# linkedin/spark-tfrecord

Measured on AMD Instinct MI355X. Metric: rows/sec read+write (1M-row Example round-trip), higher is better.
Workload: dtype wire(int64/float32/bytes); 1 GPU; model=Example{id:int64, ints:Int64List[8], floats:FloatList[16], tokens:BytesList[2]}, global_batch=1000000, parallelism=dp1, rows_per_rank=1000000, engine=gpu, storage=/dev/shm, crc_verify=True

## Files before the change

### csrc/codec_core.h

```cpp
#pragma once

#include <cstdint>
#include <cstring>

#include "crc32c.h"

namespace tfrec {

using i64 = int64_t;
using u64 = uint64_t;
using u32 = uint32_t;
using u8 = uint8_t;

enum Kind : int32_t { KIND_BYTES = 1, KIND_FLOAT = 2, KIND_INT64 = 3 };

enum RecordFormat : int32_t { FMT_EXAMPLE = 0, FMT_SEQUENCE = 1, FMT_BYTE_ARRAY = 2 };

enum CodecErr : int32_t {
  ERR_OK = 0,
  ERR_TRUNCATED = -1,
  ERR_BAD_VARINT = -2,
  ERR_KIND_MISMATCH = -3,
  ERR_BAD_WIRETYPE = -4,
  ERR_OVERFLOW = -5,
// ... 455 lines not shown
    c.crc = crc32c_step8(c.crc, c.w0, c.tab);
    c.w0 = c.w1;
    c.wpos += 8;
    c.w1 = cur_load(c, c.wpos + 8);
  }
  u32 crc = c.crc;
  for (i64 b = c.wpos; b < c.len; ++b)
    crc = c.tab[0][(crc ^ c.base[b]) & 0xFF] ^ (crc >> 8);
  return ~crc;
}

TFR_HOSTDEV inline bool cur_varint(ScanCur& c, i64 end, u64* out) {
  i64 avail = end - c.pos;
  if (avail <= 0) return false;
  u64 w = cur_peek(c);
  u64 stops = ~w & kMsbMask;
  if (stops) {
    int nb = (ctz64(stops) >> 3) + 1;
    if (nb > avail) return false;
    u64 v = 0;
    for (int i = 0; i < nb; ++i) v |= ((w >> (8 * i)) & 0x7F) << (7 * i);
    *out = v;
    cur_advance(c, nb);
    return true;
  }
  if (avail < 9) return false;
  u64 v = 0;
  for (int i = 0; i < 8; ++i) v |= ((w >> (8 * i)) & 0x7F) << (7 * i);
  cur_advance(c, 8);
  for (int shift = 56; shift < 64 && c.pos < end; shift += 7) {
    u8 b = (u8)cur_peek(c);
    v |= (u64)(b & 0x7F) << shift;
    cur_advance(c, 1);
    if (!(b & 0x80)) {
      *out = v;
      return true;
    }
  }
  return false;
}

TFR_HOSTDEV inline int32_t cur_skip_field(ScanCur& c, i64 end, u32 wt) {
  u64 tmp;
  switch (wt) {
    case 0:
      return cur_varint(c, end, &tmp) ? ERR_OK : ERR_BAD_VARINT;
    case 1:
      if (end - c.pos < 8) return ERR_TRUNCATED;
      cur_advance(c, 8);
      return ERR_OK;
    case 2:
      if (!cur_varint(c, end, &tmp)) return ERR_BAD_VARINT;
      if ((u64)(end - c.pos) < tmp) return ERR_TRUNCATED;
      cur_advance(c, (i64)tmp);
      return ERR_OK;
    case 5:
      if (end - c.pos < 4) return ERR_TRUNCATED;
      cur_advance(c, 4);
      return ERR_OK;
    default:
      return ERR_BAD_WIRETYPE;
  }
}

TFR_HOSTDEV inline i64 cur_count_terms(ScanCur& c, i64 n) {
  i64 cnt = 0;
  while (n >= 8) {
    cnt += popcount64(~cur_peek(c) & kMsbMask);
    cur_advance(c, 8);
    n -= 8;
  }
  if (n > 0) {
    u64 mask = kMsbMask >> (8 * (8 - n));
    cnt += popcount64(~cur_peek(c) & mask);
    cur_advance(c, n);
  }
  return cnt;
}

TFR_HOSTDEV inline int32_t cur_count_list_body(ScanCur& c, i64 end, int32_t kind,
                                               i64* nvals, i64* nbytes) {
  while (c.pos < end) {
    u64 tag;
    if (!cur_varint(c, end, &tag)) return ERR_BAD_VARINT;
    u32 fieldno = (u32)(tag >> 3), wt = (u32)(tag & 7);
    if (fieldno != 1) {
      int32_t rc = cur_skip_field(c, end, wt);
      if (rc != ERR_OK) return rc;
      continue;
    }
    if (kind == KIND_BYTES) {
      if (wt != 2) return ERR_BAD_WIRETYPE;
      u64 blen;
      if (!cur_varint(c, end, &blen)) return ERR_BAD_VARINT;
      if ((u64)(end - c.pos) < blen) return ERR_TRUNCATED;
      *nvals += 1;
      *nbytes += (i64)blen;
      cur_advance(c, (i64)blen);
    } else if (kind == KIND_FLOAT) {
      if (wt == 2) {
        u64 blen;
        if (!cur_varint(c, end, &blen)) return ERR_BAD_VARINT;
        if ((u64)(end - c.pos) < blen) return ERR_TRUNCATED;
        *nvals += (i64)(blen / 4);
        cur_advance(c, (i64)blen);
      } else if (wt == 5) {
        if (end - c.pos < 4) return ERR_TRUNCATED;
        *nvals += 1;
        cur_advance(c, 4);
      } else {
        return ERR_BAD_WIRETYPE;
      }
    } else {
      if (wt == 2) {
        u64 blen;
        if (!cur_varint(c, end, &blen)) return ERR_BAD_VARINT;
        if ((u64)(end - c.pos) < blen) return ERR_TRUNCATED;
        if (blen && (c.base[c.pos + (i64)blen - 1] & 0x80))
          return ERR_BAD_VARINT;
        *nvals += cur_count_terms(c, (i64)blen);
      } else if (wt == 0) {
        u64 v;
        if (!cur_varint(c, end, &v)) return ERR_BAD_VARINT;
        *nvals += 1;
      } else {
        return ERR_BAD_WIRETYPE;
      }
    }
  }
  return ERR_OK;
}

TFR_HOSTDEV inline int32_t cur_scan_feature_body(ScanCur& c, i64 end,
                                                 int32_t expect_kind,
                                                 int32_t* kind_found, i64* nvals,
                                                 i64* nbytes) {
  while (c.pos < end) {
    u64 tag;
    if (!cur_varint(c, end, &tag)) return ERR_BAD_VARINT;
    u32 fieldno = (u32)(tag >> 3), wt = (u32)(tag & 7);
    if (fieldno >= 1 && fieldno <= 3 && wt == 2) {
      u64 blen;
      if (!cur_varint(c, end, &blen)) return ERR_BAD_VARINT;
      if ((u64)(end - c.pos) < blen) return ERR_TRUNCATED;
      *kind_found = (int32_t)fieldno;
      if (expect_kind >= 0 && (int32_t)fieldno != expect_kind)
        return ERR_KIND_MISMATCH;
      int32_t rc = cur_count_list_body(c, c.pos + (i64)blen, (int32_t)fieldno,
                                       nvals, nbytes);
      if (rc != ERR_OK) return rc;
    } else {
      int32_t rc = cur_skip_field(c, end, wt);
      if (rc != ERR_OK) return rc;
    }
  }
  return ERR_OK;
}

TFR_HOSTDEV inline int32_t cur_scan_features_body(ScanCur& c, i64 end, i64 data_rel,
                                                  const SchemaView& schema,
                                                  int want_seq, FieldStat* stats) {
  i64 body_start = c.pos;
  while (c.pos < end) {
    u64 tag;
    if (!cur_varint(c, end, &tag)) return ERR_BAD_VARINT;
    u32 fieldno = (u32)(tag >> 3), wt = (u32)(tag & 7);
    if (fieldno != 1 || wt != 2) {
      int32_t rc = cur_skip_field(c, end, wt);
      if (rc != ERR_OK) return rc;
      continue;
    }
    u64 entry_len;
    if (!cur_varint(c, end, &entry_len)) return ERR_BAD_VARINT;
    if ((u64)(end - c.pos) < entry_len) return ERR_TRUNCATED;
    i64 ee = c.pos + (i64)entry_len;
    int f = -1;
    bool key_seen = false;
    bool val_seen = false;
    while (c.pos < ee) {
      u64 etag;
      if (!cur_varint(c, ee, &etag)) return ERR_BAD_VARINT;
      u32 efn = (u32)(etag >> 3), ewt = (u32)(etag & 7);
      if (efn == 1 && ewt == 2) {
        if (val_seen) return ERR_RETRY_UNFUSED;
        u64 klen;
        if (!cur_varint(c, ee, &klen)) return ERR_BAD_VARINT;
        if ((u64)(ee - c.pos) < klen) return ERR_TRUNCATED;
        f = schema_find(schema, c.base + c.pos, (int)klen, want_seq);
        key_seen = true;
        cur_advance(c, (i64)klen);
      } else if (efn == 2 && ewt == 2) {
        if (!key_seen) return ERR_RETRY_UNFUSED;
        val_seen = true;
        u64 vlen;
        if (!cur_varint(c, ee, &vlen)) return ERR_BAD_VARINT;
        if ((u64)(ee - c.pos) < vlen) return ERR_TRUNCATED;
        i64 ve = c.pos + (i64)vlen;
        if (f < 0) {
          cur_advance(c, (i64)vlen);
          continue;
        }
        FieldStat* st = &stats[f];
        st->nvals = 0;
        st->nbytes = 0;
        st->nlists = 0;
        st->kind_found = 0;
        st->err = 0;
        st->pos = data_rel + c.pos;
        st->len = (i64)vlen;
        if (!want_seq) {
          int32_t rc = cur_scan_feature_body(c, ve, schema.fields[f].kind,
                                             &st->kind_found, &st->nvals,
                                             &st->nbytes);
          if (rc == ERR_RETRY_UNFUSED) return rc;
          if (rc != ERR_OK) st->err = rc;
        } else {
          while (c.pos < ve && st->err == ERR_OK) {
            u64 ltag;
            if (!cur_varint(c, ve, &ltag)) {
              st->err = ERR_BAD_VARINT;
              break;
            }
            u32 lfn = (u32)(ltag >> 3), lwt = (u32)(ltag & 7);
            if (lfn == 1 && lwt == 2) {
              u64 flen;
              if (!cur_varint(c, ve, &flen) || (u64)(ve - c.pos) < flen) {
                st->err = ERR_TRUNCATED;
                break;
              }
              st->nlists += 1;
              int32_t kf = 0;
              int32_t rc = cur_scan_feature_body(c, c.pos + (i64)flen,
                                                 schema.fields[f].kind, &kf,
                                                 &st->nvals, &st->nbytes);
              if (rc == ERR_RETRY_UNFUSED) return rc;
              if (rc != ERR_OK) {
                st->err = rc;
                break;
              }
              if (kf) st->kind_found = kf;
            } else {
              int32_t rc = cur_skip_field(c, ve, lwt);
              if (rc != ERR_OK) {
                st->err = ERR_TRUNCATED;
                break;
              }
            }
          }
        }
        if (c.pos < ve) cur_advance(c, ve - c.pos);
      } else {
        int32_t rc = cur_skip_field(c, ee, ewt);
        if (rc != ERR_OK) return rc;
      }
    }
    if (f >= 0 && !val_seen) {
      FieldStat* st = &stats[f];
      st->pos = data_rel + body_start;
      st->len = 0;
      st->nvals = 0;
      st->nbytes = 0;
      st->nlists = 0;
      st->kind_found = 0;
      st->err = 0;
    }
  }
  return ERR_OK;
}

TFR_HOSTDEV inline int32_t scan_record_fused(const u8* data, i64 abs_off,
                                             i64 rec_len, int32_t fmt,
                                             const SchemaView& schema,
                                             FieldStat* stats, u32* crc_out,
                                             const uint32_t (*tab)[256]) {
  ScanCur c;
  cur_init(c, data + abs_off, rec_len, tab);
  while (c.pos < rec_len) {
    u64 tag;
    if (!cur_varint(c, rec_len, &tag)) return ERR_BAD_VARINT;
    u32 fieldno = (u32)(tag >> 3), wt = (u32)(tag & 7);
    bool is_features = fieldno == 1;
    bool is_fl = (fmt == FMT_SEQUENCE && fieldno == 2);
    if ((is_features || is_fl) && wt == 2) {
      u64 blen;
      if (!cur_varint(c, rec_len, &blen)) return ERR_BAD_VARINT;
      if ((u64)(rec_len - c.pos) < blen) return ERR_TRUNCATED;
      int32_t rc = cur_scan_features_body(c, c.pos + (i64)blen, abs_off, schema,
                                          is_fl ? 1 : 0, stats);
      if (rc != ERR_OK) return rc;
    } else {
      int32_t rc = cur_skip_field(c, rec_len, wt);
      if (rc != ERR_OK) return rc;
    }
  }
  *crc_out = cur_finish_crc(c);
  return ERR_OK;
}


struct DecodeDst {
  i64* i64_vals;
  float* f32_vals;
  u8* bytes_data;
  i64* elem_len;
  i64* sub_count;
};

TFR_HOSTDEV inline int32_t extract_list_body(const u8* p, const u8* end, int32_t kind,
                                             const DecodeDst& dst, i64* vi, i64* bi) {
  while (p < end) {
    u64 tag;
    p = read_varint(p, end, &tag);
    if (!p) return ERR_BAD_VARINT;
    u32 fieldno = static_cast<u32>(tag >> 3);
    u32 wt = static_cast<u32>(tag & 7);
    if (fieldno != 1) {
      p = skip_field(p, end, wt);
      if (!p) return ERR_TRUNCATED;
      continue;
    }
    if (kind == KIND_BYTES) {
      u64 len;
      p = read_varint(p, end, &len);
      if (!p || static_cast<u64>(end - p) < len) return ERR_TRUNCATED;
      u8* d = dst.bytes_data + *bi;
      u64 i = 0;
      for (; i + 8 <= len; i += 8) {
        u64 w;
        __builtin_memcpy(&w, p + i, 8);
        __builtin_memcpy(d + i, &w, 8);
      }
      for (; i < len; ++i) d[i] = p[i];
      dst.elem_len[*vi] = static_cast<i64>(len);
      *bi += static_cast<i64>(len);
      *vi += 1;
      p += len;
    } else if (kind == KIND_FLOAT) {
      if (wt == 2) {
        u64 len;
        p = read_varint(p, end, &len);
        if (!p || static_cast<u64>(end - p) < len) return ERR_TRUNCATED;
        u64 n = len / 4;
        __builtin_memcpy(dst.f32_vals + *vi, p, n * 4);
        *vi += static_cast<i64>(n);
        p += len;
      } else {
        if (end - p < 4) return ERR_TRUNCATED;
        float v;
        __builtin_memcpy(&v, p, 4);
        dst.f32_vals[(*vi)++] = v;
        p += 4;
      }
    } else {
      if (wt == 2) {
        u64 len;
        p = read_varint(p, end, &len);
        if (!p || static_cast<u64>(end - p) < len) return ERR_TRUNCATED;
        const u8* q = p;
        const u8* qe = p + len;
        while (q < qe) {
          u64 v;
          q = read_varint(q, qe, &v);
          if (!q) return ERR_BAD_VARINT;
          dst.i64_vals[(*vi)++] = static_cast<i64>(v);
        }
        p = qe;
      } else {
        u64 v;
        p = read_varint(p, end, &v);
        if (!p) return ERR_BAD_VARINT;
        dst.i64_vals[(*vi)++] = static_cast<i64>(v);
      }
    }
  }
  return ERR_OK;
}

TFR_HOSTDEV inline int32_t extract_feature_body(const u8* p, const u8* end,
                                                int32_t kind, const DecodeDst& dst,
                                                i64* vi, i64* bi) {
  while (p < end) {
    u64 tag;
    p = read_varint(p, end, &tag);
    if (!p) return ERR_BAD_VARINT;
    u32 fieldno = static_cast<u32>(tag >> 3);
    u32 wt = static_cast<u32>(tag & 7);
    if (fieldno >= 1 && fieldno <= 3 && wt == 2) {
      u64 len;
      p = read_varint(p, end, &len);
      if (!p || static_cast<u64>(end - p) < len) return ERR_TRUNCATED;
      int32_t rc = extract_list_body(p, p + len, kind, dst, vi, bi);
      if (rc != ERR_OK) return rc;
      p += len;
    } else {
      p = skip_field(p, end, wt);
      if (!p) return ERR_TRUNCATED;
    }
  }
  return ERR_OK;
}

TFR_HOSTDEV inline int32_t extract_field(const u8* data, i64 pos, i64 len,
                                         int32_t kind, int32_t is_seq,
                                         const DecodeDst& dst, i64 val_base,
                                         i64 byte_base, i64 list_base) {
  if (pos < 0) return ERR_OK;
  const u8* p = data + pos;
  const u8* end = p + len;
  i64 vi = val_base;
  i64 bi = byte_base;
  if (!is_seq) return extract_feature_body(p, end, kind, dst, &vi, &bi);
  i64 li = list_base;
  while (p < end) {
    u64 tag;
    p = read_varint(p, end, &tag);
    if (!p) return ERR_BAD_VARINT;
    u32 fieldno = static_cast<u32>(tag >> 3);
    u32 wt = static_cast<u32>(tag & 7);
    if (fieldno == 1 && wt == 2) {
      u64 flen;
      p = read_varint(p, end, &flen);
      if (!p || static_cast<u64>(end - p) < flen) return ERR_TRUNCATED;
      i64 v_before = vi;
      int32_t rc = extract_feature_body(p, p + flen, kind, dst, &vi, &bi);
      if (rc != ERR_OK) return rc;
      dst.sub_count[li++] = vi - v_before;
      p += flen;
    } else {
      p = skip_field(p, end, wt);
      if (!p) return ERR_TRUNCATED;
    }
  }
  return ERR_OK;
}


struct FieldColumn {
  int32_t kind;
  int32_t is_seq;
  const u8* presence;
  const i64* row_off;
  const i64* list_off;
  const i64* sub_off;
  const i64* elem_off;
  const u8* bytes_data;
  const i64* i64_vals;
  const float* f32_vals;
};

TFR_HOSTDEV inline i64 list_body_size(const FieldColumn& c, i64 v0, i64 v1) {
  if (c.kind == KIND_FLOAT) {
    i64 n = v1 - v0;
    return n ? (1 + varint_size(static_cast<u64>(4 * n)) + 4 * n) : 0;
  }
  if (c.kind == KIND_INT64) {
    i64 packed = 0;
    for (i64 v = v0; v < v1; ++v)
      packed += varint_size(static_cast<u64>(c.i64_vals[v]));
    return packed ? (1 + varint_size(static_cast<u64>(packed)) + packed) : 0;
  }
  i64 sz = 0;
  for (i64 v = v0; v < v1; ++v) {
    i64 blen = c.elem_off[v + 1] - c.elem_off[v];
    sz += 1 + varint_size(static_cast<u64>(blen)) + blen;
  }
  return sz;
}

TFR_HOSTDEV inline i64 feature_body_size(const FieldColumn& c, i64 v0, i64 v1) {
  i64 body = list_body_size(c, v0, v1);
  return 1 + varint_size(static_cast<u64>(body)) + body;
}

TFR_HOSTDEV inline u8* emit_list_body(u8* o, const FieldColumn& c, i64 v0, i64 v1) {
  if (c.kind == KIND_FLOAT) {
    i64 n = v1 - v0;
    if (n) {
      *o++ = 0x0A;
      o = write_varint(o, static_cast<u64>(4 * n));
      __builtin_memcpy(o, c.f32_vals + v0, static_cast<size_t>(4 * n));
      o += 4 * n;
    }
  } else if (c.kind == KIND_INT64) {
    i64 packed = 0;
    for (i64 v = v0; v < v1; ++v)
      packed += varint_size(static_cast<u64>(c.i64_vals[v]));
    if (packed) {
      *o++ = 0x0A;
      o = write_varint(o, static_cast<u64>(packed));
      for (i64 v = v0; v < v1; ++v)
        o = write_varint(o, static_cast<u64>(c.i64_vals[v]));
    }
  } else {
    for (i64 v = v0; v < v1; ++v) {
      i64 b0 = c.elem_off[v];
      i64 blen = c.elem_off[v + 1] - b0;
      *o++ = 0x0A;
      o = write_varint(o, static_cast<u64>(blen));
      for (i64 i = 0; i < blen; ++i) o[i] = c.bytes_data[b0 + i];
      o += blen;
    }
  }
  return o;
}

TFR_HOSTDEV inline u8* emit_feature_body(u8* o, const FieldColumn& c, i64 v0, i64 v1) {
  i64 body = list_body_size(c, v0, v1);
  *o++ = static_cast<u8>((c.kind << 3) | 2);
  o = write_varint(o, static_cast<u64>(body));
  return emit_list_body(o, c, v0, v1);
}

TFR_HOSTDEV inline i64 features_entry_size(const FieldColumn& c, const SchemaView& s,
                                           int f, i64 v0, i64 v1) {
  i64 fb = feature_body_size(c, v0, v1);
  i64 klen = s.name_len(f);
  return (1 + varint_size(static_cast<u64>(klen)) + klen) +
         (1 + varint_size(static_cast<u64>(fb)) + fb);
}

TFR_HOSTDEV inline u8* emit_features_entry(u8* o, const FieldColumn& c,
                                           const SchemaView& s, int f, i64 v0, i64 v1) {
  i64 fb = feature_body_size(c, v0, v1);
  i64 klen = s.name_len(f);
  *o++ = 0x0A;
  o = write_varint(o, static_cast<u64>(klen));
  const u8* nm = s.name(f);
  for (i64 i = 0; i < klen; ++i) o[i] = nm[i];
  o += klen;
  *o++ = 0x12;
  o = write_varint(o, static_cast<u64>(fb));
  return emit_feature_body(o, c, v0, v1);
}

TFR_HOSTDEV inline i64 feature_list_body_size(const FieldColumn& c, i64 r) {
  i64 sz = 0;
  for (i64 j = c.list_off[r]; j < c.list_off[r + 1]; ++j) {
    i64 fb = feature_body_size(c, c.sub_off[j], c.sub_off[j + 1]);
    sz += 1 + varint_size(static_cast<u64>(fb)) + fb;
  }
  return sz;
}

TFR_HOSTDEV inline u8* emit_feature_list_body(u8* o, const FieldColumn& c, i64 r) {
  for (i64 j = c.list_off[r]; j < c.list_off[r + 1]; ++j) {
    i64 fb = feature_body_size(c, c.sub_off[j], c.sub_off[j + 1]);
    *o++ = 0x0A;
    o = write_varint(o, static_cast<u64>(fb));
    o = emit_feature_body(o, c, c.sub_off[j], c.sub_off[j + 1]);
  }
  return o;
}

TFR_HOSTDEV inline i64 feature_lists_entry_size(const FieldColumn& c,
                                                const SchemaView& s, int f, i64 r) {
  i64 flb = feature_list_body_size(c, r);
  i64 klen = s.name_len(f);
  return (1 + varint_size(static_cast<u64>(klen)) + klen) +
         (1 + varint_size(static_cast<u64>(flb)) + flb);
}

TFR_HOSTDEV inline u8* emit_feature_lists_entry(u8* o, const FieldColumn& c,
                                                const SchemaView& s, int f, i64 r) {
  i64 flb = feature_list_body_size(c, r);
  i64 klen = s.name_len(f);
  *o++ = 0x0A;
  o = write_varint(o, static_cast<u64>(klen));
  const u8* nm = s.name(f);
  for (i64 i = 0; i < klen; ++i) o[i] = nm[i];
  o += klen;
  *o++ = 0x12;
  o = write_varint(o, static_cast<u64>(flb));
  return emit_feature_list_body(o, c, r);
}

TFR_HOSTDEV inline i64 record_payload_size(const FieldColumn* cols,
                                           const SchemaView& s, int32_t fmt, i64 r) {
  i64 ctx_body = 0;
  i64 fl_body = 0;
  for (int f = 0; f < s.nfields; ++f) {
    const FieldColumn& c = cols[f];
    if (!c.presence[r]) continue;
    if (!c.is_seq) {
      i64 e = features_entry_size(c, s, f, c.row_off[r], c.row_off[r + 1]);
      ctx_body += 1 + varint_size(static_cast<u64>(e)) + e;
    } else {
      i64 e = feature_lists_entry_size(c, s, f, r);
      fl_body += 1 + varint_size(static_cast<u64>(e)) + e;
    }
  }
  i64 total = 0;
  if (fmt == FMT_EXAMPLE) {
    total += 1 + varint_size(static_cast<u64>(ctx_body)) + ctx_body;
  } else {
    if (ctx_body) total += 1 + varint_size(static_cast<u64>(ctx_body)) + ctx_body;
    total += 1 + varint_size(static_cast<u64>(fl_body)) + fl_body;
  }
  return total;
}

TFR_HOSTDEV inline u8* emit_record_payload(u8* o, const FieldColumn* cols,
                                           const SchemaView& s, int32_t fmt, i64 r) {
  i64 ctx_body = 0, fl_body = 0;
  for (int f = 0; f < s.nfields; ++f) {
    const FieldColumn& c = cols[f];
    if (!c.presence[r]) continue;
    if (!c.is_seq) {
      i64 e = features_entry_size(c, s, f, c.row_off[r], c.row_off[r + 1]);
      ctx_body += 1 + varint_size(static_cast<u64>(e)) + e;
    } else {
      i64 e = feature_lists_entry_size(c, s, f, r);
      fl_body += 1 + varint_size(static_cast<u64>(e)) + e;
    }
  }
  auto emit_ctx = [&](u8* oo) {
    for (int f = 0; f < s.nfields; ++f) {
      const FieldColumn& c = cols[f];
      if (!c.presence[r] || c.is_seq) continue;
      i64 e = features_entry_size(c, s, f, c.row_off[r], c.row_off[r + 1]);
      *oo++ = 0x0A;
      oo = write_varint(oo, static_cast<u64>(e));
      oo = emit_features_entry(oo, c, s, f, c.row_off[r], c.row_off[r + 1]);
    }
    return oo;
  };
  auto emit_fl = [&](u8* oo) {
    for (int f = 0; f < s.nfields; ++f) {
      const FieldColumn& c = cols[f];
      if (!c.presence[r] || !c.is_seq) continue;
      i64 e = feature_lists_entry_size(c, s, f, r);
      *oo++ = 0x0A;
      oo = write_varint(oo, static_cast<u64>(e));
      oo = emit_feature_lists_entry(oo, c, s, f, r);
    }
    return oo;
  };
  if (fmt == FMT_EXAMPLE) {
    *o++ = 0x0A;
    o = write_varint(o, static_cast<u64>(ctx_body));
    o = emit_ctx(o);
  } else {
    if (ctx_body) {
      *o++ = 0x0A;
      o = write_varint(o, static_cast<u64>(ctx_body));
      o = emit_ctx(o);
    }
    *o++ = 0x12;
    o = write_varint(o, static_cast<u64>(fl_body));
    o = emit_fl(o);
  }
  return o;
}



struct WriteCur {
  u8* base;
  i64 pos;
  i64 wpos;
  u64 win;
  u32 crc;
  const uint32_t (*tab)[256];
};

TFR_HOSTDEV inline void wcur_init(WriteCur& w, u8* base,
                                  const uint32_t (*tab)[256]) {
  w.base = base;
  w.pos = 0;
  w.wpos = 0;
  w.win = 0;
  w.crc = 0xFFFFFFFFu;
  w.tab = tab;
}

TFR_HOSTDEV inline void wcur_flush8(WriteCur& w) {
  __builtin_memcpy(w.base + w.wpos, &w.win, 8);
  w.crc = crc32c_step8(w.crc, w.win, w.tab);
  w.wpos += 8;
  w.win = 0;
}

TFR_HOSTDEV inline void wcur_put(WriteCur& w, u8 b) {
  w.win |= (u64)b << (8 * (w.pos - w.wpos));
  if (++w.pos - w.wpos == 8) wcur_flush8(w);
}

TFR_HOSTDEV inline void wcur_varint(WriteCur& w, u64 v) {
  while (v >= 0x80) {
    wcur_put(w, (u8)(v | 0x80));
    v >>= 7;
  }
  wcur_put(w, (u8)v);
}

TFR_HOSTDEV inline void wcur_bytes(WriteCur& w, const u8* src, i64 n) {
  while (n > 0 && (w.pos - w.wpos) != 0) {
    wcur_put(w, *src++);
    --n;
  }
  while (n >= 8) {
    __builtin_memcpy(&w.win, src, 8);
    w.pos += 8;
    wcur_flush8(w);
    src += 8;
    n -= 8;
  }
  while (n-- > 0) wcur_put(w, *src++);
}

TFR_HOSTDEV inline u32 wcur_finish(WriteCur& w) {
  int rem = (int)(w.pos - w.wpos);
  if (!rem) return ~w.crc;
  __builtin_memcpy(w.base + w.wpos, &w.win, (size_t)rem);
  u32 crc = w.crc;
  for (int i = 0; i < rem; ++i)
    crc = w.tab[0][(crc ^ (u8)(w.win >> (8 * i))) & 0xFF] ^ (crc >> 8);
  return ~crc;
}

TFR_HOSTDEV inline void wcur_list_body(WriteCur& w, const FieldColumn& c,
                                       i64 v0, i64 v1) {
  if (c.kind == KIND_FLOAT) {
    i64 n = v1 - v0;
    if (n) {
      wcur_put(w, 0x0A);
      wcur_varint(w, (u64)(4 * n));
      wcur_bytes(w, (const u8*)(c.f32_vals + v0), 4 * n);
    }
  } else if (c.kind == KIND_INT64) {
// ... 149 lines not shown
```

### csrc/ext.cpp

```cpp

#include <pybind11/numpy.h>
#include <pybind11/pybind11.h>
#include <pybind11/stl.h>

#include <fcntl.h>
#include <unistd.h>

#include <atomic>
#include <condition_variable>
#include <cstring>
#include <functional>
#include <map>
#include <mutex>
#include <stdexcept>
#include <string>
#include <thread>
#include <vector>

#include "codec_core.h"
#include "inflate_core.h"

namespace py = pybind11;
using namespace tfrec;

namespace {


class IOPool {
 public:
  static IOPool& instance() {
    static IOPool* pool = new IOPool(8);
    return *pool;
  }

  int run(bool is_write, int fd, u8* ptr, i64 n, i64 off) {
    return run_spans(n, [=](i64 o, i64 m) {
      return is_write ? do_write(fd, ptr + o, m, off + o)
                      : do_read(fd, ptr + o, m, off + o);
    });
  }

  template <typename Fn>
  int run_spans(i64 n, Fn&& fn) {
    return run_parts(n, 64 << 10, std::forward<Fn>(fn));
  }

  template <typename Fn>
  int run_parts(i64 n, i64 min_span, Fn&& fn) {
    if (n <= 0) return 0;
    int nspan = (int)nthreads_;
    i64 span = (n + nspan - 1) / nspan;
    if (span < min_span) {
      nspan = (int)((n + min_span - 1) / min_span);
      if (nspan < 1) nspan = 1;
      span = (n + nspan - 1) / nspan;
    }
    if (nspan == 1) return fn((i64)0, n);
    if (getenv("TFREC_POOL_DEBUG"))
      fprintf(stderr, "[pool] n=%lld nspan=%d span=%lld\n", (long long)n,
              nspan, (long long)span);
    std::atomic<int> err{0};
    std::atomic<int> left{nspan};
    {
      std::unique_lock<std::mutex> lk(mu_);
      for (int t = 0; t < nspan; ++t) {
        i64 o = (i64)t * span;
        i64 m = std::min(span, n - o);
        tasks_.push_back([=, &err, &left] {
          int e = fn(o, m);
          if (e) err.store(e, std::memory_order_relaxed);
          if (left.fetch_sub(1) == 1) {
            std::lock_guard<std::mutex> dl(done_mu_);
            done_cv_.notify_all();
          }
        });
      }
      cv_.notify_all();
    }
    std::unique_lock<std::mutex> dl(done_mu_);
    done_cv_.wait(dl, [&] { return left.load() == 0; });
    return err.load();
  }

 private:
  explicit IOPool(int n) : nthreads_(n) {
    for (int i = 0; i < n; ++i)
      workers_.emplace_back([this] { worker(); });
  }

  static int do_write(int fd, const u8* p, i64 n, i64 off) {
    while (n > 0) {
      ssize_t w = ::pwrite(fd, p, (size_t)n, (off_t)off);
      if (w < 0) {
        if (errno == EINTR) continue;
        return -errno;
      }
      p += w;
      n -= w;
      off += w;
    }
    return 0;
  }

  static int do_read(int fd, u8* p, i64 n, i64 off) {
    while (n > 0) {
      ssize_t r = ::pread(fd, p, (size_t)n, (off_t)off);
      if (r < 0) {
        if (errno == EINTR) continue;
        return -errno;
      }
      if (r == 0) return -EIO;
      p += r;
      n -= r;
      off += r;
    }
    return 0;
  }

  void worker() {
    for (;;) {
      std::function<void()> task;
      {
        std::unique_lock<std::mutex> lk(mu_);
        cv_.wait(lk, [this] { return !tasks_.empty(); });
        task = std::move(tasks_.back());
        tasks_.pop_back();
      }
      task();
    }
  }

  size_t nthreads_;
  std::vector<std::thread> workers_;
  std::vector<std::function<void()>> tasks_;
  std::mutex mu_;
  std::condition_variable cv_;
  std::mutex done_mu_;
  std::condition_variable done_cv_;
};

void pwrite_parallel(int fd, uintptr_t ptr, i64 n, i64 file_off) {
  int e;
  {
    py::gil_scoped_release rel;
    e = IOPool::instance().run(true, fd, (u8*)ptr, n, file_off);
  }
  if (e) throw std::runtime_error("pwrite failed: " + std::string(strerror(-e)));
}

void pread_parallel(int fd, uintptr_t ptr, i64 n, i64 file_off) {
  int e;
  {
    py::gil_scoped_release rel;
    e = IOPool::instance().run(false, fd, (u8*)ptr, n, file_off);
  }
  if (e) throw std::runtime_error("pread failed: " + std::string(strerror(-e)));
}

struct BufView {
  const u8* data;
  i64 size;
};

BufView as_bytes(const py::buffer& b, py::buffer_info& info) {
  info = b.request();
  if (info.itemsize != 1) throw std::invalid_argument("expected a byte buffer");
  return BufView{static_cast<const u8*>(info.ptr), static_cast<i64>(info.size)};
}


std::pair<py::array_t<i64>, py::array_t<i64>> scan_frames(py::buffer data,
                                                          bool verify_crc) {
  py::buffer_info info;
  BufView buf = as_bytes(data, info);
  std::vector<i64> offs, lens;
  i64 p = 0;
  while (p < buf.size) {
    if (buf.size - p < 12)
      throw std::runtime_error("corrupt TFRecord: truncated frame header at offset " +
                               std::to_string(p));
    u64 len;
    std::memcpy(&len, buf.data + p, 8);
    u32 len_crc;
    std::memcpy(&len_crc, buf.data + p + 8, 4);
    if (verify_crc && mask_crc(crc32c(buf.data + p, 8)) != len_crc)
      throw std::runtime_error("corrupt TFRecord: bad length CRC at offset " +
                               std::to_string(p));
    if (static_cast<u64>(buf.size - p - 12) < len + 4)
      throw std::runtime_error("corrupt TFRecord: truncated payload at offset " +
                               std::to_string(p));
    if (verify_crc) {
      u32 data_crc;
      std::memcpy(&data_crc, buf.data + p + 12 + len, 4);
      if (mask_crc(crc32c(buf.data + p + 12, len)) != data_crc)
        throw std::runtime_error("corrupt TFRecord: bad data CRC at offset " +
                                 std::to_string(p));
    }
    offs.push_back(p + 12);
    lens.push_back(static_cast<i64>(len));
    p += 12 + static_cast<i64>(len) + 4;
  }
  auto off_arr = py::array_t<i64>(offs.size());
  auto len_arr = py::array_t<i64>(lens.size());
  std::memcpy(off_arr.mutable_data(), offs.data(), offs.size() * 8);
  std::memcpy(len_arr.mutable_data(), lens.data(), lens.size() * 8);
  return {off_arr, len_arr};
}

std::pair<py::array_t<i64>, py::array_t<i64>> scan_frame_headers(py::buffer data) {
  return scan_frames(data, false);
}


const char* err_name(int32_t e) {
  switch (e) {
    case ERR_TRUNCATED: return "truncated message";
    case ERR_BAD_VARINT: return "malformed varint";
    case ERR_KIND_MISMATCH: return "feature kind does not match schema";
    case ERR_BAD_WIRETYPE: return "unexpected wire type";
    default: return "codec error";
  }
}

py::list decode_records(py::buffer data, py::array_t<i64> rec_off,
                        py::array_t<i64> rec_len, py::bytes schema_blob,
                        int32_t fmt) {
  py::buffer_info info;
  BufView buf = as_bytes(data, info);
  std::string blob = schema_blob;
  SchemaView schema = schema_view(reinterpret_cast<const u8*>(blob.data()));
  const i64 R = rec_off.size();
  const int F = schema.nfields;
  auto off = rec_off.unchecked<1>();
  auto len = rec_len.unchecked<1>();

  std::vector<FieldStat> stats(static_cast<size_t>(R) * F);
  {
    std::atomic<i64> bad_rec{-1};
    std::atomic<int32_t> bad_rc{0};
    std::atomic<int> bad_field{-1};
    {
      py::gil_scoped_release rel;
      IOPool::instance().run_parts(R, 4096, [&](i64 o, i64 m) {
        for (i64 r = o; r < o + m; ++r) {
          FieldStat* st = stats.data() + r * F;
          for (int f = 0; f < F; ++f) field_stat_clear(&st[f]);
          int32_t rc = scan_record(buf.data, off(r), len(r), fmt, schema, st);
          for (int f = 0; rc == ERR_OK && f < F; ++f)
            if (st[f].err != ERR_OK) {
              rc = st[f].err;
              bad_field.store(f);
            }
          if (rc != ERR_OK) {
            bad_rec.store(r);
            bad_rc.store(rc);
            return 1;
          }
        }
        return 0;
      });
    }
    if (bad_rec.load() >= 0) {
      i64 r = bad_rec.load();
      int32_t rc = bad_rc.load();
      if (rc == ERR_KIND_MISMATCH && bad_field.load() >= 0) {
        int f = bad_field.load();
        std::string nm(reinterpret_cast<const char*>(schema.name(f)),
                       schema.name_len(f));
        throw std::runtime_error("Feature '" + nm +
                                 "' kind does not match requested data type (record " +
                                 std::to_string(r) + ")");
      }
      throw std::runtime_error(std::string("TFRecord decode failed in record ") +
                               std::to_string(r) + ": " + err_name(rc));
    }
  }

  py::list out;
  for (int f = 0; f < F; ++f) {
    const FieldDescRaw& fd = schema.fields[f];
    i64 total_vals = 0, total_bytes = 0, total_lists = 0;
    auto presence = py::array_t<u8>(R);
    auto row_off_arr = py::array_t<i64>(R + 1);
    u8* pres = presence.mutable_data();
    i64* row_off_p = row_off_arr.mutable_data();
    row_off_p[0] = 0;
    py::array_t<i64> list_off_arr(fd.is_seq ? R + 1 : 1);
    i64* list_off_p = list_off_arr.mutable_data();
    list_off_p[0] = 0;
    for (i64 r = 0; r < R; ++r) {
      const FieldStat& st = stats[r * F + f];
      pres[r] = st.pos >= 0 ? 1 : 0;
      total_vals += st.nvals;
      total_bytes += st.nbytes;
      total_lists += st.nlists;
      row_off_p[r + 1] = total_vals;
      if (fd.is_seq) list_off_p[r + 1] = total_lists;
    }

    DecodeDst dst{};
    py::array_t<i64> i64_vals(0);
    py::array_t<float> f32_vals(0);
    py::array_t<u8> bytes_data(0);
    py::array_t<i64> elem_len(0);
    py::array_t<i64> sub_count(0);
    if (fd.kind == KIND_INT64) {
      i64_vals = py::array_t<i64>(total_vals);
      dst.i64_vals = i64_vals.mutable_data();
    } else if (fd.kind == KIND_FLOAT) {
      f32_vals = py::array_t<float>(total_vals);
      dst.f32_vals = f32_vals.mutable_data();
    } else {
      bytes_data = py::array_t<u8>(total_bytes);
      elem_len = py::array_t<i64>(total_vals);
      dst.bytes_data = bytes_data.mutable_data();
      dst.elem_len = elem_len.mutable_data();
    }
    if (fd.is_seq) {
      sub_count = py::array_t<i64>(total_lists);
      dst.sub_count = sub_count.mutable_data();
    }

    {
      std::vector<i64> byte_base_v(R);
      std::vector<i64> list_base_v(fd.is_seq ? R : 0);
      i64 bb = 0, lb = 0;
      for (i64 r = 0; r < R; ++r) {
        const FieldStat& st = stats[r * F + f];
        byte_base_v[r] = bb;
        bb += st.nbytes;
        if (fd.is_seq) {
          list_base_v[r] = lb;
          lb += st.nlists;
        }
      }
      const FieldStat* stp = stats.data();
      const u8* datap = buf.data;
      int rc;
      {
        py::gil_scoped_release rel;
        rc = IOPool::instance().run_parts(R, 4096, [&](i64 o, i64 m) {
          for (i64 r = o; r < o + m; ++r) {
            const FieldStat& st = stp[r * F + f];
            int32_t e = extract_field(datap, st.pos, st.len, fd.kind,
                                      fd.is_seq, dst, row_off_p[r],
                                      byte_base_v[r],
                                      fd.is_seq ? list_base_v[r] : 0);
            if (e != ERR_OK) return (int)-e;
          }
          return 0;
        });
      }
      if (rc != 0)
        throw std::runtime_error(std::string("TFRecord decode failed: ") +
                                 err_name((int32_t)-rc));
    }

    py::dict d;
    d["presence"] = presence;
    d["row_off"] = row_off_arr;
    if (fd.kind == KIND_INT64) d["values"] = i64_vals;
    else if (fd.kind == KIND_FLOAT) d["values"] = f32_vals;
    else {
      d["values"] = bytes_data;
      d["elem_len"] = elem_len;
    }
    if (fd.is_seq) {
      d["list_off"] = list_off_arr;
      d["sub_count"] = sub_count;
    }
    out.append(d);
  }
  return out;
}


template <typename T>
const T* opt_ptr(const py::dict& d, const char* key) {
  if (!d.contains(key)) return nullptr;
  auto arr = d[key].cast<py::array_t<T>>();
  return arr.data();
}

struct ColKeepAlive {
  std::vector<py::object> refs;
  template <typename T>
  const T* get(const py::dict& d, const char* key) {
    if (!d.contains(key)) return nullptr;
    py::array_t<T, py::array::c_style | py::array::forcecast> arr =
        py::cast<py::array_t<T, py::array::c_style | py::array::forcecast>>(d[key]);
    refs.push_back(arr);
    return arr.data();
  }
};

py::bytes encode_records(py::bytes schema_blob, int32_t fmt, py::list col_dicts,
                         i64 R) {
  std::string blob = schema_blob;
  SchemaView schema = schema_view(reinterpret_cast<const u8*>(blob.data()));
  const int F = schema.nfields;
  if (static_cast<int>(col_dicts.size()) != F)
    throw std::invalid_argument("column count does not match schema");

  ColKeepAlive keep;
  std::vector<FieldColumn> cols(F);
  for (int f = 0; f < F; ++f) {
    py::dict d = col_dicts[f].cast<py::dict>();
    FieldColumn& c = cols[f];
    c.kind = schema.fields[f].kind;
    c.is_seq = schema.fields[f].is_seq;
    c.presence = keep.get<u8>(d, "presence");
    c.row_off = keep.get<i64>(d, "row_off");
    c.list_off = keep.get<i64>(d, "list_off");
    c.sub_off = keep.get<i64>(d, "sub_off");
    c.elem_off = keep.get<i64>(d, "elem_off");
    c.bytes_data = keep.get<u8>(d, "values_bytes");
    c.i64_vals = keep.get<i64>(d, "values_i64");
    c.f32_vals = keep.get<float>(d, "values_f32");
    if (!c.presence || !c.row_off)
      throw std::invalid_argument("column missing presence/row_off");
  }

  std::string out;
  bool emit_mismatch = false;
  {
    py::gil_scoped_release rel;
    std::vector<i64> frame_off(R + 1);
    std::vector<i64> psize(R);
    const FieldColumn* cp = cols.data();
    IOPool::instance().run_parts(R, 4096, [&](i64 o, i64 m) {
      for (i64 r = o; r < o + m; ++r)
        psize[r] = record_payload_size(cp, schema, fmt, r);
      return 0;
    });
    frame_off[0] = 0;
    for (i64 r = 0; r < R; ++r)
      frame_off[r + 1] = frame_off[r] + psize[r] + kFrameOverhead;
    i64 total = frame_off[R];

    out.resize(static_cast<size_t>(total), '\0');
    u8* file = reinterpret_cast<u8*>(out.data());
    int rc = IOPool::instance().run_parts(R, 4096, [&](i64 o, i64 m) {
      for (i64 r = o; r < o + m; ++r) {
        u8* dst = file + frame_off[r] + 12;
        u32 crc = 0;
        i64 emitted = emit_record_payload_fused(dst, cp, schema, fmt, r, &crc,
                                                kCrcTables.t);
        if (emitted != psize[r]) return 1;
        write_frame_header_footer_crc(file, frame_off[r], psize[r], crc,
                                      kCrcTables.t);
      }
      return 0;
    });
    emit_mismatch = rc != 0;
  }
  if (emit_mismatch)
    throw std::runtime_error("internal error: emit size mismatch");
  return py::bytes(out);
}

py::bytes frame_byte_arrays(py::buffer data, py::array_t<i64> elem_off) {
  py::buffer_info info;
  BufView buf = as_bytes(data, info);
  auto off = elem_off.unchecked<1>();
  i64 R = elem_off.size() - 1;
  i64 total = 0;
  for (i64 r = 0; r < R; ++r) total += (off(r + 1) - off(r)) + kFrameOverhead;
  std::string out(static_cast<size_t>(total), '\0');
  u8* file = reinterpret_cast<u8*>(out.data());
  i64 fo = 0;
  for (i64 r = 0; r < R; ++r) {
    i64 n = off(r + 1) - off(r);
    std::memcpy(file + fo + 12, buf.data + off(r), static_cast<size_t>(n));
    write_frame_header_footer(file, fo, n, kCrcTables.t);
    fo += n + kFrameOverhead;
  }
  return py::bytes(out);
}


inline int lattice_code_for(int32_t kind, bool multi, bool seq) {
  int rank = 4 - kind;
  if (seq) return 6 + rank;
  if (multi) return 3 + rank;
  return rank;
}

void infer_features_body(const u8* p, const u8* end, bool seq,
                         std::map<std::string, int>& codes) {
  while (p < end) {
    u64 tag;
    p = read_varint(p, end, &tag);
    if (!p) throw std::runtime_error("malformed record during schema inference");
    u32 fieldno = static_cast<u32>(tag >> 3);
    u32 wt = static_cast<u32>(tag & 7);
    if (fieldno != 1 || wt != 2) {
      p = skip_field(p, end, wt);
      if (!p) throw std::runtime_error("malformed record during schema inference");
      continue;
    }
    u64 entry_len;
    p = read_varint(p, end, &entry_len);
    if (!p || static_cast<u64>(end - p) < entry_len)
      throw std::runtime_error("malformed record during schema inference");
    const u8* ep = p;
    const u8* ee = p + entry_len;
    p = ee;
    std::string key;
    const u8* val = nullptr;
    u64 val_len = 0;
    while (ep < ee) {
      u64 etag;
      ep = read_varint(ep, ee, &etag);
      if (!ep) throw std::runtime_error("malformed map entry during schema inference");
      u32 efn = static_cast<u32>(etag >> 3);
      u32 ewt = static_cast<u32>(etag & 7);
      if (efn == 1 && ewt == 2) {
        u64 klen;
        ep = read_varint(ep, ee, &klen);
        if (!ep || static_cast<u64>(ee - ep) < klen)
          throw std::runtime_error("malformed map entry during schema inference");
        key.assign(reinterpret_cast<const char*>(ep), klen);
        ep += klen;
      } else if (efn == 2 && ewt == 2) {
        ep = read_varint(ep, ee, &val_len);
        if (!ep || static_cast<u64>(ee - ep) < val_len)
          throw std::runtime_error("malformed map entry during schema inference");
        val = ep;
        ep += val_len;
      } else {
        ep = skip_field(ep, ee, ewt);
        if (!ep) throw std::runtime_error("malformed map entry during schema inference");
      }
    }
    if (key.empty() && !val) continue;
    int code = 0;
    if (val) {
      if (!seq) {
        int32_t kf = 0;
        i64 nvals = 0, nbytes = 0;
        int32_t rc = scan_feature_body(val, val + val_len, -1, &kf, &nvals, &nbytes);
        if (rc != ERR_OK)
          throw std::runtime_error("malformed Feature during schema inference");
        if (kf != 0 && nvals > 0) code = lattice_code_for(kf, nvals > 1, false);
      } else {
        const u8* lp = val;
        const u8* le = val + val_len;
        int32_t kind_seen = 0;
        bool any_vals = false;
        while (lp < le) {
          u64 ltag;
          lp = read_varint(lp, le, &ltag);
          if (!lp) throw std::runtime_error("malformed FeatureList during inference");
          u32 lfn = static_cast<u32>(ltag >> 3);
          u32 lwt = static_cast<u32>(ltag & 7);
          if (lfn == 1 && lwt == 2) {
            u64 flen;
            lp = read_varint(lp, le, &flen);
            if (!lp || static_cast<u64>(le - lp) < flen)
              throw std::runtime_error("malformed FeatureList during inference");
            int32_t kf = 0;
            i64 nvals = 0, nbytes = 0;
            int32_t rc = scan_feature_body(lp, lp + flen, -1, &kf, &nvals, &nbytes);
            if (rc != ERR_OK)
              throw std::runtime_error("malformed Feature during schema inference");
            if (kf) {
              kind_seen = std::max(kind_seen, lattice_code_for(kf, false, false));
              if (nvals >= 0) any_vals = true;
            }
            lp += flen;
          } else {
            lp = skip_field(lp, le, lwt);
            if (!lp) throw std::runtime_error("malformed FeatureList during inference");
          }
        }
        (void)any_vals;
        if (kind_seen) code = 6 + kind_seen;
      }
    }
    auto it = codes.find(key);
    if (it == codes.end()) codes[key] = code;
    else it->second = std::max(it->second, code);
  }
}

py::dict infer_schema_codes(py::buffer data, py::array_t<i64> rec_off,
                            py::array_t<i64> rec_len, int32_t fmt) {
  py::buffer_info info;
  BufView buf = as_bytes(data, info);
  auto off = rec_off.unchecked<1>();
  auto len = rec_len.unchecked<1>();
  std::map<std::string, int> ctx_codes, seq_codes;
  for (i64 r = 0; r < rec_off.size(); ++r) {
    const u8* p = buf.data + off(r);
    const u8* end = p + len(r);
    while (p < end) {
      u64 tag;
      p = read_varint(p, end, &tag);
      if (!p) throw std::runtime_error("malformed record during schema inference");
      u32 fieldno = static_cast<u32>(tag >> 3);
      u32 wt = static_cast<u32>(tag & 7);
      bool is_features = fieldno == 1;
      bool is_fl = (fmt == FMT_SEQUENCE && fieldno == 2);
      if ((is_features || is_fl) && wt == 2) {
        u64 blen;
        p = read_varint(p, end, &blen);
        if (!p || static_cast<u64>(end - p) < blen)
          throw std::runtime_error("malformed record during schema inference");
        infer_features_body(p, p + blen, is_fl, is_fl ? seq_codes : ctx_codes);
        p += blen;
      } else {
        p = skip_field(p, end, wt);
        if (!p) throw std::runtime_error("malformed record during schema inference");
      }
    }
  }
  auto safe_str = [](const std::string& v) {
    return py::reinterpret_steal<py::str>(
        PyUnicode_DecodeUTF8(v.data(), (Py_ssize_t)v.size(), "replace"));
  };
  py::dict out;
  for (auto& kv : ctx_codes) out[safe_str(kv.first)] = kv.second;
  for (auto& kv : seq_codes) {
    out[safe_str(kv.first)] = kv.second;
  }
  return out;
}

py::dict scan_stats_debug(py::buffer data, py::array_t<i64> rec_off,
                          py::array_t<i64> rec_len, int32_t fmt,
                          py::bytes schema_blob, bool fused) {
  py::buffer_info info;
  BufView buf = as_bytes(data, info);
  std::string blob = schema_blob;
  SchemaView schema = schema_view(reinterpret_cast<const u8*>(blob.data()));
  const int F = schema.nfields;
  auto off = rec_off.unchecked<1>();
  auto len = rec_len.unchecked<1>();
  i64 R = rec_off.size();
  auto stats_arr = py::array_t<i64>({R, (i64)F, (i64)6});
  auto crc_arr = py::array_t<i64>(R);
  auto rc_arr = py::array_t<i64>(R);
  auto* st_all = reinterpret_cast<FieldStat*>(stats_arr.mutable_data());
  for (i64 r = 0; r < R; ++r) {
    FieldStat* st = st_all + r * F;
    for (int f = 0; f < F; ++f) field_stat_clear(&st[f]);
    int32_t rc;
    u32 crc = 0;
    if (fused) {
      rc = scan_record_fused(buf.data, off(r), len(r), fmt, schema, st, &crc,
                             kCrcTables.t);
      if (rc == ERR_RETRY_UNFUSED) {
        for (int f = 0; f < F; ++f) field_stat_clear(&st[f]);
        rc = scan_record(buf.data, off(r), len(r), fmt, schema, st);
        crc = crc32c(buf.data + off(r), (size_t)len(r));
      }
    } else {
      rc = scan_record(buf.data, off(r), len(r), fmt, schema, st);
      crc = crc32c(buf.data + off(r), (size_t)len(r));
    }
    crc_arr.mutable_at(r) = rc == ERR_OK ? (i64)crc : -1;
    rc_arr.mutable_at(r) = rc;
  }
  py::dict out;
  out["stats"] = stats_arr;
  out["crc"] = crc_arr;
  out["rc"] = rc_arr;
  return out;
}

py::bytes host_inflate_segment(py::buffer comp, i64 expect) {
  auto info = comp.request();
// ... 79 lines not shown
```

### csrc/hip/kernels.hip

```cpp

#include <hip/hip_runtime.h>
#include <pybind11/pybind11.h>
#include <pybind11/stl.h>
#include <rocprim/rocprim.hpp>

#include <fcntl.h>
#include <sys/mman.h>
#include <sys/stat.h>
#include <unistd.h>

#include <cstdint>
#include <map>
#include <mutex>
#include <stdexcept>
#include <string>
#include <vector>

#include "../codec_core.h"

namespace py = pybind11;
using namespace tfrec;

#define HIP_CHECK(expr)                                                          \
  do {                                                                           \
    hipError_t _e = (expr);                                                      \
    if (_e != hipSuccess)                                                        \
      throw std::runtime_error(std::string("HIP error: ") +                      \
                               hipGetErrorString(_e) + " at " __FILE__ ":" +     \
                               std::to_string(__LINE__));                        \
  } while (0)

namespace {

constexpr int kBlock = 256;

__device__ inline void stage_crc_tables(uint32_t (*lds)[256]) {
  const uint32_t* src = &kCrcTables.t[0][0];
  uint32_t* dst = &lds[0][0];
  for (int i = threadIdx.x; i < 8 * 256; i += blockDim.x) dst[i] = src[i];
  __syncthreads();
}

__device__ inline void set_err(int32_t* err, int32_t code, i64 r) {
  err[0] = code;
  i64 v = r + 1;
  atomicMax(&err[1], v > 0x7FFFFFFF ? (int32_t)0x7FFFFFFF : (int32_t)v);
}


__global__ void crc_verify_kernel(const u8* __restrict__ data,
                                  const i64* __restrict__ off,
                                  const i64* __restrict__ len, i64 R,
                                  unsigned long long* err_out) {
  __shared__ uint32_t tab[8][256];
  stage_crc_tables(tab);
  for (i64 r = blockIdx.x * (i64)blockDim.x + threadIdx.x; r < R;
       r += (i64)gridDim.x * blockDim.x) {
    const u8* h = data + off[r] - 12;
    u32 len_crc, data_crc;
    __builtin_memcpy(&len_crc, h + 8, 4);
    __builtin_memcpy(&data_crc, h + 12 + len[r], 4);
    bool ok = mask_crc(crc32c_sw(h, 8, 0, tab)) == len_crc &&
              mask_crc(crc32c_sw(h + 12, (size_t)len[r], 0, tab)) == data_crc;
    if (!ok) atomicMin(err_out, (unsigned long long)(r + 1));
  }
}


static_assert(sizeof(FieldStat) == 48, "FieldStat layout shared with Python");

__global__ void scan_records_kernel(const u8* __restrict__ data,
                                    const i64* __restrict__ off,
                                    const i64* __restrict__ len, i64 R, int32_t fmt,
                                    const u8* __restrict__ schema_blob, int F,
                                    FieldStat* __restrict__ stats,
                                    int32_t* __restrict__ err,
                                    unsigned long long* crc_err,
                                    i64 rec_base) {
  __shared__ uint32_t tab[8][256];
  if (crc_err) stage_crc_tables(tab);
  SchemaView schema = schema_view(schema_blob);
  for (i64 r = blockIdx.x * (i64)blockDim.x + threadIdx.x; r < R;
       r += (i64)gridDim.x * blockDim.x) {
    FieldStat* st = stats + r * F;
    for (int f = 0; f < F; ++f) field_stat_clear(&st[f]);
    int32_t rc;
    if (crc_err) {
      u32 payload_crc = 0;
      rc = scan_record_fused(data, off[r], len[r], fmt, schema, st,
                             &payload_crc, tab);
      if (rc == ERR_RETRY_UNFUSED) {
        for (int f = 0; f < F; ++f) field_stat_clear(&st[f]);
        rc = scan_record(data, off[r], len[r], fmt, schema, st);
        payload_crc = crc32c_sw(data + off[r], (size_t)len[r], 0, tab);
      }
      if (rc != ERR_OK)
        payload_crc = crc32c_sw(data + off[r], (size_t)len[r], 0, tab);
      const u8* h = data + off[r] - 12;
      u32 len_crc, data_crc;
      __builtin_memcpy(&len_crc, h + 8, 4);
      __builtin_memcpy(&data_crc, h + 12 + len[r], 4);
      bool ok = mask_crc(crc32c_sw(h, 8, 0, tab)) == len_crc &&
                mask_crc(payload_crc) == data_crc;
      if (!ok) atomicMin(crc_err, (unsigned long long)(rec_base + r + 1));
    } else {
      rc = scan_record(data, off[r], len[r], fmt, schema, st);
    }
    if (rc != ERR_OK) set_err(err, rc, rec_base + r);
    for (int f = 0; f < F; ++f)
      if (st[f].err != ERR_OK) set_err(err, st[f].err, rec_base + r);
  }
}


struct DevFieldDst {
  int32_t kind;
  int32_t is_seq;
  i64* i64_vals;
  float* f32_vals;
  u8* bytes_data;
  i64* elem_len;
  i64* sub_count;
  const i64* val_base;
  const i64* byte_base;
  const i64* list_base;
};

__global__ void extract_fields_kernel(const u8* __restrict__ data, i64 R, int F,
                                      const FieldStat* __restrict__ stats,
                                      const DevFieldDst* __restrict__ metas,
                                      int32_t* __restrict__ err, i64 r0) {
  i64 total = R * F;
  for (i64 idx = blockIdx.x * (i64)blockDim.x + threadIdx.x; idx < total;
       idx += (i64)gridDim.x * blockDim.x) {
    i64 q = idx / F;
    int f = (int)(idx - q * F);
    i64 r = r0 + q;
    const DevFieldDst& m = metas[f];
    const FieldStat& st = stats[r * F + f];
    DecodeDst dst{m.i64_vals, m.f32_vals, m.bytes_data, m.elem_len, m.sub_count};
    int32_t rc = extract_field(data, st.pos, st.len, m.kind, m.is_seq, dst,
                               m.val_base ? m.val_base[r] : 0,
                               m.byte_base ? m.byte_base[r] : 0,
                               m.list_base ? m.list_base[r] : 0);
    if (rc != ERR_OK) set_err(err, rc, r);
  }
}



__global__ void size_records_kernel(const FieldColumn* __restrict__ cols,
                                    const u8* __restrict__ schema_blob, int32_t fmt,
                                    i64 R, i64* __restrict__ psize) {
  SchemaView schema = schema_view(schema_blob);
  for (i64 r = blockIdx.x * (i64)blockDim.x + threadIdx.x; r < R;
       r += (i64)gridDim.x * blockDim.x) {
    psize[r] = record_payload_size(cols, schema, fmt, r) + kFrameOverhead;
  }
}

__global__ void emit_records_kernel(const FieldColumn* __restrict__ cols,
                                    const u8* __restrict__ schema_blob, int32_t fmt,
                                    i64 r0, i64 R, const i64* __restrict__ frame_off,
                                    u8* __restrict__ file,
                                    int32_t* __restrict__ err) {
  __shared__ uint32_t tab[8][256];
  stage_crc_tables(tab);
  SchemaView schema = schema_view(schema_blob);
  for (i64 r = r0 + blockIdx.x * (i64)blockDim.x + threadIdx.x; r < R;
       r += (i64)gridDim.x * blockDim.x) {
    i64 payload = (frame_off[r + 1] - frame_off[r]) - kFrameOverhead;
    u8* o = file + frame_off[r] + 12;
    u32 crc = 0;
    i64 emitted = emit_record_payload_fused(o, cols, schema, fmt, r, &crc,
                                            tab);
    if (emitted != payload) set_err(err, ERR_OVERFLOW, r);
    write_frame_header_footer_crc(file, frame_off[r], payload, crc, tab);
  }
}


constexpr i64 kWaveRecordBytes = 8 << 10;

__device__ inline u32 crc32c_wave(const u8* p, i64 n,
                                  const uint32_t (*tab)[256]) {
  int lane = threadIdx.x & 63;
  i64 chunk = (n + 63) / 64;
  if (chunk < 64) chunk = 64;
  i64 s = (i64)lane * chunk;
  i64 e = s + chunk < n ? s + chunk : n;
  u32 my = (s < e) ? crc32c_sw(p + s, (size_t)(e - s), 0, tab) : 0;
  u32 acc = __shfl(my, 0);
  if (chunk < n) {
    u32 op = crc32c_shift_elem((u64)chunk);
    for (int i = 1; i < 64; ++i) {
      i64 si = (i64)i * chunk;
      if (si >= n) break;
      u32 ci = __shfl(my, i);
      i64 li = (si + chunk < n ? chunk : n - si);
      acc = (li == chunk) ? (crc_gfmul(acc, op) ^ ci)
                          : crc32c_combine_fast(acc, ci, (u64)li);
    }
  }
  return acc;
}

__device__ inline void copy_wave(u8* d, const u8* s, i64 n) {
  int lane = threadIdx.x & 63;
  i64 i = (i64)lane * 8;
  for (; i + 8 <= n; i += 64 * 8) {
    u64 w;
    __builtin_memcpy(&w, s + i, 8);
    __builtin_memcpy(d + i, &w, 8);
  }
  i64 tail = n & ~((i64)7);
  for (i64 b = tail + lane; b < n; b += 64) d[b] = s[b];
}

__global__ void crc_verify_wave_kernel(const u8* __restrict__ data,
                                       const i64* __restrict__ off,
                                       const i64* __restrict__ len, i64 R,
                                       unsigned long long* err_out) {
  __shared__ uint32_t tab[8][256];
  stage_crc_tables(tab);
  i64 wave = (blockIdx.x * (i64)blockDim.x + threadIdx.x) / 64;
  i64 nwaves = ((i64)gridDim.x * blockDim.x) / 64;
  for (i64 r = wave; r < R; r += nwaves) {
    const u8* h = data + off[r] - 12;
    u32 payload = crc32c_wave(h + 12, len[r], tab);
    if ((threadIdx.x & 63) == 0) {
      u32 len_crc, data_crc;
      __builtin_memcpy(&len_crc, h + 8, 4);
      __builtin_memcpy(&data_crc, h + 12 + len[r], 4);
      bool ok = mask_crc(crc32c_sw(h, 8, 0, tab)) == len_crc &&
                mask_crc(payload) == data_crc;
      if (!ok) atomicMin(err_out, (unsigned long long)(r + 1));
    }
  }
}

__global__ void frame_bytes_wave_kernel(const u8* __restrict__ src,
                                        const i64* __restrict__ elem_off,
                                        const i64* __restrict__ frame_off, i64 R,
                                        u8* __restrict__ file) {
  __shared__ uint32_t tab[8][256];
  stage_crc_tables(tab);
  i64 wave = (blockIdx.x * (i64)blockDim.x + threadIdx.x) / 64;
  i64 nwaves = ((i64)gridDim.x * blockDim.x) / 64;
  for (i64 r = wave; r < R; r += nwaves) {
    i64 n = elem_off[r + 1] - elem_off[r];
    const u8* s = src + elem_off[r];
    u8* d = file + frame_off[r] + 12;
    copy_wave(d, s, n);
    u32 crc = crc32c_wave(s, n, tab);
    if ((threadIdx.x & 63) == 0)
      write_frame_header_footer_crc(file, frame_off[r], n, crc, tab);
  }
}

__global__ void gather_payloads_wave_kernel(const u8* __restrict__ data,
                                            const i64* __restrict__ off,
                                            const i64* __restrict__ len,
                                            const i64* __restrict__ dst_off,
                                            i64 R, u8* __restrict__ out) {
  i64 wave = (blockIdx.x * (i64)blockDim.x + threadIdx.x) / 64;
  i64 nwaves = ((i64)gridDim.x * blockDim.x) / 64;
  for (i64 r = wave; r < R; r += nwaves)
    copy_wave(out + dst_off[r], data + off[r], len[r]);
}


__device__ inline i64 wave_incl_scan(i64 v) {
  int lane = threadIdx.x & 63;
  for (int d = 1; d < 64; d <<= 1) {
    i64 y = __shfl_up(v, d);
    if (lane >= d) v += y;
  }
  return v;
}

__device__ inline i64 wave_extract_i64_packed(const u8* __restrict__ p, i64 n,
                                              i64* __restrict__ out, i64 base) {
  int lane = threadIdx.x & 63;
  i64 chunk = (n + 63) / 64;
  i64 lo = (i64)lane * chunk;
  i64 hi = lo + chunk < n ? lo + chunk : n;
  i64 cnt = 0;
  for (i64 i = lo; i < hi; ++i) cnt += !(p[i] & 0x80);
  i64 incl = wave_incl_scan(cnt);
  i64 excl = incl - cnt;
  i64 total = __shfl(incl, 63);
  i64 q = lo;
  i64 pre = 0;
  if (lo > 0 && lo < hi) {
    if (p[lo - 1] & 0x80) {
      while (q < hi && (p[q] & 0x80)) ++q;
      if (q < hi) {
        ++q;
        pre = 1;
      }
    }
  }
  i64 idx = base + excl + pre;
  while (q < hi) {
    u64 v = 0;
    int shift = 0;
    i64 j = q;
    while (j < n && shift < 70) {
      u8 b = p[j++];
      v |= (u64)(b & 0x7F) << shift;
      shift += 7;
      if (!(b & 0x80)) break;
    }
    out[idx++] = (i64)v;
    q = j;
  }
  return total;
}

__device__ inline int32_t extract_list_body_wave(const u8* __restrict__ p,
                                                 const u8* end, int32_t kind,
                                                 const DecodeDst& dst, i64* vi,
                                                 i64* bi) {
  int lane = threadIdx.x & 63;
  while (p < end) {
    u64 tag;
    p = read_varint(p, end, &tag);
    if (!p) return ERR_BAD_VARINT;
    u32 fieldno = (u32)(tag >> 3), wt = (u32)(tag & 7);
    if (fieldno != 1) {
      p = skip_field(p, end, wt);
      if (!p) return ERR_TRUNCATED;
      continue;
    }
    if (kind == KIND_BYTES) {
      u64 len;
      p = read_varint(p, end, &len);
      if (!p || (u64)(end - p) < len) return ERR_TRUNCATED;
      copy_wave(dst.bytes_data + *bi, p, (i64)len);
      if (lane == 0) dst.elem_len[*vi] = (i64)len;
      *bi += (i64)len;
      *vi += 1;
      p += len;
    } else if (kind == KIND_FLOAT) {
      if (wt == 2) {
        u64 len;
        p = read_varint(p, end, &len);
        if (!p || (u64)(end - p) < len) return ERR_TRUNCATED;
        u64 nv = len / 4;
        copy_wave((u8*)(dst.f32_vals + *vi), p, (i64)(nv * 4));
        *vi += (i64)nv;
        p += len;
      } else {
        if (end - p < 4) return ERR_TRUNCATED;
        if (lane == 0) {
          float v;
          __builtin_memcpy(&v, p, 4);
          dst.f32_vals[*vi] = v;
        }
        (*vi)++;
        p += 4;
      }
    } else {
      if (wt == 2) {
        u64 len;
        p = read_varint(p, end, &len);
        if (!p || (u64)(end - p) < len) return ERR_TRUNCATED;
        *vi += wave_extract_i64_packed(p, (i64)len, dst.i64_vals, *vi);
        p += len;
      } else {
        u64 v;
        p = read_varint(p, end, &v);
        if (!p) return ERR_BAD_VARINT;
        if (lane == 0) dst.i64_vals[*vi] = (i64)v;
        (*vi)++;
      }
    }
  }
  return ERR_OK;
}

__device__ inline int32_t extract_feature_body_wave(const u8* __restrict__ p,
                                                    const u8* end, int32_t kind,
                                                    const DecodeDst& dst,
                                                    i64* vi, i64* bi) {
  while (p < end) {
    u64 tag;
    p = read_varint(p, end, &tag);
    if (!p) return ERR_BAD_VARINT;
    u32 fieldno = (u32)(tag >> 3), wt = (u32)(tag & 7);
    if (fieldno >= 1 && fieldno <= 3 && wt == 2) {
      u64 len;
      p = read_varint(p, end, &len);
      if (!p || (u64)(end - p) < len) return ERR_TRUNCATED;
      int32_t rc = extract_list_body_wave(p, p + len, kind, dst, vi, bi);
      if (rc != ERR_OK) return rc;
      p += len;
    } else {
      p = skip_field(p, end, wt);
      if (!p) return ERR_TRUNCATED;
    }
  }
  return ERR_OK;
}

__device__ inline int32_t extract_field_wave(const u8* __restrict__ data,
                                             i64 pos, i64 len, int32_t kind,
                                             int32_t is_seq, const DecodeDst& dst,
                                             i64 val_base, i64 byte_base,
                                             i64 list_base) {
  if (pos < 0) return ERR_OK;
  int lane = threadIdx.x & 63;
  const u8* p = data + pos;
  const u8* end = p + len;
  i64 vi = val_base;
  i64 bi = byte_base;
  if (!is_seq) return extract_feature_body_wave(p, end, kind, dst, &vi, &bi);
  i64 li = list_base;
  while (p < end) {
    u64 tag;
    p = read_varint(p, end, &tag);
    if (!p) return ERR_BAD_VARINT;
    u32 fieldno = (u32)(tag >> 3), wt = (u32)(tag & 7);
    if (fieldno == 1 && wt == 2) {
      u64 flen;
      p = read_varint(p, end, &flen);
      if (!p || (u64)(end - p) < flen) return ERR_TRUNCATED;
      i64 v_before = vi;
      int32_t rc = extract_feature_body_wave(p, p + flen, kind, dst, &vi, &bi);
      if (rc != ERR_OK) return rc;
      if (lane == 0) dst.sub_count[li] = vi - v_before;
      ++li;
      p += flen;
    } else {
      p = skip_field(p, end, wt);
      if (!p) return ERR_TRUNCATED;
    }
  }
  return ERR_OK;
}

__global__ void scan_records_wave_kernel(const u8* __restrict__ data,
                                         const i64* __restrict__ off,
                                         const i64* __restrict__ len, i64 R,
                                         int32_t fmt,
                                         const u8* __restrict__ schema_blob,
                                         int F, FieldStat* __restrict__ stats,
                                         int32_t* __restrict__ err,
                                         unsigned long long* crc_err,
                                         i64 rec_base) {
  __shared__ uint32_t tab[8][256];
  stage_crc_tables(tab);
  SchemaView schema = schema_view(schema_blob);
  i64 wave = (blockIdx.x * (i64)blockDim.x + threadIdx.x) / 64;
  i64 nwaves = ((i64)gridDim.x * blockDim.x) / 64;
  int lane = threadIdx.x & 63;
  for (i64 r = wave; r < R; r += nwaves) {
    if (lane == 0) {
      FieldStat* st = stats + r * F;
      for (int f = 0; f < F; ++f) field_stat_clear(&st[f]);
      int32_t rc = scan_record(data, off[r], len[r], fmt, schema, st);
      if (rc != ERR_OK) set_err(err, rc, rec_base + r);
      for (int f = 0; f < F; ++f)
        if (st[f].err != ERR_OK) set_err(err, st[f].err, rec_base + r);
    }
    if (crc_err) {
      const u8* h = data + off[r] - 12;
      u32 payload = crc32c_wave(h + 12, len[r], tab);
      if (lane == 0) {
        u32 len_crc, data_crc;
        __builtin_memcpy(&len_crc, h + 8, 4);
        __builtin_memcpy(&data_crc, h + 12 + len[r], 4);
        bool ok = mask_crc(crc32c_sw(h, 8, 0, tab)) == len_crc &&
                  mask_crc(payload) == data_crc;
        if (!ok) atomicMin(crc_err, (unsigned long long)(rec_base + r + 1));
      }
    }
  }
}

__global__ void extract_fields_wave_kernel(const u8* __restrict__ data, i64 R,
                                           int F,
                                           const FieldStat* __restrict__ stats,
                                           const DevFieldDst* __restrict__ metas,
                                           int32_t* __restrict__ err, i64 r0) {
  i64 total = R * F;
  i64 wave = (blockIdx.x * (i64)blockDim.x + threadIdx.x) / 64;
  i64 nwaves = ((i64)gridDim.x * blockDim.x) / 64;
  for (i64 idx = wave; idx < total; idx += nwaves) {
    i64 q = idx / F;
    int f = (int)(idx - q * F);
    i64 r = r0 + q;
    const DevFieldDst& m = metas[f];
    const FieldStat& st = stats[r * F + f];
    DecodeDst dst{m.i64_vals, m.f32_vals, m.bytes_data, m.elem_len, m.sub_count};
    int32_t rc = extract_field_wave(data, st.pos, st.len, m.kind, m.is_seq, dst,
                                    m.val_base ? m.val_base[r] : 0,
                                    m.byte_base ? m.byte_base[r] : 0,
                                    m.list_base ? m.list_base[r] : 0);
    if (rc != ERR_OK && (threadIdx.x & 63) == 0) set_err(err, rc, r);
  }
}


__device__ inline i64 wave_emit_i64_packed(u8* __restrict__ o,
                                           const i64* __restrict__ vals,
                                           i64 v0, i64 v1) {
  int lane = threadIdx.x & 63;
  i64 n = v1 - v0;
  i64 chunk = (n + 63) / 64;
  i64 lo = v0 + (i64)lane * chunk;
  i64 hi = lo + chunk < v1 ? lo + chunk : v1;
  i64 sz = 0;
  for (i64 v = lo; v < hi; ++v) sz += varint_size((u64)vals[v]);
  i64 incl = wave_incl_scan(sz);
  u8* q = o + (incl - sz);
  for (i64 v = lo; v < hi; ++v) q = write_varint(q, (u64)vals[v]);
  return __shfl(incl, 63);
}

struct WaveCur {
  u8* base;
  i64 pos;
};

__device__ inline void wvc_put(WaveCur& w, u8 b) {
  if ((threadIdx.x & 63) == 0) w.base[w.pos] = b;
  w.pos += 1;
}

__device__ inline void wvc_varint(WaveCur& w, u64 v) {
  if ((threadIdx.x & 63) == 0) write_varint(w.base + w.pos, v);
  w.pos += varint_size(v);
}

__device__ inline void wvc_bytes(WaveCur& w, const u8* s, i64 n) {
  copy_wave(w.base + w.pos, s, n);
  w.pos += n;
}

__device__ inline void wvc_list_body(WaveCur& w, const FieldColumn& c, i64 v0,
                                     i64 v1) {
  if (c.kind == KIND_FLOAT) {
    i64 n = v1 - v0;
    if (n) {
      wvc_put(w, 0x0A);
      wvc_varint(w, (u64)(4 * n));
      wvc_bytes(w, (const u8*)(c.f32_vals + v0), 4 * n);
    }
  } else if (c.kind == KIND_INT64) {
    i64 packed = 0;
    for (i64 v = v0; v < v1; ++v) packed += varint_size((u64)c.i64_vals[v]);
    if (packed) {
      wvc_put(w, 0x0A);
      wvc_varint(w, (u64)packed);
      w.pos += wave_emit_i64_packed(w.base + w.pos, c.i64_vals, v0, v1);
    }
  } else {
    for (i64 v = v0; v < v1; ++v) {
      i64 b0 = c.elem_off[v];
      i64 blen = c.elem_off[v + 1] - b0;
      wvc_put(w, 0x0A);
      wvc_varint(w, (u64)blen);
      wvc_bytes(w, c.bytes_data + b0, blen);
    }
  }
}

__device__ inline void wvc_feature_body(WaveCur& w, const FieldColumn& c,
                                        i64 v0, i64 v1) {
  i64 body = list_body_size(c, v0, v1);
  wvc_put(w, (u8)((c.kind << 3) | 2));
  wvc_varint(w, (u64)body);
  wvc_list_body(w, c, v0, v1);
}

__device__ inline void wvc_features_entry(WaveCur& w, const FieldColumn& c,
                                          const SchemaView& s, int f, i64 v0,
                                          i64 v1) {
  i64 fb = feature_body_size(c, v0, v1);
  i64 klen = s.name_len(f);
  wvc_put(w, 0x0A);
  wvc_varint(w, (u64)klen);
  wvc_bytes(w, s.name(f), klen);
  wvc_put(w, 0x12);
  wvc_varint(w, (u64)fb);
  wvc_feature_body(w, c, v0, v1);
}

__device__ inline void wvc_feature_lists_entry(WaveCur& w, const FieldColumn& c,
                                               const SchemaView& s, int f,
                                               i64 r) {
  i64 flb = feature_list_body_size(c, r);
  i64 klen = s.name_len(f);
  wvc_put(w, 0x0A);
  wvc_varint(w, (u64)klen);
  wvc_bytes(w, s.name(f), klen);
  wvc_put(w, 0x12);
  wvc_varint(w, (u64)flb);
  for (i64 j = c.list_off[r]; j < c.list_off[r + 1]; ++j) {
    i64 fb = feature_body_size(c, c.sub_off[j], c.sub_off[j + 1]);
    wvc_put(w, 0x0A);
    wvc_varint(w, (u64)fb);
    wvc_feature_body(w, c, c.sub_off[j], c.sub_off[j + 1]);
  }
}

__device__ inline i64 emit_record_payload_wave(u8* o, const FieldColumn* cols,
                                               const SchemaView& s, int32_t fmt,
                                               i64 r) {
  i64 ctx_body = 0, fl_body = 0;
  for (int f = 0; f < s.nfields; ++f) {
    const FieldColumn& c = cols[f];
    if (!c.presence[r]) continue;
    if (!c.is_seq) {
      i64 e = features_entry_size(c, s, f, c.row_off[r], c.row_off[r + 1]);
      ctx_body += 1 + varint_size((u64)e) + e;
    } else {
      i64 e = feature_lists_entry_size(c, s, f, r);
      fl_body += 1 + varint_size((u64)e) + e;
    }
  }
  WaveCur w{o, 0};
  auto emit_ctx = [&]() {
    for (int f = 0; f < s.nfields; ++f) {
      const FieldColumn& c = cols[f];
      if (!c.presence[r] || c.is_seq) continue;
      i64 e = features_entry_size(c, s, f, c.row_off[r], c.row_off[r + 1]);
      wvc_put(w, 0x0A);
      wvc_varint(w, (u64)e);
      wvc_features_entry(w, c, s, f, c.row_off[r], c.row_off[r + 1]);
    }
  };
  auto emit_fl = [&]() {
    for (int f = 0; f < s.nfields; ++f) {
      const FieldColumn& c = cols[f];
      if (!c.presence[r] || !c.is_seq) continue;
      i64 e = feature_lists_entry_size(c, s, f, r);
      wvc_put(w, 0x0A);
      wvc_varint(w, (u64)e);
      wvc_feature_lists_entry(w, c, s, f, r);
    }
  };
  if (fmt == FMT_EXAMPLE) {
    wvc_put(w, 0x0A);
    wvc_varint(w, (u64)ctx_body);
    emit_ctx();
  } else {
    if (ctx_body) {
      wvc_put(w, 0x0A);
      wvc_varint(w, (u64)ctx_body);
      emit_ctx();
    }
    wvc_put(w, 0x12);
    wvc_varint(w, (u64)fl_body);
    emit_fl();
  }
  return w.pos;
}

__global__ void emit_records_wave_kernel(const FieldColumn* __restrict__ cols,
                                         const u8* __restrict__ schema_blob,
                                         int32_t fmt, i64 r0, i64 R,
                                         const i64* __restrict__ frame_off,
                                         u8* __restrict__ file,
                                         int32_t* __restrict__ err) {
  __shared__ uint32_t tab[8][256];
  stage_crc_tables(tab);
  SchemaView schema = schema_view(schema_blob);
  i64 wave = (blockIdx.x * (i64)blockDim.x + threadIdx.x) / 64;
  i64 nwaves = ((i64)gridDim.x * blockDim.x) / 64;
  int lane = threadIdx.x & 63;
  for (i64 r = r0 + wave; r < R; r += nwaves) {
    i64 payload = (frame_off[r + 1] - frame_off[r]) - kFrameOverhead;
    u8* o = file + frame_off[r] + 12;
    i64 emitted = emit_record_payload_wave(o, cols, schema, fmt, r);
    if (emitted != payload && lane == 0) set_err(err, ERR_OVERFLOW, r);
    __threadfence_block();
    u32 crc = crc32c_wave(o, payload, tab);
    if (lane == 0)
      write_frame_header_footer_crc(file, frame_off[r], payload, crc, tab);
  }
}

__global__ void frame_bytes_kernel(const u8* __restrict__ src,
                                   const i64* __restrict__ elem_off,
                                   const i64* __restrict__ frame_off, i64 R,
                                   u8* __restrict__ file) {
  __shared__ uint32_t tab[8][256];
  stage_crc_tables(tab);
  for (i64 r = blockIdx.x * (i64)blockDim.x + threadIdx.x; r < R;
       r += (i64)gridDim.x * blockDim.x) {
    i64 n = elem_off[r + 1] - elem_off[r];
    WriteCur w;
    wcur_init(w, file + frame_off[r] + 12, tab);
    wcur_bytes(w, src + elem_off[r], n);
    u32 crc = wcur_finish(w);
    write_frame_header_footer_crc(file, frame_off[r], n, crc, tab);
  }
}

__device__ inline u32 crc8b_reg(u64 w, const uint32_t (*tab)[256]) {
  w ^= 0xFFFFFFFFull;
  u32 c = tab[7][w & 0xFF] ^ tab[6][(w >> 8) & 0xFF] ^ tab[5][(w >> 16) & 0xFF] ^
          tab[4][(w >> 24) & 0xFF] ^ tab[3][(w >> 32) & 0xFF] ^
          tab[2][(w >> 40) & 0xFF] ^ tab[1][(w >> 48) & 0xFF] ^
          tab[0][(w >> 56) & 0xFF];
  return ~c;
}

constexpr int kPosPerLane = 16;

template <typename F>
__device__ inline void eval_frame_chunk(const u8* __restrict__ data,
                                        const u64* __restrict__ wdata, i64 N,
                                        i64 c, i64 pos_start, i64 pos_end,
                                        const uint32_t (*tab)[256], F&& f) {
  i64 p0 = c * kPosPerLane;
  i64 w0 = p0 >> 3;
  u64 w[4];
  if (p0 + 32 <= N) {
#pragma unroll
    for (int j = 0; j < 4; ++j) w[j] = wdata[w0 + j];
  } else {
#pragma unroll
    for (int j = 0; j < 4; ++j) {
      u64 v = 0;
      i64 boff = (w0 + j) * 8;
      for (int b = 0; b < 8 && boff + b < N; ++b)
        v |= (u64)data[boff + b] << (8 * b);
      w[j] = v;
    }
  }
#pragma unroll
  for (int k = 0; k < kPosPerLane; ++k) {
    i64 i = p0 + k;
    if (i + 16 > N || i >= pos_end) break;
    if (i < pos_start) continue;
    constexpr int _ppl = kPosPerLane;
    static_assert(_ppl == 16, "index math below assumes 16 positions");
    const int wi = k >> 3;
    const int sh = (k & 7) * 8;
    u64 len = (sh == 0) ? w[wi] : (w[wi] >> sh) | (w[wi + 1] << (64 - sh));
    if (len > (u64)(N - i) - 16) continue;
    const int wi2 = (k + 8) >> 3;
    const int sh2 = sh;
    u64 hi = (sh2 == 0) ? w[wi2]
                        : (w[wi2] >> sh2) | (w[wi2 + 1] << (64 - sh2));
    u32 want = (u32)hi;
    if (mask_crc(crc8b_reg(len, tab)) != want) continue;
    f(i, (i64)len);
  }
}

template <bool EMIT>
__global__ void frame_scan_pass_kernel(const u8* __restrict__ data, i64 N,
                                       i64 pos_start, i64 pos_end,
                                       i64 block_base,
                                       i64* __restrict__ block_data,
                                       i64* __restrict__ cand_pos,
                                       i64* __restrict__ cand_len) {
  __shared__ uint32_t tab[8][256];
  __shared__ unsigned int cnt[256];
  stage_crc_tables(tab);
  const u64* wdata = reinterpret_cast<const u64*>(data);
  i64 c_lo = pos_start / kPosPerLane;
  i64 c_hi = (pos_end + kPosPerLane - 1) / kPosPerLane;
  i64 c = c_lo + (i64)blockIdx.x * blockDim.x + threadIdx.x;
  unsigned int my = 0;
  if (c < c_hi)
    eval_frame_chunk(data, wdata, N, c, pos_start, pos_end, tab,
                     [&](i64, i64) { ++my; });
  cnt[threadIdx.x] = my;
  __syncthreads();
  if (!EMIT) {
    for (int off = blockDim.x / 2; off; off >>= 1) {
      if ((int)threadIdx.x < off) cnt[threadIdx.x] += cnt[threadIdx.x + off];
      __syncthreads();
    }
    if (threadIdx.x == 0) block_data[block_base + blockIdx.x] = (i64)cnt[0];
    return;
  }
  for (int off = 1; off < (int)blockDim.x; off <<= 1) {
    unsigned int v = (int)threadIdx.x >= off ? cnt[threadIdx.x - off] : 0;
    __syncthreads();
    cnt[threadIdx.x] += v;
    __syncthreads();
  }
  i64 slot = block_data[block_base + blockIdx.x] + (i64)(cnt[threadIdx.x] - my);
  if (c < c_hi)
    eval_frame_chunk(data, wdata, N, c, pos_start, pos_end, tab,
                     [&](i64 i, i64 len) {
                       cand_pos[slot] = i;
                       cand_len[slot] = len;
                       ++slot;
                     });
}

__global__ void frame_chain_kernel(const i64* __restrict__ pos,
                                   const i64* __restrict__ len, i64 C,
                                   const i64* __restrict__ carry_in,
                                   i64* __restrict__ carry_out,
                                   i64* __restrict__ off,
                                   i64* __restrict__ broken) {
  for (i64 k = blockIdx.x * (i64)blockDim.x + threadIdx.x; k < C;
       k += (i64)gridDim.x * blockDim.x) {
    i64 p = pos[k];
    i64 want = k == 0 ? *carry_in : pos[k - 1] + 16 + len[k - 1];
    if (p != want) *broken = 1;
    off[k] = p + 12;
    if (k == C - 1) *carry_out = p + 16 + len[k];
  }
}


struct InferSlot {
  unsigned long long hash;
  long long nameref;
  long long code;
};
static_assert(sizeof(InferSlot) == 24, "layout shared with Python [S,3] i64");

__device__ inline u64 fnv1a64(const u8* s, u64 n) {
  u64 h = 1469598103934665603ull;
  for (u64 i = 0; i < n; ++i) h = (h ^ s[i]) * 1099511628211ull;
  return h ? h : 1ull;
}

constexpr int kLdsInfer = 64;

struct LdsInferSlot {
  unsigned long long hash;
  long long nameref;
  unsigned int code;
};

__device__ inline bool lds_infer_merge(LdsInferSlot* ltab, u64 hash,
                                       long long nameref, int code) {
  int idx = (int)(hash % (u64)kLdsInfer);
  for (int probe = 0; probe < kLdsInfer; ++probe) {
    LdsInferSlot& s = ltab[idx];
    unsigned long long seen =
        atomicCAS(&s.hash, 0ull, (unsigned long long)hash);
    if (seen == 0ull) s.nameref = nameref;
    if (seen == 0ull || seen == hash) {
      atomicMax(&s.code, (unsigned int)code);
      return true;
    }
    idx = (idx + 1) % kLdsInfer;
  }
  return false;
}

__device__ inline bool infer_slot_merge(InferSlot* table, int lo, int half,
                                        u64 hash, long long nameref, int code) {
  int idx = lo + (int)(hash % (u64)half);
  for (int probe = 0; probe < half; ++probe) {
    InferSlot& s = table[idx];
    unsigned long long seen =
        atomicCAS(&s.hash, 0ull, (unsigned long long)hash);
    if (seen == 0ull) s.nameref = nameref;
    if (seen == 0ull || seen == hash) {
      atomicMax((unsigned long long*)&s.code, (unsigned long long)code);
      return true;
    }
    idx = (idx + 1 - lo) % half + lo;
  }
  return false;
}

__device__ inline int32_t infer_features_body_dev(const u8* data, const u8* p,
                                                  const u8* end, bool seq,
                                                  LdsInferSlot* ltab,
                                                  InferSlot* table, int nslots) {
  int half = nslots / 2;
  int lo = seq ? half : 0;
  while (p < end) {
    u64 tag;
    p = read_varint(p, end, &tag);
    if (!p) return ERR_BAD_VARINT;
    u32 fieldno = (u32)(tag >> 3), wt = (u32)(tag & 7);
    if (fieldno != 1 || wt != 2) {
      p = skip_field(p, end, wt);
      if (!p) return ERR_TRUNCATED;
      continue;
    }
    u64 entry_len;
    p = read_varint(p, end, &entry_len);
    if (!p || (u64)(end - p) < entry_len) return ERR_TRUNCATED;
    const u8* ep = p;
    const u8* ee = p + entry_len;
    p = ee;
    const u8* key = nullptr;
    u64 key_len = 0;
    const u8* val = nullptr;
    u64 val_len = 0;
    while (ep < ee) {
      u64 etag;
      ep = read_varint(ep, ee, &etag);
      if (!ep) return ERR_BAD_VARINT;
      u32 efn = (u32)(etag >> 3), ewt = (u32)(etag & 7);
      if (efn == 1 && ewt == 2) {
        ep = read_varint(ep, ee, &key_len);
        if (!ep || (u64)(ee - ep) < key_len) return ERR_TRUNCATED;
        key = ep;
        ep += key_len;
      } else if (efn == 2 && ewt == 2) {
        ep = read_varint(ep, ee, &val_len);
        if (!ep || (u64)(ee - ep) < val_len) return ERR_TRUNCATED;
        val = ep;
        ep += val_len;
      } else {
        ep = skip_field(ep, ee, ewt);
        if (!ep) return ERR_TRUNCATED;
      }
    }
    if (!key) continue;
    int code = 0;
    if (val) {
      if (!seq) {
        int32_t kf = 0;
        i64 nvals = 0, nbytes = 0;
        int32_t rc = scan_feature_body(val, val + val_len, -1, &kf, &nvals, &nbytes);
        if (rc != ERR_OK) return rc;
        if (kf != 0 && nvals > 0) code = (4 - kf) + (nvals > 1 ? 3 : 0);
      } else {
        const u8* lp = val;
        const u8* le = val + val_len;
        int kind_seen = 0;
        while (lp < le) {
          u64 ltag;
          lp = read_varint(lp, le, &ltag);
          if (!lp) return ERR_BAD_VARINT;
          u32 lfn = (u32)(ltag >> 3), lwt = (u32)(ltag & 7);
          if (lfn == 1 && lwt == 2) {
            u64 flen;
            lp = read_varint(lp, le, &flen);
            if (!lp || (u64)(le - lp) < flen) return ERR_TRUNCATED;
            int32_t kf = 0;
            i64 nvals = 0, nbytes = 0;
            int32_t rc = scan_feature_body(lp, lp + flen, -1, &kf, &nvals, &nbytes);
            if (rc != ERR_OK) return rc;
            if (kf) {
              int r = 4 - kf;
              kind_seen = kind_seen > r ? kind_seen : r;
            }
            lp += flen;
          } else {
            lp = skip_field(lp, le, lwt);
            if (!lp) return ERR_TRUNCATED;
          }
        }
        if (kind_seen) code = 6 + kind_seen;
      }
    }
    if (key_len > 0xFFFF) return ERR_NAME_TOO_LONG;
    long long nameref = ((long long)(key - data) << 16) | (long long)key_len;
    u64 hash = fnv1a64(key, key_len);
    if (!lds_infer_merge(ltab, hash, nameref, code) &&
        !infer_slot_merge(table, lo, half, hash, nameref, code))
      return ERR_OVERFLOW;
  }
  return ERR_OK;
}

__global__ void infer_codes_kernel(const u8* __restrict__ data,
                                   const i64* __restrict__ off,
                                   const i64* __restrict__ len, i64 R, int32_t fmt,
                                   InferSlot* __restrict__ table, int nslots,
                                   int32_t* __restrict__ err) {
  __shared__ LdsInferSlot lctx[kLdsInfer];
  __shared__ LdsInferSlot lseq[kLdsInfer];
  for (int i = threadIdx.x; i < kLdsInfer; i += blockDim.x) {
    lctx[i].hash = 0;
    lctx[i].code = 0;
    lseq[i].hash = 0;
    lseq[i].code = 0;
  }
  __syncthreads();
  for (i64 r = blockIdx.x * (i64)blockDim.x + threadIdx.x; r < R;
       r += (i64)gridDim.x * blockDim.x) {
    const u8* p = data + off[r];
    const u8* end = p + len[r];
    while (p < end) {
      u64 tag;
      const u8* np = read_varint(p, end, &tag);
      if (!np) {
        set_err(err, ERR_BAD_VARINT, r);
        break;
      }
      p = np;
      u32 fieldno = (u32)(tag >> 3), wt = (u32)(tag & 7);
      bool is_features = fieldno == 1;
      bool is_fl = (fmt == FMT_SEQUENCE && fieldno == 2);
      if ((is_features || is_fl) && wt == 2) {
        u64 blen;
        p = read_varint(p, end, &blen);
        if (!p || (u64)(end - p) < blen) {
          set_err(err, ERR_TRUNCATED, r);
          break;
        }
        int32_t rc = infer_features_body_dev(data, p, p + blen, is_fl,
                                             is_fl ? lseq : lctx, table, nslots);
        if (rc != ERR_OK) {
          set_err(err, rc, r);
          break;
        }
        p += blen;
      } else {
        p = skip_field(p, end, wt);
        if (!p) {
          set_err(err, ERR_TRUNCATED, r);
          break;
        }
      }
    }
  }
  __syncthreads();
  int half = nslots / 2;
  for (int i = threadIdx.x; i < kLdsInfer; i += blockDim.x) {
    if (lctx[i].hash &&
        !infer_slot_merge(table, 0, half, lctx[i].hash, lctx[i].nameref,
                          (int)lctx[i].code))
      err[0] = ERR_OVERFLOW;
    if (lseq[i].hash &&
        !infer_slot_merge(table, half, half, lseq[i].hash, lseq[i].nameref,
                          (int)lseq[i].code))
      err[0] = ERR_OVERFLOW;
  }
}

__global__ void gather_payloads_kernel(const u8* __restrict__ data,
                                       const i64* __restrict__ off,
                                       const i64* __restrict__ len,
                                       const i64* __restrict__ dst_off, i64 R,
                                       u8* __restrict__ out) {
  for (i64 r = blockIdx.x * (i64)blockDim.x + threadIdx.x; r < R;
       r += (i64)gridDim.x * blockDim.x) {
    const u8* s = data + off[r];
    u8* d = out + dst_off[r];
    i64 n = len[r];
    i64 i = 0;
    for (; i + 8 <= n; i += 8) {
      u64 w;
      __builtin_memcpy(&w, s + i, 8);
      __builtin_memcpy(d + i, &w, 8);
    }
    for (; i < n; ++i) d[i] = s[i];
  }
}


inline int grid_for(i64 n, i64 max_blocks = 0) {
  i64 blocks = (n + kBlock - 1) / kBlock;
  i64 cap = max_blocks > 0 && max_blocks < 8192 ? max_blocks : 8192;
  if (blocks > cap) blocks = cap;
  if (blocks < 1) blocks = 1;
  return (int)blocks;
}

void gpu_crc_verify(uintptr_t data, uintptr_t off, uintptr_t len, i64 R,
                    uintptr_t err_out, uintptr_t stream, i64 avg_bytes) {
  if (avg_bytes > kWaveRecordBytes) {
    hipLaunchKernelGGL(crc_verify_wave_kernel, dim3(grid_for(R * 64)),
                       dim3(kBlock), 0, (hipStream_t)stream, (const u8*)data,
                       (const i64*)off, (const i64*)len, R,
                       (unsigned long long*)err_out);
  } else {
    hipLaunchKernelGGL(crc_verify_kernel, dim3(grid_for(R)), dim3(kBlock), 0,
                       (hipStream_t)stream, (const u8*)data, (const i64*)off,
                       (const i64*)len, R, (unsigned long long*)err_out);
  }
  HIP_CHECK(hipGetLastError());
}

void gpu_scan_records(uintptr_t data, uintptr_t off, uintptr_t len, i64 R,
                      int32_t fmt, uintptr_t schema_blob, int F, uintptr_t stats,
                      uintptr_t err, uintptr_t crc_err, uintptr_t stream,
                      i64 avg_bytes, i64 rec_base, i64 max_blocks) {
  if (R <= 0) return;
  if (avg_bytes > kWaveRecordBytes) {
    hipLaunchKernelGGL(scan_records_wave_kernel,
                       dim3(grid_for(R * 64, max_blocks)), dim3(kBlock), 0,
                       (hipStream_t)stream, (const u8*)data, (const i64*)off,
                       (const i64*)len, R, fmt, (const u8*)schema_blob, F,
                       (FieldStat*)stats, (int32_t*)err,
                       (unsigned long long*)crc_err, rec_base);
  } else {
    hipLaunchKernelGGL(scan_records_kernel, dim3(grid_for(R, max_blocks)),
                       dim3(kBlock), 0, (hipStream_t)stream, (const u8*)data,
                       (const i64*)off, (const i64*)len, R, fmt,
                       (const u8*)schema_blob, F, (FieldStat*)stats,
                       (int32_t*)err, (unsigned long long*)crc_err, rec_base);
  }
  HIP_CHECK(hipGetLastError());
}

void gpu_extract_fields(uintptr_t data, i64 R, int F, uintptr_t stats,
                        py::list metas, uintptr_t meta_dev, uintptr_t err,
                        uintptr_t stream, i64 avg_bytes, i64 r0,
                        i64 max_blocks) {
  if (R <= 0 || F <= 0) return;
  std::vector<DevFieldDst> host_metas(F);
  for (int f = 0; f < F; ++f) {
    py::dict d = metas[f].cast<py::dict>();
    DevFieldDst& m = host_metas[f];
    m.kind = d["kind"].cast<int32_t>();
    m.is_seq = d["is_seq"].cast<int32_t>();
    m.i64_vals = (i64*)d["i64_vals"].cast<uintptr_t>();
    m.f32_vals = (float*)d["f32_vals"].cast<uintptr_t>();
    m.bytes_data = (u8*)d["bytes_data"].cast<uintptr_t>();
    m.elem_len = (i64*)d["elem_len"].cast<uintptr_t>();
    m.sub_count = (i64*)d["sub_count"].cast<uintptr_t>();
    m.val_base = (const i64*)d["val_base"].cast<uintptr_t>();
    m.byte_base = (const i64*)d["byte_base"].cast<uintptr_t>();
    m.list_base = (const i64*)d["list_base"].cast<uintptr_t>();
  }
  HIP_CHECK(hipMemcpyAsync((void*)meta_dev, host_metas.data(),
                           sizeof(DevFieldDst) * F, hipMemcpyHostToDevice,
                           (hipStream_t)stream));
  if (avg_bytes > kWaveRecordBytes) {
    hipLaunchKernelGGL(extract_fields_wave_kernel,
                       dim3(grid_for(R * F * 64, max_blocks)), dim3(kBlock), 0,
                       (hipStream_t)stream, (const u8*)data, R, F,
                       (const FieldStat*)stats, (const DevFieldDst*)meta_dev,
                       (int32_t*)err, r0);
  } else {
    hipLaunchKernelGGL(extract_fields_kernel,
                       dim3(grid_for(R * F, max_blocks)), dim3(kBlock), 0,
                       (hipStream_t)stream, (const u8*)data, R, F,
                       (const FieldStat*)stats, (const DevFieldDst*)meta_dev,
                       (int32_t*)err, r0);
  }
  HIP_CHECK(hipGetLastError());
}

size_t gpu_devcols_bytes(int F) { return sizeof(FieldColumn) * (size_t)F; }

void fill_devcols(py::list cols, std::vector<FieldColumn>& out) {
  int F = (int)cols.size();
  out.resize(F);
  for (int f = 0; f < F; ++f) {
    py::dict d = cols[f].cast<py::dict>();
    FieldColumn& c = out[f];
    c.kind = d["kind"].cast<int32_t>();
    c.is_seq = d["is_seq"].cast<int32_t>();
    c.presence = (const u8*)d["presence"].cast<uintptr_t>();
    c.row_off = (const i64*)d["row_off"].cast<uintptr_t>();
    c.list_off = (const i64*)d["list_off"].cast<uintptr_t>();
    c.sub_off = (const i64*)d["sub_off"].cast<uintptr_t>();
    c.elem_off = (const i64*)d["elem_off"].cast<uintptr_t>();
    c.bytes_data = (const u8*)d["values_bytes"].cast<uintptr_t>();
    c.i64_vals = (const i64*)d["values_i64"].cast<uintptr_t>();
    c.f32_vals = (const float*)d["values_f32"].cast<uintptr_t>();
  }
}

void gpu_size_records(py::list cols, uintptr_t cols_dev, uintptr_t schema_blob,
                      int32_t fmt, i64 R, uintptr_t psize, uintptr_t stream) {
  static thread_local std::vector<FieldColumn> host_cols;
  fill_devcols(cols, host_cols);
  HIP_CHECK(hipMemcpyAsync((void*)cols_dev, host_cols.data(),
                           sizeof(FieldColumn) * host_cols.size(),
                           hipMemcpyHostToDevice, (hipStream_t)stream));
  hipLaunchKernelGGL(size_records_kernel, dim3(grid_for(R)), dim3(kBlock), 0,
                     (hipStream_t)stream, (const FieldColumn*)cols_dev,
                     (const u8*)schema_blob, fmt, R, (i64*)psize);
  HIP_CHECK(hipGetLastError());
}

void gpu_emit_records(uintptr_t cols_dev, uintptr_t schema_blob, int32_t fmt,
                      i64 r0, i64 R, uintptr_t frame_off, uintptr_t file,
                      uintptr_t err, uintptr_t stream, i64 avg_bytes) {
  if (avg_bytes > kWaveRecordBytes) {
    hipLaunchKernelGGL(emit_records_wave_kernel, dim3(grid_for((R - r0) * 64)),
                       dim3(kBlock), 0, (hipStream_t)stream,
                       (const FieldColumn*)cols_dev, (const u8*)schema_blob,
                       fmt, r0, R, (const i64*)frame_off, (u8*)file,
                       (int32_t*)err);
  } else {
    hipLaunchKernelGGL(emit_records_kernel, dim3(grid_for(R - r0)),
                       dim3(kBlock), 0, (hipStream_t)stream,
                       (const FieldColumn*)cols_dev, (const u8*)schema_blob,
                       fmt, r0, R, (const i64*)frame_off, (u8*)file,
                       (int32_t*)err);
  }
  HIP_CHECK(hipGetLastError());
}

void gpu_frame_bytes(uintptr_t src, uintptr_t elem_off, uintptr_t frame_off, i64 R,
                     uintptr_t file, uintptr_t stream, i64 avg_bytes) {
  if (avg_bytes > kWaveRecordBytes) {
    hipLaunchKernelGGL(frame_bytes_wave_kernel, dim3(grid_for(R * 64)),
                       dim3(kBlock), 0, (hipStream_t)stream, (const u8*)src,
                       (const i64*)elem_off, (const i64*)frame_off, R,
                       (u8*)file);
  } else {
    hipLaunchKernelGGL(frame_bytes_kernel, dim3(grid_for(R)), dim3(kBlock), 0,
                       (hipStream_t)stream, (const u8*)src, (const i64*)elem_off,
                       (const i64*)frame_off, R, (u8*)file);
  }
  HIP_CHECK(hipGetLastError());
}

i64 gpu_frame_scan_blocks(i64 pos_start, i64 pos_end) {
  i64 c_lo = pos_start / kPosPerLane;
  i64 c_hi = (pos_end + kPosPerLane - 1) / kPosPerLane;
  i64 n = c_hi - c_lo;
  return (n + kBlock - 1) / kBlock;
}

void gpu_frame_scan_count(uintptr_t data, i64 N, i64 pos_start, i64 pos_end,
                          i64 block_base, uintptr_t block_counts,
                          uintptr_t stream) {
  i64 B = gpu_frame_scan_blocks(pos_start, pos_end);
  if (B <= 0) return;
  hipLaunchKernelGGL(frame_scan_pass_kernel<false>, dim3((uint32_t)B),
                     dim3(kBlock), 0, (hipStream_t)stream, (const u8*)data, N,
                     pos_start, pos_end, block_base, (i64*)block_counts,
                     nullptr, nullptr);
  HIP_CHECK(hipGetLastError());
}

void gpu_frame_scan_emit(uintptr_t data, i64 N, i64 pos_start, i64 pos_end,
                         i64 block_base, uintptr_t block_off,
                         uintptr_t cand_pos, uintptr_t cand_len,
                         uintptr_t stream) {
  i64 B = gpu_frame_scan_blocks(pos_start, pos_end);
  if (B <= 0) return;
  hipLaunchKernelGGL(frame_scan_pass_kernel<true>, dim3((uint32_t)B),
                     dim3(kBlock), 0, (hipStream_t)stream, (const u8*)data, N,
                     pos_start, pos_end, block_base, (i64*)block_off,
                     (i64*)cand_pos, (i64*)cand_len);
  HIP_CHECK(hipGetLastError());
}

void gpu_frame_chain(uintptr_t pos, uintptr_t len, i64 C, uintptr_t carry_in,
                     uintptr_t carry_out, uintptr_t off, uintptr_t broken,
                     uintptr_t stream) {
  if (C <= 0) return;
  hipLaunchKernelGGL(frame_chain_kernel, dim3(grid_for(C)), dim3(kBlock), 0,
                     (hipStream_t)stream, (const i64*)pos, (const i64*)len, C,
                     (const i64*)carry_in, (i64*)carry_out, (i64*)off,
                     (i64*)broken);
  HIP_CHECK(hipGetLastError());
}

void gpu_infer_codes(uintptr_t data, uintptr_t off, uintptr_t len, i64 R,
                     int32_t fmt, uintptr_t table, int nslots, uintptr_t err,
                     uintptr_t stream) {
  hipLaunchKernelGGL(infer_codes_kernel, dim3(grid_for(R)), dim3(kBlock), 0,
                     (hipStream_t)stream, (const u8*)data, (const i64*)off,
                     (const i64*)len, R, fmt, (InferSlot*)table, nslots,
                     (int32_t*)err);
  HIP_CHECK(hipGetLastError());
}

void gpu_gather_payloads(uintptr_t data, uintptr_t off, uintptr_t len,
                         uintptr_t dst_off, i64 R, uintptr_t out,
                         uintptr_t stream, i64 avg_bytes) {
  if (avg_bytes > kWaveRecordBytes) {
    hipLaunchKernelGGL(gather_payloads_wave_kernel, dim3(grid_for(R * 64)),
                       dim3(kBlock), 0, (hipStream_t)stream, (const u8*)data,
                       (const i64*)off, (const i64*)len, (const i64*)dst_off,
                       R, (u8*)out);
  } else {
    hipLaunchKernelGGL(gather_payloads_kernel, dim3(grid_for(R)), dim3(kBlock),
                       0, (hipStream_t)stream, (const u8*)data,
                       (const i64*)off, (const i64*)len, (const i64*)dst_off,
                       R, (u8*)out);
  }
  HIP_CHECK(hipGetLastError());
}


struct StridedLoadI64 {
  const i64* p;
  i64 stride;
  __host__ __device__ i64 operator()(i64 i) const { return p[i * stride]; }
};

size_t gpu_scan_temp_bytes(i64 n) {
  size_t bytes = 0;
  auto it = rocprim::make_transform_iterator(
      rocprim::make_counting_iterator<i64>(0), StridedLoadI64{nullptr, 1});
  (void)rocprim::inclusive_scan(nullptr, bytes, it, (i64*)nullptr, (size_t)n,
                                rocprim::plus<i64>());
  return bytes;
}


struct Seg3 {
  i64 v0, v1, v2;
  u32 flag;
};

struct Seg3Combine {
  __host__ __device__ Seg3 operator()(const Seg3& a, const Seg3& b) const {
    if (b.flag) return b;
    return Seg3{a.v0 + b.v0, a.v1 + b.v1, a.v2 + b.v2, a.flag};
  }
};

struct Seg3Load {
  const i64* stats;
  i64 n;
  int F;
  i64 r0;
  i64 stride;
  const i64* b0;
  const i64* b1;
  const i64* b2;
  __host__ __device__ Seg3 operator()(i64 idx) const {
    i64 f = idx / n;
    i64 q = idx - f * n;
    const i64* st = stats + ((r0 + q) * F + f) * 6;
    if (q != 0) return Seg3{st[2], st[3], st[4], 0u};
    i64 at = f * stride + r0;
    return Seg3{st[2] + b0[at], st[3] + b1[at], st[4] + b2[at], 1u};
  }
};

struct Seg3OutRef {
  i64* o0;
  i64* o1;
  i64* o2;
  __host__ __device__ Seg3OutRef& operator=(const Seg3& v) {
    *o0 = v.v0;
    *o1 = v.v1;
    *o2 = v.v2;
    return *this;
  }
};

struct Seg3OutIt {
  using value_type = Seg3;
  using reference = Seg3OutRef;
  using pointer = Seg3OutRef*;
  using difference_type = i64;
  using iterator_category = std::random_access_iterator_tag;
  i64* b0;
  i64* b1;
  i64* b2;
  i64 n;
  i64 r0;
  i64 stride;
  i64 pos;
  __host__ __device__ Seg3OutRef operator*() const { return (*this)[0]; }
  __host__ __device__ Seg3OutRef operator[](i64 k) const {
    i64 idx = pos + k;
    i64 f = idx / n;
    i64 q = idx - f * n;
    i64 at = f * stride + r0 + q + 1;
    return Seg3OutRef{b0 + at, b1 + at, b2 + at};
  }
  __host__ __device__ Seg3OutIt operator+(i64 k) const {
    return Seg3OutIt{b0, b1, b2, n, r0, stride, pos + k};
  }
  __host__ __device__ Seg3OutIt& operator+=(i64 k) {
    pos += k;
    return *this;
  }
  __host__ __device__ Seg3OutIt& operator++() {
    ++pos;
    return *this;
  }
};

size_t gpu_stat_scan_temp_bytes(i64 R, int F) {
  size_t bytes = 0;
  auto in = rocprim::make_transform_iterator(
      rocprim::make_counting_iterator<i64>(0),
      Seg3Load{nullptr, R, F, 0, R + 1, nullptr, nullptr, nullptr});
  Seg3OutIt out{nullptr, nullptr, nullptr, R, 0, R + 1, 0};
  (void)rocprim::inclusive_scan(nullptr, bytes, in, out, (size_t)(R * F),
                                Seg3Combine());
  return bytes;
}

void gpu_stat_scans(uintptr_t temp, size_t temp_bytes, uintptr_t stats, i64 R,
                    int F, uintptr_t val_base, uintptr_t byte_base,
                    uintptr_t list_base, uintptr_t stream, i64 r0, i64 r1,
                    i64 stride) {
  auto s = (hipStream_t)stream;
  if (r1 < 0) r1 = R;
  if (stride <= 0) stride = R + 1;
  if (r0 < 0 || r1 > R || r1 >= stride)
    throw std::runtime_error("gpu_stat_scans: range outside the planes");
  i64 n = r1 - r0;
  if (n <= 0 || F <= 0) return;
  auto in = rocprim::make_transform_iterator(
      rocprim::make_counting_iterator<i64>(0),
      Seg3Load{(const i64*)stats, n, F, r0, stride, (const i64*)val_base,
               (const i64*)byte_base, (const i64*)list_base});
  Seg3OutIt out{(i64*)val_base, (i64*)byte_base, (i64*)list_base, n, r0,
                stride, 0};
  size_t tb = temp_bytes;
  HIP_CHECK(rocprim::inclusive_scan((void*)temp, tb, in, out,
                                    (size_t)(n * F), Seg3Combine(), s));
}

void gpu_excl_sum_strided(uintptr_t temp, size_t temp_bytes, uintptr_t in,
                          i64 stride, uintptr_t out, i64 n, uintptr_t stream) {
  auto s = (hipStream_t)stream;
  HIP_CHECK(hipMemsetAsync((void*)out, 0, sizeof(i64), s));
  if (n <= 0) return;
  auto it = rocprim::make_transform_iterator(
      rocprim::make_counting_iterator<i64>(0), StridedLoadI64{(const i64*)in, stride});
  size_t tb = temp_bytes;
  hipError_t e = rocprim::inclusive_scan((void*)temp, tb, it, (i64*)out + 1,
                                         (size_t)n, rocprim::plus<i64>(), s);
  HIP_CHECK(e);
}


struct MappedFile {
  void* ptr = nullptr;
  size_t n = 0;
  dev_t dev = 0;
  ino_t ino = 0;
  bool pinned = false;
  bool writable = false;
};

std::map<std::string, MappedFile> g_mmap_cache;
std::mutex g_mmap_mu;
size_t g_mmap_bytes = 0;
constexpr size_t kMmapCacheCap = 4ull << 30;

void drop_mapping_locked(const std::string& key) {
  auto it = g_mmap_cache.find(key);
  if (it == g_mmap_cache.end()) return;
  if (it->second.pinned) {
    (void)hipDeviceSynchronize();
    (void)hipHostUnregister(it->second.ptr);
  }
  munmap(it->second.ptr, it->second.n);
  g_mmap_bytes -= it->second.n;
  g_mmap_cache.erase(it);
}

void sweep_stale_locked() {
  for (auto it = g_mmap_cache.begin(); it != g_mmap_cache.end();) {
    struct stat st {};
    bool live = stat(it->first.c_str(), &st) == 0 &&
                st.st_dev == it->second.dev && st.st_ino == it->second.ino &&
                (size_t)st.st_size >= it->second.n;
    if (live) {
      ++it;
    } else {
      auto key = it->first;
      ++it;
      drop_mapping_locked(key);
    }
  }
}

py::tuple file_mmap_pinned(const std::string& path, i64 n, bool writable) {
  if (n <= 0) return py::make_tuple((uintptr_t)0, true);
  std::lock_guard<std::mutex> lk(g_mmap_mu);
  sweep_stale_locked();
  int flags = writable ? (O_RDWR | O_CREAT) : O_RDWR;
  int fd = ::open(path.c_str(), flags, 0644);
  bool rdonly = false;
  if (fd < 0 && !writable) {
    fd = ::open(path.c_str(), O_RDONLY);
    rdonly = true;
  }
  if (fd < 0)
    throw std::runtime_error("open failed: " + path + ": " + strerror(errno));
  struct stat st {};
  if (fstat(fd, &st) != 0) {
    ::close(fd);
    throw std::runtime_error("stat failed: " + path);
  }
  auto it = g_mmap_cache.find(path);
  if (it != g_mmap_cache.end()) {
    MappedFile& m = it->second;
    if (m.dev == st.st_dev && m.ino == st.st_ino && m.n == (size_t)n &&
        st.st_size >= (off_t)n && (m.writable || !writable)) {
      ::close(fd);
      return py::make_tuple((uintptr_t)m.ptr, m.pinned);
    }
    drop_mapping_locked(path);
  }
  if (writable && st.st_size != (off_t)n && ftruncate(fd, (off_t)n) != 0) {
    int e = errno;
    ::close(fd);
    throw std::runtime_error("ftruncate failed: " + path + ": " + strerror(e));
  }
  if (!writable && st.st_size < (off_t)n) {
    ::close(fd);
    throw std::runtime_error("short file: " + path);
  }
  while (g_mmap_bytes + (size_t)n > kMmapCacheCap && !g_mmap_cache.empty())
    drop_mapping_locked(g_mmap_cache.begin()->first);
  int prot = PROT_READ | ((writable || !rdonly) ? PROT_WRITE : 0);
  void* p = mmap(nullptr, (size_t)n, prot, MAP_SHARED, fd, 0);
  ::close(fd);
  if (p == MAP_FAILED)
    throw std::runtime_error("mmap failed: " + path + ": " + strerror(errno));
  bool pinned = hipHostRegister(p, (size_t)n, hipHostRegisterDefault) == hipSuccess;
  if (!pinned) (void)hipGetLastError();
  MappedFile m{p, (size_t)n, st.st_dev, st.st_ino, pinned,
               writable || !rdonly};
  g_mmap_cache[path] = m;
  g_mmap_bytes += (size_t)n;
  return py::make_tuple((uintptr_t)p, pinned);
}

void file_mmap_drop(const std::string& path) {
  std::lock_guard<std::mutex> lk(g_mmap_mu);
  drop_mapping_locked(path);
}

void file_mmap_sync(const std::string& path) {
  std::lock_guard<std::mutex> lk(g_mmap_mu);
  auto it = g_mmap_cache.find(path);
  if (it != g_mmap_cache.end() && it->second.ptr) {
    if (msync(it->second.ptr, it->second.n, MS_SYNC) != 0)
      throw std::runtime_error("msync failed: " + path + ": " +
                               strerror(errno));
  }
  int fd = ::open(path.c_str(), O_RDONLY);
  if (fd >= 0) {
    (void)fsync(fd);
    ::close(fd);
  }
}


void gpu_memcpy_d2h(uintptr_t dst, uintptr_t src, i64 n, uintptr_t stream) {
  HIP_CHECK(hipMemcpyAsync((void*)dst, (const void*)src, (size_t)n,
                           hipMemcpyDeviceToHost, (hipStream_t)stream));
}

void gpu_memcpy_h2d(uintptr_t dst, uintptr_t src, i64 n, uintptr_t stream) {
  HIP_CHECK(hipMemcpyAsync((void*)dst, (const void*)src, (size_t)n,
                           hipMemcpyHostToDevice, (hipStream_t)stream));
}

}

void register_gpu(py::module_& m) {
  m.def("gpu_device_count", []() {
    int n = 0;
    hipError_t e = hipGetDeviceCount(&n);
    return (e == hipSuccess) ? n : -static_cast<int>(e);
  });
  m.def("gpu_crc_verify", &gpu_crc_verify, py::arg("data"), py::arg("off"),
        py::arg("len"), py::arg("R"), py::arg("err_out"), py::arg("stream"),
        py::arg("avg_bytes") = 0);
  m.def("gpu_scan_records", &gpu_scan_records, py::arg("data"), py::arg("off"),
        py::arg("len"), py::arg("R"), py::arg("fmt"), py::arg("schema_blob"),
        py::arg("F"), py::arg("stats"), py::arg("err"), py::arg("crc_err"),
        py::arg("stream"), py::arg("avg_bytes") = 0, py::arg("rec_base") = 0,
        py::arg("max_blocks") = 0);
  m.def("gpu_extract_fields", &gpu_extract_fields, py::arg("data"),
        py::arg("R"), py::arg("F"), py::arg("stats"), py::arg("metas"),
        py::arg("meta_dev"), py::arg("err"), py::arg("stream"),
        py::arg("avg_bytes") = 0, py::arg("r0") = 0,
        py::arg("max_blocks") = 0);
  m.def("gpu_size_records", &gpu_size_records);
  m.def("gpu_emit_records", &gpu_emit_records, py::arg("cols_dev"),
        py::arg("schema_blob"), py::arg("fmt"), py::arg("r0"), py::arg("R"),
        py::arg("frame_off"), py::arg("file"), py::arg("err"),
        py::arg("stream"), py::arg("avg_bytes") = 0);
  m.def("gpu_frame_bytes", &gpu_frame_bytes, py::arg("src"),
        py::arg("elem_off"), py::arg("frame_off"), py::arg("R"),
        py::arg("file"), py::arg("stream"), py::arg("avg_bytes") = 0);
  m.def("gpu_frame_scan_blocks", &gpu_frame_scan_blocks);
  m.def("gpu_frame_scan_count", &gpu_frame_scan_count);
  m.def("gpu_frame_scan_emit", &gpu_frame_scan_emit);
  m.def("gpu_frame_chain", &gpu_frame_chain);
  m.def("gpu_gather_payloads", &gpu_gather_payloads, py::arg("data"),
        py::arg("off"), py::arg("len"), py::arg("dst_off"), py::arg("R"),
        py::arg("out"), py::arg("stream"), py::arg("avg_bytes") = 0);
  m.def("gpu_infer_codes", &gpu_infer_codes);
  m.def("gpu_scan_temp_bytes", &gpu_scan_temp_bytes);
  m.def("gpu_stat_scan_temp_bytes", &gpu_stat_scan_temp_bytes);
  m.def("gpu_stat_scans", &gpu_stat_scans, py::arg("temp"),
        py::arg("temp_bytes"), py::arg("stats"), py::arg("R"), py::arg("F"),
        py::arg("val_base"), py::arg("byte_base"), py::arg("list_base"),
        py::arg("stream"), py::arg("r0") = 0, py::arg("r1") = -1,
        py::arg("stride") = 0);
  m.def("gpu_excl_sum_strided", &gpu_excl_sum_strided);
  m.def("file_mmap_pinned", &file_mmap_pinned, py::arg("path"), py::arg("n"),
        py::arg("writable"));
  m.def("file_mmap_drop", &file_mmap_drop);
  m.def("file_mmap_sync", &file_mmap_sync);
  m.def("gpu_memcpy_d2h", &gpu_memcpy_d2h);
  m.def("gpu_memcpy_h2d", &gpu_memcpy_h2d);
  m.def("gpu_devcols_bytes", &gpu_devcols_bytes);
  m.def("gpu_devmeta_bytes", []() { return sizeof(DevFieldDst); });
  m.def("gpu_fieldstat_words", []() { return sizeof(FieldStat) / 8; });
}
```

### spark_tfrecord_amd/columnar.py

```python

from __future__ import annotations

import decimal
import struct
from dataclasses import dataclass, field
from typing import Any, List, Optional, Sequence

import numpy as np

from .schema import (
    ArrayType,
    BinaryType,
    DataType,
    DecimalType,
    DoubleType,
    FloatType,
    IntegerType,
    KIND_BYTES,
    KIND_FLOAT,
    KIND_INT64,
    LongType,
    NullType,
    StringType,
    StructField,
    StructType,
    is_sequence_field,
    wire_kind_of,
)

__all__ = ["WireColumn", "RecordBatch", "schema_blob", "column_from_values",
           "column_to_pylist", "wire_to_native_dict", "native_dict_to_wire"]


def schema_blob(schema: StructType) -> bytes:
    names = b""
    descs = b""
    nf = 0
    for f in schema.fields:
        if isinstance(f.dataType, NullType):
            continue
        nb = f.name.encode("utf-8")
        kind = wire_kind_of(f.dataType)
        seq = 1 if is_sequence_field(f.dataType) else 0
        descs += struct.pack("<iiii", kind, seq, len(names), len(nb))
        names += nb
        nf += 1
    return struct.pack("<i", nf) + descs + names


def wire_fields(schema: StructType) -> List[StructField]:
    return [f for f in schema.fields if not isinstance(f.dataType, NullType)]


@dataclass
class WireColumn:

    kind: int
    is_seq: bool
    presence: Any
    row_off: Any
    values: Any
    elem_off: Optional[Any] = None
    list_off: Optional[Any] = None
    sub_off: Optional[Any] = None

    @property
    def num_rows(self) -> int:
        return len(self.presence)


@dataclass
class RecordBatch:

    schema: StructType
    columns: List[WireColumn]
    num_rows: int

    def column(self, name: str) -> WireColumn:
        for f, c in zip(wire_fields(self.schema), self.columns):
            if f.name == name:
                return c
        raise KeyError(name)



def wire_to_native_dict(col: WireColumn) -> dict:
    d = {
        "presence": np.ascontiguousarray(col.presence, dtype=np.uint8),
        "row_off": np.ascontiguousarray(col.row_off, dtype=np.int64),
    }
    if col.kind == KIND_INT64:
        d["values_i64"] = np.ascontiguousarray(col.values, dtype=np.int64)
    elif col.kind == KIND_FLOAT:
        d["values_f32"] = np.ascontiguousarray(col.values, dtype=np.float32)
    else:
        d["values_bytes"] = np.ascontiguousarray(col.values, dtype=np.uint8)
        d["elem_off"] = np.ascontiguousarray(col.elem_off, dtype=np.int64)
    if col.is_seq:
        d["list_off"] = np.ascontiguousarray(col.list_off, dtype=np.int64)
        d["sub_off"] = np.ascontiguousarray(col.sub_off, dtype=np.int64)
    return d


def native_dict_to_wire(d: dict, kind: int, is_seq: bool) -> WireColumn:
    elem_off = None
    if "elem_len" in d:
        elem_off = np.zeros(len(d["elem_len"]) + 1, dtype=np.int64)
        np.cumsum(d["elem_len"], out=elem_off[1:])
    sub_off = None
    if "sub_count" in d:
        sub_off = np.zeros(len(d["sub_count"]) + 1, dtype=np.int64)
        np.cumsum(d["sub_count"], out=sub_off[1:])
    return WireColumn(
        kind=kind,
        is_seq=is_seq,
        presence=d["presence"],
        row_off=d["row_off"],
        values=d["values"],
        elem_off=elem_off,
        list_off=d.get("list_off"),
        sub_off=sub_off,
    )



def _to_f32(v, name: str):
    if isinstance(v, decimal.Decimal):
        return np.float32(float(v))
    return np.float32(v)


def _to_i64(v, name: str):
    if isinstance(v, (bool, np.bool_)):
        raise TypeError(f"Cannot convert field '{name}': boolean is not supported")
    return np.int64(v)


def _to_bytes(v, name: str) -> bytes:
    if isinstance(v, str):
        return v.encode("utf-8")
    if isinstance(v, (bytes, bytearray, memoryview)):
        return bytes(v)
    if isinstance(v, np.ndarray) and v.dtype == np.uint8:
        return v.tobytes()
    raise TypeError(f"Cannot convert field '{name}' value {type(v).__name__} to bytes")


def _validate_serializable(dt: DataType, name: str):
    if isinstance(dt, NullType):
        return
    if isinstance(dt, ArrayType):
        inner = dt.elementType
        if isinstance(inner, ArrayType):
            if isinstance(inner.elementType, (ArrayType, StructType, NullType)):
                raise TypeError(
                    f"Cannot convert field '{name}': arrays nested deeper than 2 are not supported")
            wire_kind_of(inner.elementType)
            return
        if isinstance(inner, (StructType, NullType)):
            raise TypeError(f"Cannot convert field '{name}' to a TFRecord feature")
        wire_kind_of(inner)
        return
    if isinstance(dt, StructType):
        raise TypeError(f"Cannot convert field '{name}': nested structs are not supported")
    wire_kind_of(dt)


def _is_null(v) -> bool:
    if v is None:
        return True
    if isinstance(v, float) and v != v:
        return True
    return False


def column_from_values(values: Sequence, dt: DataType, nullable: bool,
                       name: str) -> WireColumn:
    _validate_serializable(dt, name)
    kind = wire_kind_of(dt)
    seq = is_sequence_field(dt)
    R = len(values)

    if not seq and not isinstance(dt, ArrayType) and isinstance(values, np.ndarray) \
            and values.dtype != object:
        if kind == KIND_INT64 and np.issubdtype(values.dtype, np.integer):
            vals = values.astype(np.int64, copy=False)
            return WireColumn(kind, False, np.ones(R, np.uint8),
                              np.arange(R + 1, dtype=np.int64), vals)
        if kind == KIND_FLOAT and np.issubdtype(values.dtype, np.floating):
            vals = values.astype(np.float32, copy=False)
            return WireColumn(kind, False, np.ones(R, np.uint8),
                              np.arange(R + 1, dtype=np.int64), vals)

    presence = np.ones(R, np.uint8)
    row_counts = np.zeros(R, np.int64)
    flat: List[Any] = []
    list_counts = np.zeros(R, np.int64) if seq else None
    sub_counts: List[int] = []

    for r, v in enumerate(values):
        if _is_null(v):
            if not nullable:
                raise ValueError(
                    f"null value in non-nullable field '{name}' (row {r})")
            presence[r] = 0
            continue
        if seq:
            n = 0
            nls = 0
            for sub in v:
                if sub is None:
                    raise ValueError(
                        f"null inner array in field '{name}' (row {r})")
                sub = list(sub)
                sub_counts.append(len(sub))
                flat.extend(sub)
                n += len(sub)
                nls += 1
            row_counts[r] = n
            list_counts[r] = nls
        elif isinstance(dt, ArrayType):
            v = list(v)
            flat.extend(v)
            row_counts[r] = len(v)
        else:
            flat.append(v)
            row_counts[r] = 1

    row_off = np.zeros(R + 1, np.int64)
    np.cumsum(row_counts, out=row_off[1:])

    elem_off = None
    if kind == KIND_INT64:
        vals = np.fromiter((_to_i64(v, name) for v in flat), np.int64, len(flat))
    elif kind == KIND_FLOAT:
        vals = np.fromiter((_to_f32(v, name) for v in flat), np.float32, len(flat))
    else:
        bs = [_to_bytes(v, name) for v in flat]
        elem_off = np.zeros(len(bs) + 1, np.int64)
        np.cumsum(np.fromiter((len(b) for b in bs), np.int64, len(bs)),
                  out=elem_off[1:])
        vals = np.frombuffer(b"".join(bs), np.uint8).copy() if bs else np.zeros(0, np.uint8)

    list_off = sub_off = None
    if seq:
        list_off = np.zeros(R + 1, np.int64)
        np.cumsum(list_counts, out=list_off[1:])
        sub_off = np.zeros(len(sub_counts) + 1, np.int64)
        np.cumsum(np.asarray(sub_counts, np.int64), out=sub_off[1:])

    return WireColumn(kind, seq, presence, row_off, vals, elem_off, list_off, sub_off)



def _scalar_convert(dt: DataType, raw):
    if isinstance(dt, IntegerType):
        return int(np.int32(raw))
    if isinstance(dt, LongType):
        return int(raw)
    if isinstance(dt, FloatType):
        return float(np.float32(raw))
    if isinstance(dt, DoubleType):
        return float(raw)
    if isinstance(dt, DecimalType):
        return decimal.Decimal(repr(float(np.float32(raw))))
    raise TypeError(f"Unsupported scalar type {dt!r}")


def _bytes_convert(dt: DataType, b: bytes):
    if isinstance(dt, StringType):
        return b.decode("utf-8", errors="replace")
    if isinstance(dt, BinaryType):
        return b
    raise TypeError(f"Unsupported bytes type {dt!r}")


def _check_kind(col: WireColumn, dt: DataType, name: str):
    expect = wire_kind_of(dt)
    if col.kind != expect:
        raise RuntimeError(
            f"Feature '{name}' kind does not match requested type {dt.simple_string()}")


def column_to_pylist(col: WireColumn, dt: DataType, nullable: bool,
                     name: str) -> List[Any]:
    if isinstance(dt, NullType):
        return [None] * col.num_rows
    _check_kind(col, dt, name)
    R = col.num_rows
    presence = np.asarray(col.presence)
    row_off = np.asarray(col.row_off)
    out: List[Any] = [None] * R

    def elem(vi: int):
        if col.kind == KIND_BYTES:
            b0, b1 = int(col.elem_off[vi]), int(col.elem_off[vi + 1])
            return bytes(np.asarray(col.values[b0:b1]).tobytes())
        return col.values[vi]

    seq = is_sequence_field(dt)
    if seq != col.is_seq:
        raise RuntimeError(f"Feature '{name}' dimensionality does not match schema")

    for r in range(R):
        if not presence[r]:
            if not nullable:
                raise ValueError(f"Feature '{name}' is required but missing (row {r})")
            out[r] = None
            continue
        if seq:
            inner_dt = dt.elementType.elementType
            lists = []
            for j in range(int(col.list_off[r]), int(col.list_off[r + 1])):
                v0, v1 = int(col.sub_off[j]), int(col.sub_off[j + 1])
                if col.kind == KIND_BYTES:
                    lists.append([_bytes_convert(inner_dt, elem(v)) for v in range(v0, v1)])
                else:
                    lists.append([_scalar_convert(inner_dt, col.values[v]) for v in range(v0, v1)])
            out[r] = lists
        elif isinstance(dt, ArrayType):
            v0, v1 = int(row_off[r]), int(row_off[r + 1])
            inner_dt = dt.elementType
            if col.kind == KIND_BYTES:
                out[r] = [_bytes_convert(inner_dt, elem(v)) for v in range(v0, v1)]
            else:
                out[r] = [_scalar_convert(inner_dt, col.values[v]) for v in range(v0, v1)]
        else:
            v0, v1 = int(row_off[r]), int(row_off[r + 1])
            if v1 == v0:
                raise ValueError(
                    f"Feature '{name}' is present but empty; cannot read scalar (row {r})")
            if col.kind == KIND_BYTES:
                out[r] = _bytes_convert(dt, elem(v0))
            else:
                out[r] = _scalar_convert(dt, col.values[v0])
    return out
```

### spark_tfrecord_amd/engine/gpu.py

```python

from __future__ import annotations

import os
from typing import List, Optional

import numpy as np
import torch

from .. import _native
from . import stream_plan
from ..columnar import RecordBatch, WireColumn, schema_blob, wire_fields
from ..schema import KIND_BYTES, KIND_FLOAT, KIND_INT64, StructType, is_sequence_field, wire_kind_of

FMT = {"Example": _native.FMT_EXAMPLE, "SequenceExample": _native.FMT_SEQUENCE}

_U64_MAX = 0xFFFFFFFFFFFFFFFF


def _stream() -> int:
    return torch.cuda.current_stream().cuda_stream


def _dev(x, dtype, device="cuda") -> torch.Tensor:
    if isinstance(x, torch.Tensor):
        return x.to(device=device, dtype=dtype).contiguous()
    arr = np.ascontiguousarray(x)
    import warnings

    with warnings.catch_warnings():
        warnings.simplefilter("ignore", UserWarning)
        return torch.as_tensor(arr, dtype=dtype).to(device)


def check_native():
    if not getattr(_native, "HAS_GPU_KERNELS", False):
        raise RuntimeError("_native was built without HIP kernels; rebuild "
                           "with build_native.py before using the GPU engine")



import threading as _threading

_pinned_tls = _threading.local()


def pinned_buffer(tag: str, nbytes: int) -> torch.Tensor:
    pool = getattr(_pinned_tls, "pool", None)
    if pool is None:
        pool = _pinned_tls.pool = {}
    buf = pool.get(tag)
    if buf is None or buf.numel() < nbytes:
        cap = max(nbytes, int((buf.numel() if buf is not None else 1 << 20) * 1.5))
        buf = torch.empty(cap, dtype=torch.uint8, pin_memory=True)
        pool[tag] = buf
    return buf


_CHUNK = 64 << 20
_READ_SLICE = int(os.environ.get("TFREC_READ_SLICE", 32 << 20))
_SPLIT_SLICES = os.environ.get("TFREC_READ_SPLIT", "1") != "0"
_WRITE_SLICES = int(os.environ.get("TFREC_WRITE_SLICES", 8))
_STREAM_DECODE = os.environ.get("TFREC_STREAM_DECODE", "1") != "0"
_STREAM_HEADROOM = float(os.environ.get("TFREC_STREAM_HEADROOM", 1.125))
_STREAM_MAX_BLOCKS = int(os.environ.get("TFREC_STREAM_MAX_BLOCKS", 0))
_STREAM_EXTRACT = os.environ.get("TFREC_STREAM_EXTRACT", "1") != "0"
_SYNC_WRITES = os.environ.get("TFREC_SYNC", "1") != "0"


def read_file_to_device(path: str, device="cuda") -> torch.Tensor:
    import os as _os

    n = _os.path.getsize(path)
    dev_t = torch.empty(max(n, 1), dtype=torch.uint8, device=device)[:n]
    if n:
        ptr, pinned = _native.file_mmap_pinned(path, n, False)
        if pinned:
            _multi_dma(dev_t.data_ptr(), ptr, n, _native.gpu_memcpy_h2d,
                       after_main=True)
            return dev_t
    return _read_file_staged(path, dev_t)


_copy_streams: Optional[list] = None


def _dma_streams() -> list:
    global _copy_streams
    if _copy_streams is None:
        _copy_streams = [torch.cuda.Stream() for _ in range(2)]
    return _copy_streams


def _multi_dma(dst: int, src: int, n: int, fn, after_main: bool):
    streams = _dma_streams()
    main = torch.cuda.current_stream()
    k = min(len(streams), max(1, n // (16 << 20)))
    span = (n + k - 1) // k
    for i in range(k):
        o = i * span
        m = min(span, n - o)
        s = streams[i]
        s.wait_stream(main)
        fn(dst + o, src + o, m, s.cuda_stream)
    if after_main:
        for i in range(k):
            main.wait_stream(streams[i])
    else:
        for i in range(k):
            streams[i].synchronize()


def _read_file_staged(path: str, dev: torch.Tensor) -> torch.Tensor:
    import os as _os

    n = dev.numel()
    buf = pinned_buffer("fread", min(n, 2 * _CHUNK) or 1)
    ev = [torch.cuda.Event(), torch.cuda.Event()]
    fd = _os.open(path, _os.O_RDONLY)
    try:
        pos = 0
        which = 0
        while pos < n:
            m = min(_CHUNK, n - pos)
            ev[which].synchronize()
            _native.pread_parallel(fd, buf.data_ptr() + which * _CHUNK, m, pos)
            dev[pos:pos + m].copy_(buf[which * _CHUNK:which * _CHUNK + m],
                                   non_blocking=True)
            ev[which].record()
            pos += m
            which ^= 1 if n > _CHUNK else 0
    finally:
        _os.close(fd)
    return dev


def device_to_file(img: torch.Tensor, path: str):
    import os as _os

    n = img.numel()
    if n == 0:
        open(path, "wb").close()
        return
    ptr, pinned = _native.file_mmap_pinned(path, n, True)
    if pinned:
        _multi_dma(ptr, img.data_ptr(), n, _native.gpu_memcpy_d2h,
                   after_main=False)
        if _SYNC_WRITES:
            _native.file_mmap_sync(path)
        return
    _write_file_staged(img, path)


def _write_file_staged(img: torch.Tensor, path: str):
    import os as _os

    n = img.numel()
    buf = pinned_buffer("fwrite", min(n, 2 * _CHUNK) or 1)
    ev = [torch.cuda.Event(), torch.cuda.Event()]
    fd = _os.open(path, _os.O_RDWR | _os.O_CREAT, 0o644)
    try:
        pos = 0
        which = 0
        m0 = min(_CHUNK, n)
        if n:
            buf[0:m0].copy_(img[0:m0], non_blocking=True)
            ev[0].record()
        while pos < n:
            m = min(_CHUNK, n - pos)
            nxt = pos + m
            nwhich = which ^ (1 if n > _CHUNK else 0)
            if nxt < n:
                m2 = min(_CHUNK, n - nxt)
                buf[nwhich * _CHUNK:nwhich * _CHUNK + m2].copy_(
                    img[nxt:nxt + m2], non_blocking=True)
                ev[nwhich].record()
            ev[which].synchronize()
            _native.pwrite_parallel(fd, buf.data_ptr() + which * _CHUNK, m, pos)
            pos = nxt
            which = nwhich
        _os.ftruncate(fd, n)
        if _SYNC_WRITES:
            _os.fsync(fd)
    finally:
        _os.close(fd)



_scan_ws = {}


def _scan_workspace(n: int, device) -> torch.Tensor:
    key = (device.index if hasattr(device, "index") else 0)
    need = _native.gpu_scan_temp_bytes(max(n, 1))
    ws = _scan_ws.get(key)
    if ws is None or ws.numel() < need:
        ws = torch.empty(int(need * 2), dtype=torch.uint8, device=device)
        _scan_ws[key] = ws
    return ws


def _excl_sum_into(out_ptr: int, in_ptr: int, stride: int, n: int, device):
    ws = _scan_workspace(n, device)
    _native.gpu_excl_sum_strided(ws.data_ptr(), ws.numel(), in_ptr, stride,
                                 out_ptr, n, _stream())


def _stat_scan_workspace(R: int, F: int, device) -> torch.Tensor:
    key = ("stat", device.index if hasattr(device, "index") else 0)
    need = _native.gpu_stat_scan_temp_bytes(R, F)
    ws = _scan_ws.get(key)
    if ws is None or ws.numel() < need:
        ws = torch.empty(int(need * 2) or 1, dtype=torch.uint8, device=device)
        _scan_ws[key] = ws
    return ws


def excl_sum(t: torch.Tensor) -> torch.Tensor:
    n = t.numel()
    out = torch.empty(n + 1, dtype=torch.int64, device=t.device)
    _excl_sum_into(out.data_ptr(), t.data_ptr(), 1, n, t.device)
    return out


def device_to_bytes(img: torch.Tensor) -> bytes:
    n = img.numel()
    buf = pinned_buffer("d2h", n)
    buf[:n].copy_(img, non_blocking=True)
    torch.cuda.synchronize()
    return buf.numpy()[:n].tobytes()


def device_to_pinned_view(img: torch.Tensor, tag: str = "d2h_img") -> np.ndarray:
    n = img.numel()
    buf = pinned_buffer(tag, n)
    buf[:n].copy_(img, non_blocking=True)
    torch.cuda.synchronize()
    return buf.numpy()[:n]



def scan_frames_device(data: torch.Tensor):
    check_native()
    N = data.numel()
    device = data.device
    if N == 0:
        z = torch.zeros(0, dtype=torch.int64, device=device)
        return z, z.clone()
    B = _native.gpu_frame_scan_blocks(0, N)
    block_counts = torch.empty(B, dtype=torch.int64, device=device)
    _native.gpu_frame_scan_count(data.data_ptr(), N, 0, N, 0,
                                 block_counts.data_ptr(), _stream())
    off, lens, _ = _emit_and_chain(data, [(0, N)], block_counts, N)
    return off, lens


def _emit_and_chain(data, ranges, block_counts, N):
    device = data.device
    block_off = excl_sum(block_counts)
    C = int(block_off[-1].item())
    if C == 0:
        raise RuntimeError("corrupt TFRecord: no valid frame header found")
    pos = torch.empty(C, dtype=torch.int64, device=device)
    lens = torch.empty(C, dtype=torch.int64, device=device)
    base = 0
    for s, e in ranges:
        _native.gpu_frame_scan_emit(data.data_ptr(), N, s, e, base,
                                    block_off.data_ptr(), pos.data_ptr(),
                                    lens.data_ptr(), _stream())
        base += _native.gpu_frame_scan_blocks(s, e)
    expect_next = pos + 16 + lens
    ok = bool(((pos[0] == 0) & (expect_next[-1] == N)
               & (expect_next[:-1] == pos[1:]).all()).item())
    if not ok:
        pos_h = pos.cpu().numpy()
        len_h = lens.cpu().numpy()
        import numpy as _np

        keep = []
        cur = 0
        idx = 0
        pmap = {int(p): i for i, p in enumerate(pos_h)}
        while cur < N:
            i = pmap.get(cur)
            if i is None:
                raise RuntimeError(
                    f"corrupt TFRecord: broken frame chain at offset {cur}")
            keep.append(i)
            cur = int(pos_h[i] + 16 + len_h[i])
        sel = torch.as_tensor(_np.asarray(keep, _np.int64), device=device)
        pos = pos[sel]
        lens = lens[sel]
    return pos + 12, lens, ok



def crc_verify_device(data: torch.Tensor, off: torch.Tensor, lens: torch.Tensor,
                      avg_bytes: int = 0):
    R = off.numel()
    if R == 0:
        return
    if not avg_bytes:
        avg_bytes = max(0, (data.numel() // R) - 16)
    err = torch.full((1,), -1, dtype=torch.int64, device=data.device)
    _native.gpu_crc_verify(data.data_ptr(), off.data_ptr(), lens.data_ptr(), R,
                           err.data_ptr(), _stream(), avg_bytes)
    bad = int(err.item())
    if bad != -1:
        raise RuntimeError(
            f"corrupt TFRecord: bad CRC in record {bad - 1 if bad > 0 else bad}")


def decode_device(data: torch.Tensor, off: torch.Tensor, lens: torch.Tensor,
                  schema: StructType, record_type: str,
                  verify_crc: bool = True) -> RecordBatch:
    check_native()
    device = data.device
    R = off.numel()
    fields = wire_fields(schema)
    F = len(fields)
    if verify_crc and record_type == "ByteArray":
        crc_verify_device(data, off, lens)

    if record_type == "ByteArray":
        dst_off = excl_sum(lens.contiguous())
        total = int(dst_off[-1].item())
        out = torch.empty(total, dtype=torch.uint8, device=device)
        if R:
            _native.gpu_gather_payloads(data.data_ptr(), off.data_ptr(),
                                        lens.data_ptr(), dst_off.data_ptr(), R,
                                        out.data_ptr(), _stream(), total // R)
        col = WireColumn(kind=KIND_BYTES, is_seq=False,
                         presence=torch.ones(R, dtype=torch.uint8, device=device),
                         row_off=torch.arange(R + 1, dtype=torch.int64, device=device),
                         values=out, elem_off=dst_off)
        return RecordBatch(schema, [col], R)

    if F == 0 or R == 0:
        cols = [WireColumn(wire_kind_of(f.dataType), is_sequence_field(f.dataType),
                           torch.zeros(R, dtype=torch.uint8, device=device),
                           torch.zeros(R + 1, dtype=torch.int64, device=device),
                           torch.zeros(0, dtype=torch.int64, device=device))
                for f in fields]
        return RecordBatch(schema, cols, R)

    blob = _schema_blob_device(schema, device)
    stats = torch.empty((R, F, 6), dtype=torch.int64, device=device)
    err = torch.zeros(2, dtype=torch.int32, device=device)
    crc_err = None
    fuse_crc = verify_crc
    if fuse_crc:
        crc_err = torch.full((1,), -1, dtype=torch.int64, device=device)
    avg_bytes = max(0, (data.numel() // R) - 16) if R else 0
    _native.gpu_scan_records(data.data_ptr(), off.data_ptr(), lens.data_ptr(),
                             R, FMT[record_type], blob.data_ptr(), F,
                             stats.data_ptr(), err.data_ptr(),
                             crc_err.data_ptr() if fuse_crc else 0,
                             _stream(), avg_bytes)

    val_base = torch.empty((F, R + 1), dtype=torch.int64, device=device)
    byte_base = torch.empty((F, R + 1), dtype=torch.int64, device=device)
    list_base = torch.empty((F, R + 1), dtype=torch.int64, device=device)
    val_base[:, 0] = 0
    byte_base[:, 0] = 0
    list_base[:, 0] = 0
    ws = _stat_scan_workspace(R, F, device)
    _native.gpu_stat_scans(ws.data_ptr(), ws.numel(), stats.data_ptr(), R, F,
                           val_base.data_ptr(), byte_base.data_ptr(),
                           list_base.data_ptr(), _stream())
    totals = torch.stack([val_base[:, -1], byte_base[:, -1], list_base[:, -1]])
    totals_h = totals.cpu()
    _raise_scan_errors(int(crc_err.item()) if fuse_crc else -1,
                       int(err[0].item()), int(err[1].item()))
    cols = _extract_columns(data, R, fields, stats, val_base, byte_base,
                            list_base, totals_h, err, avg_bytes)
    if int(err[0].item()) != 0:
        _raise_extract_error(int(err[0].item()), int(err[1].item()))
    return RecordBatch(schema, cols, R)


_schema_blobs = {}


def _schema_blob_device(schema: StructType, device) -> torch.Tensor:
    raw = bytes(schema_blob(schema))
    key = (raw, str(torch.device(device)))
    blob = _schema_blobs.get(key)
    if blob is None:
        if len(_schema_blobs) >= 64:
            _schema_blobs.clear()
        blob = torch.frombuffer(bytearray(raw), dtype=torch.uint8).to(device)
        _schema_blobs[key] = blob
    return blob


def _raise_scan_errors(crc_bad: int, rc: int, rec1: int):
    if crc_bad != -1:
        raise RuntimeError(f"corrupt TFRecord: bad CRC in record {crc_bad - 1}")
    if rc != 0:
        rec = rec1 - 1
        where = f" in record {rec}" if rec >= 0 else ""
        raise RuntimeError(f"TFRecord decode failed{where} (native error "
                           f"{rc}; kind mismatch or malformed record)")


def _raise_extract_error(rc: int, rec1: int):
    rec = rec1 - 1
    where = f" (record {rec})" if rec >= 0 else ""
    raise RuntimeError(f"TFRecord decode failed in value extraction"
                       f"{where} (native error {rc})")


def _extract_columns(data, R, fields, stats, val_base, byte_base, list_base,
                     totals_h, err, avg_bytes) -> List[WireColumn]:
    device = data.device
    F = len(fields)
    metas = []
    outs = []
    for i, f in enumerate(fields):
        kind = wire_kind_of(f.dataType)
        seq = is_sequence_field(f.dataType)
        nv = int(totals_h[0][i])
        nb = int(totals_h[1][i])
        nl = int(totals_h[2][i])
        o = {"kind": kind, "seq": seq}
        o["i64_vals"] = torch.empty(nv if kind == KIND_INT64 else 0,
                                    dtype=torch.int64, device=device)
        o["f32_vals"] = torch.empty(nv if kind == KIND_FLOAT else 0,
                                    dtype=torch.float32, device=device)
        o["bytes_data"] = torch.empty(nb, dtype=torch.uint8, device=device)
        o["elem_len"] = torch.empty(nv if kind == KIND_BYTES else 0,
                                    dtype=torch.int64, device=device)
        o["sub_count"] = torch.empty(nl, dtype=torch.int64, device=device)
        outs.append(o)
        metas.append({
            "kind": kind, "is_seq": 1 if seq else 0,
            "i64_vals": o["i64_vals"].data_ptr(),
            "f32_vals": o["f32_vals"].data_ptr(),
            "bytes_data": o["bytes_data"].data_ptr(),
            "elem_len": o["elem_len"].data_ptr(),
            "sub_count": o["sub_count"].data_ptr(),
            "val_base": val_base[i].data_ptr(),
            "byte_base": byte_base[i].data_ptr(),
            "list_base": list_base[i].data_ptr() if seq else 0,
        })

    meta_dev = torch.empty(F * _native.gpu_devmeta_bytes(), dtype=torch.uint8,
                           device=device)
    _native.gpu_extract_fields(data.data_ptr(), R, F, stats.data_ptr(), metas,
                               meta_dev.data_ptr(), err.data_ptr(), _stream(),
                               avg_bytes)

    cols: List[WireColumn] = []
    for i, (f, o) in enumerate(zip(fields, outs)):
        kind = o["kind"]
        seq = o["seq"]
        presence = (stats[:, i, 0] >= 0).to(torch.uint8)
        elem_off = None
        if kind == KIND_BYTES:
            elem_off = excl_sum(o["elem_len"])
        sub_off = None
        if seq:
            sub_off = excl_sum(o["sub_count"])
        values = (o["i64_vals"] if kind == KIND_INT64 else
                  o["f32_vals"] if kind == KIND_FLOAT else o["bytes_data"])
        cols.append(WireColumn(kind, seq, presence, val_base[i], values,
                               elem_off, list_base[i] if seq else None, sub_off))
    return cols


def decode_buffer_device(data_np: np.ndarray, schema: StructType, record_type: str,
                         verify_crc: bool = True, device="cuda") -> RecordBatch:
    data_np = np.ascontiguousarray(data_np, np.uint8)
    n = data_np.size
    stage = pinned_buffer("h2d", n)
    stage.numpy()[:n] = data_np
    data = torch.empty(n, dtype=torch.uint8, device=device)
    data.copy_(stage[:n], non_blocking=True)
    off, lens = scan_frames_device(data)
    return decode_device(data, off, lens, schema, record_type, verify_crc)


def read_file_to_batch(path: str, schema: StructType, record_type: str,
                       verify_crc: bool = True, device="cuda") -> RecordBatch:
    return read_file_to_batch_pipelined(path, schema, record_type, verify_crc,
                                        device)



def _col_ptrs(col: WireColumn) -> dict:
    def p(t):
        return t.data_ptr() if isinstance(t, torch.Tensor) and t.numel() else 0

    return {
        "kind": col.kind, "is_seq": 1 if col.is_seq else 0,
        "presence": p(col.presence), "row_off": p(col.row_off),
        "list_off": p(col.list_off) if col.list_off is not None else 0,
        "sub_off": p(col.sub_off) if col.sub_off is not None else 0,
        "elem_off": p(col.elem_off) if col.elem_off is not None else 0,
        "values_bytes": p(col.values) if col.kind == KIND_BYTES else 0,
        "values_i64": p(col.values) if col.kind == KIND_INT64 else 0,
        "values_f32": p(col.values) if col.kind == KIND_FLOAT else 0,
    }


def _check_emit_err(err: torch.Tensor):
    if int(err[0].item()) != 0:
        rec = int(err[1].item()) - 1
        where = f" in record {rec}" if rec >= 0 else ""
        raise RuntimeError(f"TFRecord encode failed: size/emit mismatch{where}")


def encode_device(batch: RecordBatch, record_type: str) -> torch.Tensor:
    check_native()
    R = batch.num_rows
    device = batch.columns[0].presence.device if batch.columns else torch.device("cuda")
    if record_type == "ByteArray":
        col = batch.columns[0]
        lens = col.elem_off[1:] - col.elem_off[:-1]
        frame_off = excl_sum((lens + 16).contiguous())
        total = int(frame_off[-1].item())
        file = torch.empty(total, dtype=torch.uint8, device=device)
        if R:
            _native.gpu_frame_bytes(col.values.data_ptr(), col.elem_off.data_ptr(),
                                    frame_off.data_ptr(), R, file.data_ptr(),
                                    _stream(), (total // R) - 16)
        return file

    blob = torch.frombuffer(bytearray(schema_blob(batch.schema)),
                            dtype=torch.uint8).to(device)
    col_dicts = [_col_ptrs(c) for c in batch.columns]
    cols_dev = torch.empty(_native.gpu_devcols_bytes(len(col_dicts)),
                           dtype=torch.uint8, device=device)
    psize = torch.empty(R, dtype=torch.int64, device=device)
    _native.gpu_size_records(col_dicts, cols_dev.data_ptr(), blob.data_ptr(),
                             FMT[record_type], R, psize.data_ptr(), _stream())
    frame_off = excl_sum(psize)
    total = int(frame_off[-1].item())
    file = torch.empty(total, dtype=torch.uint8, device=device)
    err = torch.zeros(2, dtype=torch.int32, device=device)
    _native.gpu_emit_records(cols_dev.data_ptr(), blob.data_ptr(),
                             FMT[record_type], 0, R, frame_off.data_ptr(),
                             file.data_ptr(), err.data_ptr(), _stream(),
                             total // max(R, 1))
    _check_emit_err(err)
    return file


def write_batch_to_file(batch: RecordBatch, path: str,
                        record_type: str = "Example",
                        slices: Optional[int] = None) -> int:
    check_native()
    R = batch.num_rows
    if record_type == "ByteArray" or R == 0:
        img = encode_device(batch, record_type)
        device_to_file(img, path)
        return img.numel()
    device = batch.columns[0].presence.device
    blob = torch.frombuffer(bytearray(schema_blob(batch.schema)),
                            dtype=torch.uint8).to(device)
    col_dicts = [_col_ptrs(c) for c in batch.columns]
    cols_dev = torch.empty(_native.gpu_devcols_bytes(len(col_dicts)),
                           dtype=torch.uint8, device=device)
    psize = torch.empty(R, dtype=torch.int64, device=device)
    _native.gpu_size_records(col_dicts, cols_dev.data_ptr(), blob.data_ptr(),
                             FMT[record_type], R, psize.data_ptr(), _stream())
    frame_off = excl_sum(psize)
    S = max(1, min(slices if slices is not None else _WRITE_SLICES, R))
    ridx = [R * s // S for s in range(S + 1)]
    bounds = frame_off[ridx].cpu()
    total = int(bounds[-1])
    file = torch.empty(total, dtype=torch.uint8, device=device)
    err = torch.zeros(2, dtype=torch.int32, device=device)
    ptr, pinned = _native.file_mmap_pinned(path, total, True)
    if not pinned:
        _native.gpu_emit_records(cols_dev.data_ptr(), blob.data_ptr(),
                                 FMT[record_type], 0, R, frame_off.data_ptr(),
                                 file.data_ptr(), err.data_ptr(), _stream(),
                                 total // R)
        _check_emit_err(err)
        _write_file_staged(file, path)
        return total
    main = torch.cuda.current_stream()
    streams = _dma_streams()
    for s in range(S):
        _native.gpu_emit_records(cols_dev.data_ptr(), blob.data_ptr(),
                                 FMT[record_type], ridx[s], ridx[s + 1],
                                 frame_off.data_ptr(), file.data_ptr(),
                                 err.data_ptr(), _stream(), total // R)
        b0, b1 = int(bounds[s]), int(bounds[s + 1])
        if b1 > b0:
            w = streams[s % len(streams)]
            w.wait_stream(main)
            _native.gpu_memcpy_d2h(ptr + b0, file.data_ptr() + b0, b1 - b0,
                                   w.cuda_stream)
    for w in streams:
        w.synchronize()
    if _SYNC_WRITES:
        _native.file_mmap_sync(path)
    _check_emit_err(err)
    return total


last_read = {}


def read_file_to_batch_pipelined(path: str, schema: StructType, record_type: str,
                                 verify_crc: bool = True,
                                 device="cuda") -> RecordBatch:
    import os as _os

    check_native()
    n = _os.path.getsize(path)
    if n == 0:
        z = torch.zeros(0, dtype=torch.int64, device=device)
        return decode_device(torch.zeros(0, dtype=torch.uint8, device=device),
                             z, z.clone(), schema, record_type, verify_crc)
    ptr, pinned = _native.file_mmap_pinned(path, n, False)
    if not pinned:
        data = _read_file_staged(path, torch.empty(n, dtype=torch.uint8,
                                                   device=device))
        off, lens = scan_frames_device(data)
        return decode_device(data, off, lens, schema, record_type, verify_crc)
    data = torch.empty(n, dtype=torch.uint8, device=device)
    device = data.device
    plan = stream_plan.plan_slices(n, _READ_SLICE)
    S = len(plan)
    nblocks = [int(_native.gpu_frame_scan_blocks(p.scan_lo, p.scan_hi))
               if p.scan_hi > p.scan_lo else 0 for p in plan]
    block_counts = torch.empty(max(sum(nblocks), 1), dtype=torch.int64,
                               device=device)
    main = torch.cuda.current_stream()
    streams = _dma_streams()
    events = []
    for st in streams:
        st.wait_stream(main)
    for s, p in enumerate(plan):
        half = (p.b1 - p.b0) // 2 if _SPLIT_SLICES and len(streams) > 1 else 0
        parts = ([(p.b0, p.b0 + half, 0), (p.b0 + half, p.b1, 1)] if half
                 else [(p.b0, p.b1, s % len(streams))])
        evs = []
        for lo, hi, k in parts:
            st = streams[k]
            _native.gpu_memcpy_h2d(data.data_ptr() + lo, ptr + lo, hi - lo,
                                   st.cuda_stream)
            ev = torch.cuda.Event()
            ev.record(st)
            evs.append(ev)
        events.append(evs)
    data.record_stream(streams[0])
    if len(streams) > 1:
        data.record_stream(streams[1])

    fields = wire_fields(schema)
    F = len(fields)
    streaming = _STREAM_DECODE
    last_read.update(path="streamed", slices=S, regrows=0)
    do_scan = streaming and record_type != "ByteArray" and F > 0
    fuse_crc = verify_crc
    vals = None
    if streaming:
        status = torch.zeros(_ST_CARRY + 1 + S, dtype=torch.int64,
                             device=device)
        status[_ST_CRC] = -1
        sp = status.data_ptr()
        err = status[_ST_ERR:_ST_ERR + 1].view(torch.int32)
        xerr = status[_ST_XERR:_ST_XERR + 1].view(torch.int32)
        rows = _StreamRows(n, F if do_scan else 0, device)
        if do_scan:
            blob = _schema_blob_device(schema, device)
            vals = _StreamValues(fields, n, device) if _STREAM_EXTRACT else None
            meta_dev = torch.empty(F * _native.gpu_devmeta_bytes(),
                                   dtype=torch.uint8, device=device)

    base = 0
    C = 0
    nchain = 0
    r_done = 0
    pending = None
    avg_bytes = None
    for s, p in enumerate(plan):
        for ev in events[s]:
            main.wait_event(ev)
        last = s == S - 1
        nb = nblocks[s]
        if nb:
            _native.gpu_frame_scan_count(data.data_ptr(), n, p.scan_lo,
                                         p.scan_hi, base,
                                         block_counts.data_ptr(), _stream())
        if not streaming:
            base += nb
            continue
        if nb:
            block_off = excl_sum(block_counts[base:base + nb])
            c_s = int(block_off[-1].item())
            base += nb
            if c_s:
                rows.reserve(C + c_s, C, r_done, p.scan_hi)
                _native.gpu_frame_scan_emit(
                    data.data_ptr(), n, p.scan_lo, p.scan_hi, 0,
                    block_off.data_ptr(), rows.pos.data_ptr() + C * 8,
                    rows.lens.data_ptr() + C * 8, _stream())
                _native.gpu_frame_chain(
                    rows.pos.data_ptr() + C * 8, rows.lens.data_ptr() + C * 8,
                    c_s, sp + (_ST_CARRY + nchain) * 8,
                    sp + (_ST_CARRY + 1 + nchain) * 8,
                    rows.off.data_ptr() + C * 8, sp + _ST_BROKEN * 8, _stream())
                nchain += 1
                C += c_s
        if not do_scan or C == r_done:
            continue
        if last:
            avail = C
            end = n
        else:
            st_h = status.cpu()
            if int(st_h[_ST_BROKEN]) != 0:
                streaming = do_scan = False
                continue
            end = int(st_h[_ST_CARRY + nchain])
            avail = stream_plan.arrived_records(C, end, p.b1)
            if avail < C:
                end = p.b1
        if avail > r_done:
            if avg_bytes is None:
                avg_bytes = max(0, end // avail - 16)
            _native.gpu_scan_records(
                data.data_ptr(), rows.off.data_ptr() + r_done * 8,
                rows.lens.data_ptr() + r_done * 8, avail - r_done,
                FMT[record_type], blob.data_ptr(), F,
                rows.stats.data_ptr() + r_done * F * 48, err.data_ptr(),
                sp + _ST_CRC * 8 if fuse_crc else 0, _stream(), avg_bytes,
                rec_base=r_done, max_blocks=0 if last else _STREAM_MAX_BLOCKS)
            if vals is not None:
                rows.scan_stats(r_done, avail)
                if last:
                    pending = (r_done, avail)
                elif vals.ok:
                    h = torch.cat(rows.totals(avail)
                                  + [status[:_ST_CARRY]]).cpu()
                    pair = h[3 * F + _ST_ERR:3 * F + _ST_ERR + 1].view(torch.int32)
                    if int(h[3 * F + _ST_CRC]) != -1 or int(pair[0]) != 0:
                        vals.ok = False
                    else:
                        vals.extract(data, rows, r_done, avail,
                                     h[:3 * F].view(3, F), end, meta_dev,
                                     xerr, avg_bytes,
                                     _STREAM_MAX_BLOCKS)
            r_done = avail

    def unstreamed():
        last_read["path"] = "fallback" if _STREAM_DECODE else "unstreamed"
        ranges = [(p.scan_lo, p.scan_hi) for p in plan if p.scan_hi > p.scan_lo]
        off, lens, _ = _emit_and_chain(data, ranges, block_counts, n)
        return decode_device(data, off, lens, schema, record_type, verify_crc)

    if not streaming or C == 0:
        return unstreamed()
    R = C
    if not do_scan:
        st_h = status.cpu()
        if int(st_h[_ST_BROKEN]) != 0 or int(st_h[_ST_CARRY + nchain]) != n:
            return unstreamed()
        return decode_device(data, rows.off[:R], rows.lens[:R], schema,
                             record_type, verify_crc)

    stats = rows.stats[:R]
    if vals is None:
        rows.scan_stats(0, R)
    packed = torch.cat(rows.totals(R) + [status]).cpu()
    st_h = packed[3 * F:]
    if int(st_h[_ST_BROKEN]) != 0 or int(st_h[_ST_CARRY + nchain]) != n:
        return unstreamed()
    pair = st_h[_ST_ERR:_ST_ERR + 1].view(torch.int32)
    _raise_scan_errors(int(st_h[_ST_CRC]) if fuse_crc else -1, int(pair[0]),
                       int(pair[1]))
    totals_h = packed[:3 * F].view(3, F)
    val_base, byte_base, list_base = rows.planes
    if vals is None:
        cols = _extract_columns(data, R, fields, stats,
                                val_base[:, :R + 1], byte_base[:, :R + 1],
                                list_base[:, :R + 1], totals_h, xerr,
                                max(0, n // R - 16))
    else:
        if not vals.ok:
            raise RuntimeError("streamed decode: scan error lost")
        if pending is not None:
            vals.extract(data, rows, pending[0], pending[1], totals_h, n,
                         meta_dev, xerr, avg_bytes, 0)
        cols = vals.columns(stats, val_base, list_base, R)
    err_h = xerr.cpu()
    if int(err_h[0]) != 0:
        _raise_extract_error(int(err_h[0]), int(err_h[1]))
    return RecordBatch(schema, cols, R)


_ST_BROKEN, _ST_CRC, _ST_ERR, _ST_XERR, _ST_CARRY = 0, 1, 2, 3, 4


class _StreamRows:

    def __init__(self, total_bytes: int, F: int, device):
        self.total_bytes = total_bytes
        self.F = F
        self.device = device
        self.cap = 0
        self.pos = self.lens = self.off = self.stats = None
        self.planes = None

    def _alloc(self, cap: int):
        i64 = dict(dtype=torch.int64, device=self.device)
        planes = None
        if self.F:
            planes = [torch.empty((self.F, cap + 1), **i64) for _ in range(3)]
            for t in planes:
                t[:, 0] = 0
        return (torch.empty(cap, **i64), torch.empty(cap, **i64),
                torch.empty(cap, **i64),
                torch.empty((cap, self.F, 6), **i64) if self.F else None,
                planes)

    def scan_stats(self, r0: int, r1: int):
        ws = _stat_scan_workspace(r1 - r0, self.F, self.device)
        v, b, l = self.planes
        _native.gpu_stat_scans(ws.data_ptr(), ws.numel(),
                               self.stats.data_ptr(), r1, self.F, v.data_ptr(),
                               b.data_ptr(), l.data_ptr(), _stream(), r0=r0,
                               r1=r1, stride=self.cap + 1)

    def totals(self, r: int) -> list:
        return [t[:, r] for t in self.planes]

    def reserve(self, need: int, n_cand: int, n_scanned: int, bytes_seen: int):
        cap = stream_plan.grown_capacity(self.cap, need, bytes_seen,
                                         self.total_bytes, _STREAM_HEADROOM)
        if cap == self.cap:
            return
        pos, lens, off, stats, planes = self._alloc(cap)
        if n_cand:
            pos[:n_cand].copy_(self.pos[:n_cand])
            lens[:n_cand].copy_(self.lens[:n_cand])
            off[:n_cand].copy_(self.off[:n_cand])
        if n_scanned and stats is not None:
            stats[:n_scanned].copy_(self.stats[:n_scanned])
            for new, old in zip(planes, self.planes):
                new[:, :n_scanned + 1].copy_(old[:, :n_scanned + 1])
        self.pos, self.lens, self.off, self.stats = pos, lens, off, stats
        self.planes = planes
        if self.cap:
            last_read["regrows"] = last_read.get("regrows", 0) + 1
        self.cap = cap


class _StreamValues:

    _DIMS = (("i64_vals", 0), ("f32_vals", 0), ("elem_len", 0),
             ("bytes_data", 1), ("sub_count", 2))

    def __init__(self, fields, total_bytes: int, device):
        self.total_bytes = total_bytes
        self.device = device
        self.ok = True
        self.kinds = [wire_kind_of(f.dataType) for f in fields]
        self.seqs = [is_sequence_field(f.dataType) for f in fields]
        self.filled = [[0] * len(fields) for _ in range(3)]
        self.bufs = []
        for kind in self.kinds:
            dt = {"i64_vals": torch.int64, "f32_vals": torch.float32,
                  "elem_len": torch.int64, "bytes_data": torch.uint8,
                  "sub_count": torch.int64}
            self.bufs.append({k: torch.empty(0, dtype=d, device=device)
                              for k, d in dt.items()})

    def _used(self, i: int, name: str) -> bool:
        kind = self.kinds[i]
        return {"i64_vals": kind == KIND_INT64, "f32_vals": kind == KIND_FLOAT,
                "elem_len": kind == KIND_BYTES}.get(name, True)

    def _reserve(self, totals, bytes_seen: int):
        for i, bufs in enumerate(self.bufs):
            for name, dim in self._DIMS:
                if not self._used(i, name):
                    continue
                need = int(totals[dim][i])
                old = bufs[name]
                cap = stream_plan.grown_capacity(
                    old.numel(), need, bytes_seen, self.total_bytes,
                    _STREAM_HEADROOM, min_unit=1)
                if cap == old.numel():
                    continue
                new = torch.empty(cap, dtype=old.dtype, device=self.device)
                k = self.filled[dim][i]
                if k:
                    new[:k].copy_(old[:k])
                if old.numel():
                    last_read["regrows"] = last_read.get("regrows", 0) + 1
                bufs[name] = new

    def extract(self, data, rows, r0: int, r1: int, totals, bytes_seen: int,
                meta_dev, xerr, avg_bytes: int, max_blocks: int):
        self._reserve(totals, bytes_seen)
        v, b, l = rows.planes
        metas = []
        for i, bufs in enumerate(self.bufs):
            metas.append({
                "kind": self.kinds[i], "is_seq": 1 if self.seqs[i] else 0,
                "i64_vals": bufs["i64_vals"].data_ptr(),
                "f32_vals": bufs["f32_vals"].data_ptr(),
                "bytes_data": bufs["bytes_data"].data_ptr(),
                "elem_len": bufs["elem_len"].data_ptr(),
                "sub_count": bufs["sub_count"].data_ptr(),
                "val_base": v[i].data_ptr(),
                "byte_base": b[i].data_ptr(),
                "list_base": l[i].data_ptr() if self.seqs[i] else 0,
            })
        _native.gpu_extract_fields(data.data_ptr(), r1 - r0, len(self.bufs),
                                   rows.stats.data_ptr(), metas,
                                   meta_dev.data_ptr(), xerr.data_ptr(),
                                   _stream(), avg_bytes, r0=r0,
                                   max_blocks=max_blocks)
        self.filled = [[int(totals[d][i]) for i in range(len(self.bufs))]
                       for d in range(3)]

    def columns(self, stats, val_base, list_base, R: int) -> List[WireColumn]:
        cols = []
        for i, bufs in enumerate(self.bufs):
            kind, seq = self.kinds[i], self.seqs[i]
            nv, nb, nl = (self.filled[d][i] for d in range(3))
            presence = (stats[:, i, 0] >= 0).to(torch.uint8)
            elem_off = None
            if kind == KIND_BYTES:
                elem_off = excl_sum(bufs["elem_len"][:nv])
            sub_off = None
            if seq:
                sub_off = excl_sum(bufs["sub_count"][:nl])
            values = (bufs["i64_vals"][:nv] if kind == KIND_INT64 else
                      bufs["f32_vals"][:nv] if kind == KIND_FLOAT else
                      bufs["bytes_data"][:nb])
            cols.append(WireColumn(kind, seq, presence, val_base[i][:R + 1],
                                   values, elem_off,
                                   list_base[i][:R + 1] if seq else None,
                                   sub_off))
        return cols


def gz_device_meta(path: str):
    from ..io import paths as P

    if not getattr(_native, "HAS_GPU_KERNELS", False):
        return None
    return P.parse_gz_segments_file(path)


def _device_inflate_group(data: torch.Tensor, gz_items, device) -> bool:
    import os as _os

    comp_sizes = [_os.path.getsize(p) for p, _, _ in gz_items]
    comp_total = sum(comp_sizes)
    comp = torch.empty(max(comp_total, 1), dtype=torch.uint8,
                       device=device)[:comp_total]
    main = torch.cuda.current_stream()
    streams = _dma_streams()
    in_off = []
    in_len = []
    out_off = []
    out_len = []
    used = []
    coff = 0
    for k, (p, meta, out_base) in enumerate(gz_items):
        body_off, segs, _crc, _isize = meta
        ptr, pinned = _native.file_mmap_pinned(p, comp_sizes[k], False)
        if pinned:
            st = streams[k % len(streams)]
            st.wait_stream(main)
            _native.gpu_memcpy_h2d(comp.data_ptr() + coff, ptr, comp_sizes[k],
                                   st.cuda_stream)
            used.append(st)
        else:
            _read_file_staged(p, comp[coff:coff + comp_sizes[k]])
        so = coff + body_off
        uo = out_base
        for c, u in segs:
            in_off.append(so)
            in_len.append(c)
            out_off.append(uo)
            out_len.append(u)
            so += c
            uo += u
        coff += comp_sizes[k]
    for st in set(used):
        main.wait_stream(st)
    meta_np = np.array([in_off, in_len, out_off, out_len], np.int64)
    force = _os.environ.get("TFREC_INFLATE_STREAMS", "")
    spw_lit = 2
    if force in ("1", "2", "4"):
        spw_lit = int(force)
        lit = np.full(meta_np.shape[1], spw_lit > 1)
    else:
        lit = meta_np[1] >= (0.85 * np.maximum(meta_np[3], 1))
    err = torch.full((1,), -1, dtype=torch.int64, device=device)
    for mask, spw in ((lit, spw_lit), (~lit, 1)):
        k = int(mask.sum())
        if k == 0:
            continue
        idx = np.nonzero(mask)[0]
        if spw == 2 and k > 2:
            idx = idx[np.argsort(-meta_np[3, idx], kind="stable")]
        sub = torch.as_tensor(
            np.ascontiguousarray(meta_np[:, idx])).to(device)
        _native.gpu_inflate_segments(
            comp.data_ptr(), sub[0].data_ptr(), sub[1].data_ptr(),
            sub[2].data_ptr(), sub[3].data_ptr(), k,
            data.data_ptr(), err.data_ptr(), _stream(), spw)
    return int(err.item()) == -1


def read_gzip_file_to_device(path: str, device="cuda") -> Optional[torch.Tensor]:
    meta = gz_device_meta(path)
    if meta is None:
        return None
    total_u = sum(u for _, u in meta[1])
    data = torch.empty(max(total_u, 1), dtype=torch.uint8,
                       device=device)[:total_u]
    if not _device_inflate_group(data, [(path, meta, 0)], device):
        return None
    return data


def read_files_to_batch(paths, schema: StructType, record_type: str,
                        verify_crc: bool = True, device="cuda"):
    import os as _os

    from ..io import paths as P

    check_native()
    metas = []
    sizes = []
    for p in paths:
        if P.codec_from_path(p) == "gzip":
            meta = P.parse_gz_segments_file(p)
            if meta is None:
                raise ValueError(f"gzip file without segment table: {p} "
                                 "(host path required)")
            metas.append(meta)
            sizes.append(sum(u for _, u in meta[1]))
        else:
            metas.append(None)
            sizes.append(_os.path.getsize(p))
    n = sum(sizes)
    if n == 0:
        if schema is None:
            raise ValueError(
                "Could not infer schema: no non-empty TFRecord files found")
        z = torch.zeros(0, dtype=torch.int64, device=device)
        return (decode_device(torch.zeros(0, dtype=torch.uint8, device=device),
                              z, z.clone(), schema, record_type, verify_crc),
                np.zeros(len(paths), np.int64))
    data = torch.empty(n, dtype=torch.uint8, device=device)
    bounds = np.zeros(len(paths) + 1, np.int64)
    np.cumsum(sizes, out=bounds[1:])
    main = torch.cuda.current_stream()
    streams = _dma_streams()
    gz_items = []
    for i, p in enumerate(paths):
        if not sizes[i]:
            continue
        if metas[i] is not None:
            gz_items.append((p, metas[i], int(bounds[i])))
            continue
        ptr, pinned = _native.file_mmap_pinned(p, sizes[i], False)
        if pinned:
            st = streams[i % len(streams)]
            _native.gpu_memcpy_h2d(data.data_ptr() + int(bounds[i]), ptr,
                                   sizes[i], st.cuda_stream)
            main.wait_stream(st)
        else:
            _read_file_staged(p, data[int(bounds[i]):int(bounds[i + 1])])
    if gz_items and not _device_inflate_group(data, gz_items, device):
        import logging

        logging.getLogger(__name__).warning(
            "device inflate rejected a segment; host zlib fallback for "
            "%d gzip file(s)", len(gz_items))
        for p, meta, base in gz_items:
            blob = np.frombuffer(P.decompress_file(p), np.uint8)
            stage = pinned_buffer("gzfb", blob.size)
            stage.numpy()[:blob.size] = blob
            data[base:base + blob.size].copy_(stage[:blob.size],
                                              non_blocking=True)
            torch.cuda.current_stream().synchronize()
    off, lens = scan_frames_device(data)
    frame_start = off - 12
    counts = torch.searchsorted(
        frame_start, torch.as_tensor(bounds, device=device)).cpu().numpy()
    row_counts = np.diff(counts)
    if schema is None:
        from ..infer import byte_array_schema, schema_from_codes

        if record_type == "ByteArray":
            schema = byte_array_schema()
        else:
            i = next((k for k in range(len(paths)) if row_counts[k] > 0), None)
            if i is None:
                raise ValueError(
                    "Could not infer schema: no non-empty TFRecord files found")
            r0, r1 = int(counts[i]), int(counts[i + 1])
            codes = infer_codes_device(data, off[r0:r1].contiguous(),
                                       lens[r0:r1].contiguous(), record_type)
            schema = schema_from_codes(codes)
    batch = decode_device(data, off, lens, schema, record_type, verify_crc)
    return batch, row_counts


def encode_partitions_device(batch: RecordBatch, part_codes: np.ndarray,
                             num_parts: int, record_type: str):
    check_native()
    R = batch.num_rows
    device = batch.columns[0].presence.device if batch.columns else torch.device("cuda")
    blob = torch.frombuffer(bytearray(schema_blob(batch.schema)),
                            dtype=torch.uint8).to(device)
    col_dicts = [_col_ptrs(c) for c in batch.columns]
    cols_dev = torch.empty(_native.gpu_devcols_bytes(len(col_dicts)),
                           dtype=torch.uint8, device=device)
    psize = torch.empty(R, dtype=torch.int64, device=device)
    _native.gpu_size_records(col_dicts, cols_dev.data_ptr(), blob.data_ptr(),
                             FMT[record_type], R, psize.data_ptr(), _stream())
    frame_off = excl_sum(psize)
    total = int(frame_off[-1].item())
    file = torch.empty(total, dtype=torch.uint8, device=device)
    err = torch.zeros(2, dtype=torch.int32, device=device)
    _native.gpu_emit_records(cols_dev.data_ptr(), blob.data_ptr(),
                             FMT[record_type], 0, R, frame_off.data_ptr(),
                             file.data_ptr(), err.data_ptr(), _stream(),
                             total // max(R, 1))
    codes = torch.as_tensor(np.ascontiguousarray(part_codes, np.int64),
                            device=device)
    order = torch.argsort(codes, stable=True)
    sizes = psize[order].contiguous()
    dst_off = excl_sum(sizes)
    src_off = frame_off[:-1][order].contiguous()
    out = torch.empty(total, dtype=torch.uint8, device=device)
    _native.gpu_gather_payloads(file.data_ptr(), src_off.data_ptr(),
                                sizes.data_ptr(), dst_off.data_ptr(), R,
                                out.data_ptr(), _stream(), total // max(R, 1))
    counts = torch.bincount(codes, minlength=num_parts)
    row_bound = torch.nn.functional.pad(torch.cumsum(counts, 0), (1, 0))
    byte_bound = dst_off[row_bound].cpu().numpy()
    _check_emit_err(err)
    ranges = [(p, int(byte_bound[p]), int(byte_bound[p + 1]))
              for p in range(num_parts) if byte_bound[p + 1] > byte_bound[p]]
    return out, ranges



_INFER_SLOTS = 2048
_INFER_SLOTS_MAX = 1 << 21
_ERR_OVERFLOW = -5
_ERR_NAME_TOO_LONG = -6


def infer_codes_device(data: torch.Tensor, off: torch.Tensor,
                       lens: torch.Tensor, record_type: str) -> dict:
    check_native()
    device = data.device
    fmt = FMT["SequenceExample" if record_type == "SequenceExample" else "Example"]
    R = off.numel()
    slots = _INFER_SLOTS
    while True:
        table = torch.zeros((slots, 3), dtype=torch.int64, device=device)
        err = torch.zeros(2, dtype=torch.int32, device=device)
        if R:
            _native.gpu_infer_codes(data.data_ptr(), off.data_ptr(),
                                    lens.data_ptr(), R, fmt, table.data_ptr(),
                                    slots, err.data_ptr(), _stream())
        tab = table.cpu().numpy()
        rc = int(err[0].item())
        if rc == _ERR_OVERFLOW:
            if slots < _INFER_SLOTS_MAX:
                slots *= 4
                continue
            raise RuntimeError(
                "schema inference failed: more than "
                f"{_INFER_SLOTS_MAX // 2} distinct feature names")
        if rc == _ERR_NAME_TOO_LONG:
            raise RuntimeError(
                "schema inference failed: a feature name exceeds 65535 bytes")
        if rc != 0:
            rec = int(err[1].item()) - 1
            where = f" (record {rec})" if rec >= 0 else ""
            raise RuntimeError(f"malformed record during schema inference"
                               f"{where} (native error {rc})")
        break
    used = np.nonzero(tab[:, 0])[0]
    if len(used) == 0:
        return {}
    refs = tab[used, 1]
    offs = (refs >> 16).astype(np.int64)
    nlens = (refs & 0xFFFF).astype(np.int64)
    lo = int(offs.min())
    hi = int((offs + nlens).max())
    codes: dict = {}
    if hi - lo <= (4 << 20):
        blob = data[lo:hi].cpu().numpy().tobytes()
        for o, ln, code in zip(offs, nlens, tab[used, 2]):
            name = blob[o - lo:o - lo + ln].decode("utf-8", errors="replace")
            codes[name] = max(codes.get(name, 0), int(code))
    else:
        for o, ln, code in zip(offs, nlens, tab[used, 2]):
            name = data[o:o + ln].cpu().numpy().tobytes().decode("utf-8", errors="replace")
            codes[name] = max(codes.get(name, 0), int(code))
    return codes


def infer_schema_file(path: str, record_type: str, device="cuda"):
    from ..infer import schema_from_codes

    data = read_file_to_device(path, device)
    off, lens = scan_frames_device(data)
    return schema_from_codes(infer_codes_device(data, off, lens, record_type))


def batch_to_device(batch: RecordBatch, device="cuda") -> RecordBatch:
    cols = []
    for c in batch.columns:
        cols.append(WireColumn(
            c.kind, c.is_seq,
            _dev(c.presence, torch.uint8, device),
            _dev(c.row_off, torch.int64, device),
            _dev(c.values, {KIND_INT64: torch.int64, KIND_FLOAT: torch.float32,
                            KIND_BYTES: torch.uint8}[c.kind], device),
            _dev(c.elem_off, torch.int64, device) if c.elem_off is not None else None,
            _dev(c.list_off, torch.int64, device) if c.list_off is not None else None,
            _dev(c.sub_off, torch.int64, device) if c.sub_off is not None else None,
        ))
    return RecordBatch(batch.schema, cols, batch.num_rows)


def batch_to_host(batch: RecordBatch) -> RecordBatch:
# ... 59 lines not shown
```

Before: 112.6 million rows/s.

## Emit offsets and presence directly in extract kernels, inline field table, add frame find/gather

Extract kernels now write element and sub-list offsets directly instead of lengths and counts, and write presence per row. This removes the separate exclusive-sum scans and the presence comparison kernels. The field metadata table is passed as a kernel argument when there are at most 32 fields, which avoids a host-to-device copy. A new mask-based frame find/offsets/gather kernel path is added for record framing. Together these touch many parts of the pipeline and change the output formats between stages.

```diff
diff --git a/csrc/codec_core.h b/csrc/codec_core.h
--- a/csrc/codec_core.h
+++ b/csrc/codec_core.h
@@ -781,8 +781,8 @@
   i64* i64_vals;
   float* f32_vals;
   u8* bytes_data;
-  i64* elem_len;
-  i64* sub_count;
+  i64* elem_off;
+  i64* sub_off;
 };
 
 TFR_HOSTDEV inline int32_t extract_list_body(const u8* p, const u8* end, int32_t kind,
@@ -803,6 +803,7 @@
       p = read_varint(p, end, &len);
       if (!p || static_cast<u64>(end - p) < len) return ERR_TRUNCATED;
       u8* d = dst.bytes_data + *bi;
+      dst.elem_off[*vi] = *bi;
       u64 i = 0;
       for (; i + 8 <= len; i += 8) {
         u64 w;
@@ -810,7 +811,6 @@
         __builtin_memcpy(d + i, &w, 8);
       }
       for (; i < len; ++i) d[i] = p[i];
-      dst.elem_len[*vi] = static_cast<i64>(len);
       *bi += static_cast<i64>(len);
       *vi += 1;
       p += len;
@@ -900,10 +900,9 @@
       u64 flen;
       p = read_varint(p, end, &flen);
       if (!p || static_cast<u64>(end - p) < flen) return ERR_TRUNCATED;
-      i64 v_before = vi;
+      dst.sub_off[li++] = vi;
       int32_t rc = extract_feature_body(p, p + flen, kind, dst, &vi, &bi);
       if (rc != ERR_OK) return rc;
-      dst.sub_count[li++] = vi - v_before;
       p += flen;
     } else {
       p = skip_field(p, end, wt);
diff --git a/csrc/ext.cpp b/csrc/ext.cpp
--- a/csrc/ext.cpp
+++ b/csrc/ext.cpp
@@ -302,8 +302,8 @@
     py::array_t<i64> i64_vals(0);
     py::array_t<float> f32_vals(0);
     py::array_t<u8> bytes_data(0);
-    py::array_t<i64> elem_len(0);
-    py::array_t<i64> sub_count(0);
+    py::array_t<i64> elem_off(0);
+    py::array_t<i64> sub_off(0);
     if (fd.kind == KIND_INT64) {
       i64_vals = py::array_t<i64>(total_vals);
       dst.i64_vals = i64_vals.mutable_data();
@@ -312,13 +312,15 @@
       dst.f32_vals = f32_vals.mutable_data();
     } else {
       bytes_data = py::array_t<u8>(total_bytes);
-      elem_len = py::array_t<i64>(total_vals);
+      elem_off = py::array_t<i64>(total_vals + 1);
       dst.bytes_data = bytes_data.mutable_data();
-      dst.elem_len = elem_len.mutable_data();
+      dst.elem_off = elem_off.mutable_data();
+      dst.elem_off[total_vals] = total_bytes;
     }
     if (fd.is_seq) {
-      sub_count = py::array_t<i64>(total_lists);
-      dst.sub_count = sub_count.mutable_data();
+      sub_off = py::array_t<i64>(total_lists + 1);
+      dst.sub_off = sub_off.mutable_data();
+      dst.sub_off[total_lists] = total_vals;
     }
 
     {
@@ -363,11 +365,11 @@
     else if (fd.kind == KIND_FLOAT) d["values"] = f32_vals;
     else {
       d["values"] = bytes_data;
-      d["elem_len"] = elem_len;
+      d["elem_off"] = elem_off;
     }
     if (fd.is_seq) {
       d["list_off"] = list_off_arr;
-      d["sub_count"] = sub_count;
+      d["sub_off"] = sub_off;
     }
     out.append(d);
   }
diff --git a/csrc/hip/kernels.hip b/csrc/hip/kernels.hip
--- a/csrc/hip/kernels.hip
+++ b/csrc/hip/kernels.hip
@@ -119,17 +119,32 @@
   i64* i64_vals;
   float* f32_vals;
   u8* bytes_data;
-  i64* elem_len;
-  i64* sub_count;
+  i64* elem_off;
+  i64* sub_off;
+  u8* presence;
   const i64* val_base;
   const i64* byte_base;
   const i64* list_base;
 };
 
-__global__ void extract_fields_kernel(const u8* __restrict__ data, i64 R, int F,
-                                      const FieldStat* __restrict__ stats,
-                                      const DevFieldDst* __restrict__ metas,
-                                      int32_t* __restrict__ err, i64 r0) {
+constexpr int kInlineFields = 32;
+struct DevFieldTable {
+  DevFieldDst m[kInlineFields];
+};
+static_assert(sizeof(DevFieldTable) < 3072, "field table must fit the kernargs");
+
+__device__ inline void finish_field_row(const DevFieldDst& m, i64 pos, i64 r,
+                                        bool last) {
+  m.presence[r] = pos >= 0 ? 1 : 0;
+  if (!last) return;
+  if (m.kind == KIND_BYTES) m.elem_off[m.val_base[r + 1]] = m.byte_base[r + 1];
+  if (m.is_seq) m.sub_off[m.list_base[r + 1]] = m.val_base[r + 1];
+}
+
+__device__ __forceinline__ void extract_fields_body(
+    const u8* __restrict__ data, i64 R, int F,
+    const FieldStat* __restrict__ stats, const DevFieldDst* __restrict__ metas,
+    int32_t* __restrict__ err, i64 r0) {
   i64 total = R * F;
   for (i64 idx = blockIdx.x * (i64)blockDim.x + threadIdx.x; idx < total;
        idx += (i64)gridDim.x * blockDim.x) {
@@ -138,13 +153,29 @@
     i64 r = r0 + q;
     const DevFieldDst& m = metas[f];
     const FieldStat& st = stats[r * F + f];
-    DecodeDst dst{m.i64_vals, m.f32_vals, m.bytes_data, m.elem_len, m.sub_count};
+    finish_field_row(m, st.pos, r, q == R - 1);
+    DecodeDst dst{m.i64_vals, m.f32_vals, m.bytes_data, m.elem_off, m.sub_off};
     int32_t rc = extract_field(data, st.pos, st.len, m.kind, m.is_seq, dst,
                                m.val_base ? m.val_base[r] : 0,
                                m.byte_base ? m.byte_base[r] : 0,
                                m.list_base ? m.list_base[r] : 0);
     if (rc != ERR_OK) set_err(err, rc, r);
   }
+}
+
+__global__ void extract_fields_kernel(const u8* __restrict__ data, i64 R, int F,
+                                      const FieldStat* __restrict__ stats,
+                                      const DevFieldTable tab,
+                                      int32_t* __restrict__ err, i64 r0) {
+  extract_fields_body(data, R, F, stats, tab.m, err, r0);
+}
+
+__global__ void extract_fields_big_kernel(const u8* __restrict__ data, i64 R,
+                                          int F,
+                                          const FieldStat* __restrict__ stats,
+                                          const DevFieldDst* __restrict__ metas,
+                                          int32_t* __restrict__ err, i64 r0) {
+  extract_fields_body(data, R, F, stats, metas, err, r0);
 }
 
 
@@ -337,8 +368,8 @@
       u64 len;
       p = read_varint(p, end, &len);
       if (!p || (u64)(end - p) < len) return ERR_TRUNCATED;
+      if (lane == 0) dst.elem_off[*vi] = *bi;
       copy_wave(dst.bytes_data + *bi, p, (i64)len);
-      if (lane == 0) dst.elem_len[*vi] = (i64)len;
       *bi += (i64)len;
       *vi += 1;
       p += len;
@@ -426,11 +457,10 @@
       u64 flen;
       p = read_varint(p, end, &flen);
       if (!p || (u64)(end - p) < flen) return ERR_TRUNCATED;
-      i64 v_before = vi;
+      if (lane == 0) dst.sub_off[li] = vi;
+      ++li;
       int32_t rc = extract_feature_body_wave(p, p + flen, kind, dst, &vi, &bi);
       if (rc != ERR_OK) return rc;
-      if (lane == 0) dst.sub_count[li] = vi - v_before;
-      ++li;
       p += flen;
     } else {
       p = skip_field(p, end, wt);
@@ -479,11 +509,10 @@
   }
 }
 
-__global__ void extract_fields_wave_kernel(const u8* __restrict__ data, i64 R,
-                                           int F,
-                                           const FieldStat* __restrict__ stats,
-                                           const DevFieldDst* __restrict__ metas,
-                                           int32_t* __restrict__ err, i64 r0) {
+__device__ __forceinline__ void extract_fields_wave_body(
+    const u8* __restrict__ data, i64 R, int F,
+    const FieldStat* __restrict__ stats, const DevFieldDst* __restrict__ metas,
+    int32_t* __restrict__ err, i64 r0) {
   i64 total = R * F;
   i64 wave = (blockIdx.x * (i64)blockDim.x + threadIdx.x) / 64;
   i64 nwaves = ((i64)gridDim.x * blockDim.x) / 64;
@@ -493,13 +522,29 @@
     i64 r = r0 + q;
     const DevFieldDst& m = metas[f];
     const FieldStat& st = stats[r * F + f];
-    DecodeDst dst{m.i64_vals, m.f32_vals, m.bytes_data, m.elem_len, m.sub_count};
+    if ((threadIdx.x & 63) == 0) finish_field_row(m, st.pos, r, q == R - 1);
+    DecodeDst dst{m.i64_vals, m.f32_vals, m.bytes_data, m.elem_off, m.sub_off};
     int32_t rc = extract_field_wave(data, st.pos, st.len, m.kind, m.is_seq, dst,
                                     m.val_base ? m.val_base[r] : 0,
                                     m.byte_base ? m.byte_base[r] : 0,
                                     m.list_base ? m.list_base[r] : 0);
     if (rc != ERR_OK && (threadIdx.x & 63) == 0) set_err(err, rc, r);
   }
+}
+
+__global__ void extract_fields_wave_kernel(const u8* __restrict__ data, i64 R,
+                                           int F,
+                                           const FieldStat* __restrict__ stats,
+                                           const DevFieldTable tab,
+                                           int32_t* __restrict__ err, i64 r0) {
+  extract_fields_wave_body(data, R, F, stats, tab.m, err, r0);
+}
+
+__global__ void extract_fields_wave_big_kernel(
+    const u8* __restrict__ data, i64 R, int F,
+    const FieldStat* __restrict__ stats, const DevFieldDst* __restrict__ metas,
+    int32_t* __restrict__ err, i64 r0) {
+  extract_fields_wave_body(data, R, F, stats, metas, err, r0);
 }
 
 
@@ -795,6 +840,118 @@
                        cand_len[slot] = len;
                        ++slot;
                      });
+}
+
+
+template <int J>
+__global__ void frame_find_kernel(const u8* __restrict__ data, i64 N,
+                                  i64 pos_start, i64 pos_end,
+                                  uint16_t* __restrict__ masks,
+                                  i64* __restrict__ block_counts) {
+  __shared__ uint32_t tab[8][256];
+  __shared__ unsigned int wsum[kBlock / 64];
+  stage_crc_tables(tab);
+  const u64* wdata = reinterpret_cast<const u64*>(data);
+  const i64 c_lo = pos_start / kPosPerLane;
+  const i64 c_hi = (pos_end + kPosPerLane - 1) / kPosPerLane;
+  const i64 rel0 = (i64)blockIdx.x * (J * kBlock) + threadIdx.x;
+  unsigned int my = 0;
+#pragma unroll 1
+  for (int j = 0; j < J; ++j) {
+    const i64 rel = rel0 + (i64)j * kBlock;
+    const i64 c = c_lo + rel;
+    if (c >= c_hi) break;
+    const i64 p0 = c * kPosPerLane;
+    unsigned int m = 0;
+    eval_frame_chunk(data, wdata, N, c, pos_start, pos_end, tab,
+                     [&](i64 i, i64) { m |= 1u << (int)(i - p0); });
+    masks[rel] = (uint16_t)m;
+    my += __popc(m);
+  }
+  for (int d = 32; d; d >>= 1) my += __shfl_down(my, d);
+  if ((threadIdx.x & 63) == 0) wsum[threadIdx.x >> 6] = my;
+  __syncthreads();
+  if (threadIdx.x == 0) {
+    unsigned int s = 0;
+    for (int w = 0; w < kBlock / 64; ++w) s += wsum[w];
+    block_counts[blockIdx.x] = (i64)s;
+  }
+}
+
+__global__ void frame_offsets_kernel(const i64* __restrict__ counts, i64 B,
+                                     i64* __restrict__ off) {
+  __shared__ i64 part[kBlock];
+  const int t = threadIdx.x;
+  const i64 per = (B + kBlock - 1) / kBlock;
+  i64 lo = (i64)t * per;
+  if (lo > B) lo = B;
+  const i64 hi = lo + per < B ? lo + per : B;
+  i64 s = 0;
+  for (i64 i = lo; i < hi; ++i) s += counts[i];
+  part[t] = s;
+  __syncthreads();
+  for (int d = 1; d < kBlock; d <<= 1) {
+    i64 v = t >= d ? part[t - d] : 0;
+    __syncthreads();
+    part[t] += v;
+    __syncthreads();
+  }
+  i64 run = part[t] - s;
+  for (i64 i = lo; i < hi; ++i) {
+    off[i] = run;
+    run += counts[i];
+  }
+  if (t == kBlock - 1) off[B] = part[t];
+}
+
+template <int J>
+__global__ void frame_gather_kernel(const u8* __restrict__ data, i64 pos_start,
+                                    i64 pos_end,
+                                    const uint16_t* __restrict__ masks,
+                                    const i64* __restrict__ block_off,
+                                    i64* __restrict__ cand_pos,
+                                    i64* __restrict__ cand_len) {
+  __shared__ unsigned int cnt[J][kBlock];
+  const i64 base = block_off[blockIdx.x];
+  if (block_off[blockIdx.x + 1] == base) return;
+  const int t = threadIdx.x;
+  const i64 c_lo = pos_start / kPosPerLane;
+  const i64 c_hi = (pos_end + kPosPerLane - 1) / kPosPerLane;
+  const i64 rel0 = (i64)blockIdx.x * (J * kBlock) + t;
+  unsigned int m[J];
+#pragma unroll
+  for (int j = 0; j < J; ++j) {
+    const i64 rel = rel0 + (i64)j * kBlock;
+    m[j] = c_lo + rel < c_hi ? masks[rel] : 0u;
+    cnt[j][t] = __popc(m[j]);
+  }
+  __syncthreads();
+  for (int d = 1; d < kBlock; d <<= 1) {
+    unsigned int v[J];
+#pragma unroll
+    for (int j = 0; j < J; ++j) v[j] = t >= d ? cnt[j][t - d] : 0u;
+    __syncthreads();
+#pragma unroll
+    for (int j = 0; j < J; ++j) cnt[j][t] += v[j];
+    __syncthreads();
+  }
+  i64 row = base;
+#pragma unroll
+  for (int j = 0; j < J; ++j) {
+    unsigned int mm = m[j];
+    i64 slot = row + (i64)(cnt[j][t] - __popc(mm));
+    row += (i64)cnt[j][kBlock - 1];
+    const i64 p0 = (c_lo + rel0 + (i64)j * kBlock) * kPosPerLane;
+    while (mm) {
+      const i64 pos = p0 + (__ffs(mm) - 1);
+      mm &= mm - 1;
+      u64 len;
+      __builtin_memcpy(&len, data + pos, 8);
+      cand_pos[slot] = pos;
+      cand_len[slot] = (i64)len;
+      ++slot;
+    }
+  }
 }
 
 __global__ void frame_chain_kernel(const i64* __restrict__ pos,
@@ -1101,7 +1258,10 @@
                         uintptr_t stream, i64 avg_bytes, i64 r0,
                         i64 max_blocks) {
   if (R <= 0 || F <= 0) return;
-  std::vector<DevFieldDst> host_metas(F);
+  const bool inl = F <= kInlineFields;
+  DevFieldTable tab{};
+  std::vector<DevFieldDst> big(inl ? 0 : F);
+  DevFieldDst* host_metas = inl ? tab.m : big.data();
   for (int f = 0; f < F; ++f) {
     py::dict d = metas[f].cast<py::dict>();
     DevFieldDst& m = host_metas[f];
@@ -1110,27 +1270,39 @@
     m.i64_vals = (i64*)d["i64_vals"].cast<uintptr_t>();
     m.f32_vals = (float*)d["f32_vals"].cast<uintptr_t>();
     m.bytes_data = (u8*)d["bytes_data"].cast<uintptr_t>();
-    m.elem_len = (i64*)d["elem_len"].cast<uintptr_t>();
-    m.sub_count = (i64*)d["sub_count"].cast<uintptr_t>();
+    m.elem_off = (i64*)d["elem_off"].cast<uintptr_t>();
+    m.sub_off = (i64*)d["sub_off"].cast<uintptr_t>();
+    m.presence = (u8*)d["presence"].cast<uintptr_t>();
     m.val_base = (const i64*)d["val_base"].cast<uintptr_t>();
     m.byte_base = (const i64*)d["byte_base"].cast<uintptr_t>();
     m.list_base = (const i64*)d["list_base"].cast<uintptr_t>();
   }
-  HIP_CHECK(hipMemcpyAsync((void*)meta_dev, host_metas.data(),
-                           sizeof(DevFieldDst) * F, hipMemcpyHostToDevice,
-                           (hipStream_t)stream));
-  if (avg_bytes > kWaveRecordBytes) {
-    hipLaunchKernelGGL(extract_fields_wave_kernel,
-                       dim3(grid_for(R * F * 64, max_blocks)), dim3(kBlock), 0,
-                       (hipStream_t)stream, (const u8*)data, R, F,
-                       (const FieldStat*)stats, (const DevFieldDst*)meta_dev,
-                       (int32_t*)err, r0);
+  const bool wave = avg_bytes > kWaveRecordBytes;
+  dim3 grid(grid_for(wave ? R * F * 64 : R * F, max_blocks));
+  auto s = (hipStream_t)stream;
+  if (inl) {
+    if (wave)
+      hipLaunchKernelGGL(extract_fields_wave_kernel, grid, dim3(kBlock), 0, s,
+                         (const u8*)data, R, F, (const FieldStat*)stats, tab,
+                         (int32_t*)err, r0);
+    else
+      hipLaunchKernelGGL(extract_fields_kernel, grid, dim3(kBlock), 0, s,
+                         (const u8*)data, R, F, (const FieldStat*)stats, tab,
+                         (int32_t*)err, r0);
   } else {
-    hipLaunchKernelGGL(extract_fields_kernel,
-                       dim3(grid_for(R * F, max_blocks)), dim3(kBlock), 0,
-                       (hipStream_t)stream, (const u8*)data, R, F,
-                       (const FieldStat*)stats, (const DevFieldDst*)meta_dev,
-                       (int32_t*)err, r0);
+    if (!meta_dev)
+      throw std::runtime_error("gpu_extract_fields: meta_dev needed for F > " +
+                               std::to_string(kInlineFields));
+    HIP_CHECK(hipMemcpyAsync((void*)meta_dev, big.data(),
+                             sizeof(DevFieldDst) * F, hipMemcpyHostToDevice, s));
+    if (wave)
+      hipLaunchKernelGGL(extract_fields_wave_big_kernel, grid, dim3(kBlock), 0,
+                         s, (const u8*)data, R, F, (const FieldStat*)stats,
+                         (const DevFieldDst*)meta_dev, (int32_t*)err, r0);
+    else
+      hipLaunchKernelGGL(extract_fields_big_kernel, grid, dim3(kBlock), 0, s,
+                         (const u8*)data, R, F, (const FieldStat*)stats,
+                         (const DevFieldDst*)meta_dev, (int32_t*)err, r0);
   }
   HIP_CHECK(hipGetLastError());
 }
@@ -1232,6 +1404,67 @@
                      dim3(kBlock), 0, (hipStream_t)stream, (const u8*)data, N,
                      pos_start, pos_end, block_base, (i64*)block_off,
                      (i64*)cand_pos, (i64*)cand_len);
+  HIP_CHECK(hipGetLastError());
+}
+
+int find_rows(i64 tile_kib) {
+  if (tile_kib != 16 && tile_kib != 32 && tile_kib != 64)
+    throw std::runtime_error("frame find: tile must be 16, 32 or 64 KiB");
+  return (int)(tile_kib * 1024 / (kPosPerLane * kBlock));
+}
+
+i64 gpu_frame_find_chunks(i64 pos_start, i64 pos_end) {
+  if (pos_end <= pos_start) return 0;
+  return (pos_end + kPosPerLane - 1) / kPosPerLane - pos_start / kPosPerLane;
+}
+
+i64 gpu_frame_find_blocks(i64 pos_start, i64 pos_end, i64 tile_kib) {
+  i64 per = (i64)find_rows(tile_kib) * kBlock;
+  return (gpu_frame_find_chunks(pos_start, pos_end) + per - 1) / per;
+}
+
+void gpu_frame_find(uintptr_t data, i64 N, i64 pos_start, i64 pos_end,
+                    i64 tile_kib, uintptr_t masks, uintptr_t block_counts,
+                    uintptr_t stream) {
+  i64 B = gpu_frame_find_blocks(pos_start, pos_end, tile_kib);
+  if (B <= 0) return;
+  auto go = [&](auto kernel) {
+    hipLaunchKernelGGL(kernel, dim3((uint32_t)B), dim3(kBlock), 0,
+                       (hipStream_t)stream, (const u8*)data, N, pos_start,
+                       pos_end, (uint16_t*)masks, (i64*)block_counts);
+  };
+  switch (find_rows(tile_kib)) {
+    case 4: go(frame_find_kernel<4>); break;
+    case 8: go(frame_find_kernel<8>); break;
+    default: go(frame_find_kernel<16>); break;
+  }
+  HIP_CHECK(hipGetLastError());
+}
+
+void gpu_frame_offsets(uintptr_t counts, i64 B, uintptr_t off,
+                       uintptr_t stream) {
+  if (B < 0) return;
+  hipLaunchKernelGGL(frame_offsets_kernel, dim3(1), dim3(kBlock), 0,
+                     (hipStream_t)stream, (const i64*)counts, B, (i64*)off);
+  HIP_CHECK(hipGetLastError());
+}
+
+void gpu_frame_gather(uintptr_t data, i64 pos_start, i64 pos_end, i64 tile_kib,
+                      uintptr_t masks, uintptr_t block_off, uintptr_t cand_pos,
+                      uintptr_t cand_len, uintptr_t stream) {
+  i64 B = gpu_frame_find_blocks(pos_start, pos_end, tile_kib);
+  if (B <= 0) return;
+  auto go = [&](auto kernel) {
+    hipLaunchKernelGGL(kernel, dim3((uint32_t)B), dim3(kBlock), 0,
+                       (hipStream_t)stream, (const u8*)data, pos_start, pos_end,
+                       (const uint16_t*)masks, (const i64*)block_off,
+                       (i64*)cand_pos, (i64*)cand_len);
+  };
+  switch (find_rows(tile_kib)) {
+    case 4: go(frame_gather_kernel<4>); break;
+    case 8: go(frame_gather_kernel<8>); break;
+    default: go(frame_gather_kernel<16>); break;
+  }
   HIP_CHECK(hipGetLastError());
 }
 
@@ -1572,6 +1805,11 @@
   m.def("gpu_frame_scan_blocks", &gpu_frame_scan_blocks);
   m.def("gpu_frame_scan_count", &gpu_frame_scan_count);
   m.def("gpu_frame_scan_emit", &gpu_frame_scan_emit);
+  m.def("gpu_frame_find_chunks", &gpu_frame_find_chunks);
+  m.def("gpu_frame_find_blocks", &gpu_frame_find_blocks);
+  m.def("gpu_frame_find", &gpu_frame_find);
+  m.def("gpu_frame_offsets", &gpu_frame_offsets);
+  m.def("gpu_frame_gather", &gpu_frame_gather);
   m.def("gpu_frame_chain", &gpu_frame_chain);
   m.def("gpu_gather_payloads", &gpu_gather_payloads, py::arg("data"),
         py::arg("off"), py::arg("len"), py::arg("dst_off"), py::arg("R"),
@@ -1593,5 +1831,6 @@
   m.def("gpu_memcpy_h2d", &gpu_memcpy_h2d);
   m.def("gpu_devcols_bytes", &gpu_devcols_bytes);
   m.def("gpu_devmeta_bytes", []() { return sizeof(DevFieldDst); });
+  m.def("gpu_inline_fields", []() { return kInlineFields; });
   m.def("gpu_fieldstat_words", []() { return sizeof(FieldStat) / 8; });
 }
diff --git a/spark_tfrecord_amd/columnar.py b/spark_tfrecord_amd/columnar.py
--- a/spark_tfrecord_amd/columnar.py
+++ b/spark_tfrecord_amd/columnar.py
@@ -103,14 +103,8 @@
 
 
 def native_dict_to_wire(d: dict, kind: int, is_seq: bool) -> WireColumn:
-    elem_off = None
-    if "elem_len" in d:
-        elem_off = np.zeros(len(d["elem_len"]) + 1, dtype=np.int64)
-        np.cumsum(d["elem_len"], out=elem_off[1:])
-    sub_off = None
-    if "sub_count" in d:
-        sub_off = np.zeros(len(d["sub_count"]) + 1, dtype=np.int64)
-        np.cumsum(d["sub_count"], out=sub_off[1:])
+    elem_off = d.get("elem_off")
+    sub_off = d.get("sub_off")
     return WireColumn(
         kind=kind,
         is_seq=is_seq,
diff --git a/spark_tfrecord_amd/engine/gpu.py b/spark_tfrecord_amd/engine/gpu.py
--- a/spark_tfrecord_amd/engine/gpu.py
+++ b/spark_tfrecord_amd/engine/gpu.py
@@ -64,6 +64,8 @@
 _STREAM_HEADROOM = float(os.environ.get("TFREC_STREAM_HEADROOM", 1.125))
 _STREAM_MAX_BLOCKS = int(os.environ.get("TFREC_STREAM_MAX_BLOCKS", 0))
 _STREAM_EXTRACT = os.environ.get("TFREC_STREAM_EXTRACT", "1") != "0"
+_FRAME_FIND = os.environ.get("TFREC_FRAME_FIND", "1") != "0"
+_FIND_TILE = int(os.environ.get("TFREC_FIND_TILE", 16))
 _SYNC_WRITES = os.environ.get("TFREC_SYNC", "1") != "0"
 
 
@@ -428,44 +430,48 @@
         o["f32_vals"] = torch.empty(nv if kind == KIND_FLOAT else 0,
                                     dtype=torch.float32, device=device)
         o["bytes_data"] = torch.empty(nb, dtype=torch.uint8, device=device)
-        o["elem_len"] = torch.empty(nv if kind == KIND_BYTES else 0,
+        o["elem_off"] = torch.empty(nv + 1 if kind == KIND_BYTES else 0,
                                     dtype=torch.int64, device=device)
-        o["sub_count"] = torch.empty(nl, dtype=torch.int64, device=device)
+        o["sub_off"] = torch.empty(nl + 1 if seq else 0, dtype=torch.int64,
+                                   device=device)
+        o["presence"] = torch.empty(R, dtype=torch.uint8, device=device)
         outs.append(o)
         metas.append({
             "kind": kind, "is_seq": 1 if seq else 0,
             "i64_vals": o["i64_vals"].data_ptr(),
             "f32_vals": o["f32_vals"].data_ptr(),
             "bytes_data": o["bytes_data"].data_ptr(),
-            "elem_len": o["elem_len"].data_ptr(),
-            "sub_count": o["sub_count"].data_ptr(),
+            "elem_off": o["elem_off"].data_ptr(),
+            "sub_off": o["sub_off"].data_ptr(),
+            "presence": o["presence"].data_ptr(),
             "val_base": val_base[i].data_ptr(),
             "byte_base": byte_base[i].data_ptr(),
             "list_base": list_base[i].data_ptr() if seq else 0,
         })
 
-    meta_dev = torch.empty(F * _native.gpu_devmeta_bytes(), dtype=torch.uint8,
-                           device=device)
+    meta_dev = _field_table_buffer(F, device)
     _native.gpu_extract_fields(data.data_ptr(), R, F, stats.data_ptr(), metas,
-                               meta_dev.data_ptr(), err.data_ptr(), _stream(),
-                               avg_bytes)
+                               meta_dev.data_ptr() if meta_dev is not None
+                               else 0, err.data_ptr(), _stream(), avg_bytes)
 
     cols: List[WireColumn] = []
-    for i, (f, o) in enumerate(zip(fields, outs)):
+    for i, o in enumerate(outs):
         kind = o["kind"]
         seq = o["seq"]
-        presence = (stats[:, i, 0] >= 0).to(torch.uint8)
-        elem_off = None
-        if kind == KIND_BYTES:
-            elem_off = excl_sum(o["elem_len"])
-        sub_off = None
-        if seq:
-            sub_off = excl_sum(o["sub_count"])
         values = (o["i64_vals"] if kind == KIND_INT64 else
                   o["f32_vals"] if kind == KIND_FLOAT else o["bytes_data"])
-        cols.append(WireColumn(kind, seq, presence, val_base[i], values,
-                               elem_off, list_base[i] if seq else None, sub_off))
+        cols.append(WireColumn(kind, seq, o["presence"], val_base[i], values,
+                               o["elem_off"] if kind == KIND_BYTES else None,
+                               list_base[i] if seq else None,
+                               o["sub_off"] if seq else None))
     return cols
+
+
+def _field_table_buffer(F: int, device):
+    if F <= _native.gpu_inline_fields():
+        return None
+    return torch.empty(F * _native.gpu_devmeta_bytes(), dtype=torch.uint8,
+                       device=device)
 
 
 def decode_buffer_device(data_np: np.ndarray, schema: StructType, record_type: str,
@@ -625,10 +631,23 @@
     device = data.device
     plan = stream_plan.plan_slices(n, _READ_SLICE)
     S = len(plan)
-    nblocks = [int(_native.gpu_frame_scan_blocks(p.scan_lo, p.scan_hi))
-               if p.scan_hi > p.scan_lo else 0 for p in plan]
-    block_counts = torch.empty(max(sum(nblocks), 1), dtype=torch.int64,
-                               device=device)
+    use_find = _FRAME_FIND and _STREAM_DECODE
+    if use_find:
+        nblocks = [int(_native.gpu_frame_find_blocks(p.scan_lo, p.scan_hi,
+                                                     _FIND_TILE))
+                   if p.scan_hi > p.scan_lo else 0 for p in plan]
+        masks = torch.empty(
+            max(max(int(_native.gpu_frame_find_chunks(p.scan_lo, p.scan_hi))
+                    for p in plan), 1), dtype=torch.int16, device=device)
+        block_counts = torch.empty(max(max(nblocks), 1), dtype=torch.int64,
+                                   device=device)
+        block_off = torch.empty(max(nblocks) + 1, dtype=torch.int64,
+                                device=device)
+    else:
+        nblocks = [int(_native.gpu_frame_scan_blocks(p.scan_lo, p.scan_hi))
+                   if p.scan_hi > p.scan_lo else 0 for p in plan]
+        block_counts = torch.empty(max(sum(nblocks), 1), dtype=torch.int64,
+                                   device=device)
     main = torch.cuda.current_stream()
     streams = _dma_streams()
     events = []
@@ -669,8 +688,7 @@
         if do_scan:
             blob = _schema_blob_device(schema, device)
             vals = _StreamValues(fields, n, device) if _STREAM_EXTRACT else None
-            meta_dev = torch.empty(F * _native.gpu_devmeta_bytes(),
-                                   dtype=torch.uint8, device=device)
+            meta_dev = _field_table_buffer(F, device)
 
     base = 0
     C = 0
@@ -683,7 +701,7 @@
             main.wait_event(ev)
         last = s == S - 1
         nb = nblocks[s]
-        if nb:
+        if nb and not use_find:
             _native.gpu_frame_scan_count(data.data_ptr(), n, p.scan_lo,
                                          p.scan_hi, base,
                                          block_counts.data_ptr(), _stream())
@@ -691,15 +709,30 @@
             base += nb
             continue
         if nb:
-            block_off = excl_sum(block_counts[base:base + nb])
-            c_s = int(block_off[-1].item())
+            if use_find:
+                _native.gpu_frame_find(data.data_ptr(), n, p.scan_lo,
+                                       p.scan_hi, _FIND_TILE, masks.data_ptr(),
+                                       block_counts.data_ptr(), _stream())
+                _native.gpu_frame_offsets(block_counts.data_ptr(), nb,
+                                          block_off.data_ptr(), _stream())
+                c_s = int(block_off[nb].item())
+            else:
+                block_off = excl_sum(block_counts[base:base + nb])
+                c_s = int(block_off[-1].item())
             base += nb
             if c_s:
                 rows.reserve(C + c_s, C, r_done, p.scan_hi)
-                _native.gpu_frame_scan_emit(
-                    data.data_ptr(), n, p.scan_lo, p.scan_hi, 0,
-                    block_off.data_ptr(), rows.pos.data_ptr() + C * 8,
-                    rows.lens.data_ptr() + C * 8, _stream())
+                if use_find:
+                    _native.gpu_frame_gather(
+                        data.data_ptr(), p.scan_lo, p.scan_hi, _FIND_TILE,
+                        masks.data_ptr(), block_off.data_ptr(),
+                        rows.pos.data_ptr() + C * 8,
+                        rows.lens.data_ptr() + C * 8, _stream())
+                else:
+                    _native.gpu_frame_scan_emit(
+                        data.data_ptr(), n, p.scan_lo, p.scan_hi, 0,
+                        block_off.data_ptr(), rows.pos.data_ptr() + C * 8,
+                        rows.lens.data_ptr() + C * 8, _stream())
                 _native.gpu_frame_chain(
                     rows.pos.data_ptr() + C * 8, rows.lens.data_ptr() + C * 8,
                     c_s, sp + (_ST_CARRY + nchain) * 8,
@@ -750,8 +783,12 @@
 
     def unstreamed():
         last_read["path"] = "fallback" if _STREAM_DECODE else "unstreamed"
-        ranges = [(p.scan_lo, p.scan_hi) for p in plan if p.scan_hi > p.scan_lo]
-        off, lens, _ = _emit_and_chain(data, ranges, block_counts, n)
+        if use_find:
+            off, lens = scan_frames_device(data)
+        else:
+            ranges = [(p.scan_lo, p.scan_hi) for p in plan
+                      if p.scan_hi > p.scan_lo]
+            off, lens, _ = _emit_and_chain(data, ranges, block_counts, n)
         return decode_device(data, off, lens, schema, record_type, verify_crc)
 
     if not streaming or C == 0:
@@ -787,7 +824,7 @@
         if pending is not None:
             vals.extract(data, rows, pending[0], pending[1], totals_h, n,
                          meta_dev, xerr, avg_bytes, 0)
-        cols = vals.columns(stats, val_base, list_base, R)
+        cols = vals.columns(rows, val_base, list_base, R)
     err_h = xerr.cpu()
     if int(err_h[0]) != 0:
         _raise_extract_error(int(err_h[0]), int(err_h[1]))
@@ -806,18 +843,21 @@
         self.cap = 0
         self.pos = self.lens = self.off = self.stats = None
         self.planes = None
+        self.presence = None
 
     def _alloc(self, cap: int):
         i64 = dict(dtype=torch.int64, device=self.device)
-        planes = None
+        planes = presence = None
         if self.F:
             planes = [torch.empty((self.F, cap + 1), **i64) for _ in range(3)]
             for t in planes:
                 t[:, 0] = 0
+            presence = torch.empty((self.F, cap), dtype=torch.uint8,
+                                   device=self.device)
         return (torch.empty(cap, **i64), torch.empty(cap, **i64),
                 torch.empty(cap, **i64),
                 torch.empty((cap, self.F, 6), **i64) if self.F else None,
-                planes)
+                planes, presence)
 
     def scan_stats(self, r0: int, r1: int):
         ws = _stat_scan_workspace(r1 - r0, self.F, self.device)
@@ -835,7 +875,7 @@
                                          self.total_bytes, _STREAM_HEADROOM)
         if cap == self.cap:
             return
-        pos, lens, off, stats, planes = self._alloc(cap)
+        pos, lens, off, stats, planes, presence = self._alloc(cap)
         if n_cand:
             pos[:n_cand].copy_(self.pos[:n_cand])
             lens[:n_cand].copy_(self.lens[:n_cand])
@@ -844,8 +884,9 @@
             stats[:n_scanned].copy_(self.stats[:n_scanned])
             for new, old in zip(planes, self.planes):
                 new[:, :n_scanned + 1].copy_(old[:, :n_scanned + 1])
+            presence[:, :n_scanned].copy_(self.presence[:, :n_scanned])
         self.pos, self.lens, self.off, self.stats = pos, lens, off, stats
-        self.planes = planes
+        self.planes, self.presence = planes, presence
         if self.cap:
             last_read["regrows"] = last_read.get("regrows", 0) + 1
         self.cap = cap
@@ -853,8 +894,8 @@
 
 class _StreamValues:
 
-    _DIMS = (("i64_vals", 0), ("f32_vals", 0), ("elem_len", 0),
-             ("bytes_data", 1), ("sub_count", 2))
+    _DIMS = (("i64_vals", 0, 0), ("f32_vals", 0, 0), ("elem_off", 0, 1),
+             ("bytes_data", 1, 0), ("sub_off", 2, 1))
 
     def __init__(self, fields, total_bytes: int, device):
         self.total_bytes = total_bytes
@@ -866,22 +907,23 @@
         self.bufs = []
         for kind in self.kinds:
             dt = {"i64_vals": torch.int64, "f32_vals": torch.float32,
-                  "elem_len": torch.int64, "bytes_data": torch.uint8,
-                  "sub_count": torch.int64}
+                  "elem_off": torch.int64, "bytes_data": torch.uint8,
+                  "sub_off": torch.int64}
             self.bufs.append({k: torch.empty(0, dtype=d, device=device)
                               for k, d in dt.items()})
 
     def _used(self, i: int, name: str) -> bool:
         kind = self.kinds[i]
         return {"i64_vals": kind == KIND_INT64, "f32_vals": kind == KIND_FLOAT,
-                "elem_len": kind == KIND_BYTES}.get(name, True)
+                "elem_off": kind == KIND_BYTES,
+                "sub_off": self.seqs[i]}.get(name, True)
 
     def _reserve(self, totals, bytes_seen: int):
         for i, bufs in enumerate(self.bufs):
-            for name, dim in self._DIMS:
+            for name, dim, extra in self._DIMS:
                 if not self._used(i, name):
                     continue
-                need = int(totals[dim][i])
+                need = int(totals[dim][i]) + extra
                 old = bufs[name]
                 cap = stream_plan.grown_capacity(
                     old.numel(), need, bytes_seen, self.total_bytes,
@@ -889,7 +931,7 @@
                 if cap == old.numel():
                     continue
                 new = torch.empty(cap, dtype=old.dtype, device=self.device)
-                k = self.filled[dim][i]
+                k = min(self.filled[dim][i] + extra, old.numel())
                 if k:
                     new[:k].copy_(old[:k])
                 if old.numel():
@@ -907,32 +949,30 @@
                 "i64_vals": bufs["i64_vals"].data_ptr(),
                 "f32_vals": bufs["f32_vals"].data_ptr(),
                 "bytes_data": bufs["bytes_data"].data_ptr(),
-                "elem_len": bufs["elem_len"].data_ptr(),
-                "sub_count": bufs["sub_count"].data_ptr(),
+                "elem_off": bufs["elem_off"].data_ptr(),
+                "sub_off": bufs["sub_off"].data_ptr(),
+                "presence": rows.presence[i].data_ptr(),
                 "val_base": v[i].data_ptr(),
                 "byte_base": b[i].data_ptr(),
                 "list_base": l[i].data_ptr() if self.seqs[i] else 0,
             })
         _native.gpu_extract_fields(data.data_ptr(), r1 - r0, len(self.bufs),
                                    rows.stats.data_ptr(), metas,
-                                   meta_dev.data_ptr(), xerr.data_ptr(),
+                                   meta_dev.data_ptr() if meta_dev is not None
+                                   else 0, xerr.data_ptr(),
                                    _stream(), avg_bytes, r0=r0,
                                    max_blocks=max_blocks)
         self.filled = [[int(totals[d][i]) for i in range(len(self.bufs))]
                        for d in range(3)]
 
-    def columns(self, stats, val_base, list_base, R: int) -> List[WireColumn]:
+    def columns(self, rows, val_base, list_base, R: int) -> List[WireColumn]:
         cols = []
         for i, bufs in enumerate(self.bufs):
             kind, seq = self.kinds[i], self.seqs[i]
             nv, nb, nl = (self.filled[d][i] for d in range(3))
-            presence = (stats[:, i, 0] >= 0).to(torch.uint8)
-            elem_off = None
-            if kind == KIND_BYTES:
-                elem_off = excl_sum(bufs["elem_len"][:nv])
-            sub_off = None
-            if seq:
-                sub_off = excl_sum(bufs["sub_count"][:nl])
+            presence = rows.presence[i][:R]
+            elem_off = bufs["elem_off"][:nv + 1] if kind == KIND_BYTES else None
+            sub_off = bufs["sub_off"][:nl + 1] if seq else None
             values = (bufs["i64_vals"][:nv] if kind == KIND_INT64 else
                       bufs["f32_vals"][:nv] if kind == KIND_FLOAT else
                       bufs["bytes_data"][:nb])
```

After: 116.3 million rows/s (median of 3 runs). 1.03x the previous value.
